# eloj/radix-sorting

Hardware: AMD Instinct MI355X
Metric: Gkeys/s sorting 2^28 u32 (1 GPU) + HBM GB/s vs roofline; 1/2/4/8-GPU scaling (higher is better)
Workload: dtype u32

## Files before the change

### radix_sorting_amd/csrc/rsx_env.hpp

```cpp
#pragma once

#include <algorithm>
#include <atomic>
#include <climits>
#include <cstdint>
#include <cstdlib>
#include <mutex>

namespace {

std::atomic<uint32_t> g_env_epoch{0};
enum : unsigned { UNIQUE_MAX_BITS_COMPILED = 30, UNIQUE_MAX_BITS_DEFAULT = 24 };
enum : unsigned { GROUP_MAX_BITS_COMPILED = 30, GROUP_MAX_BITS_DEFAULT = 24 };
enum : unsigned { LEX_PACK_BYTES_DEFAULT = 4 };
enum : unsigned { LOCATE_MAX_VALUES_DEFAULT = 4096 };
enum : unsigned { REDUCE_LDS_BITS_COMPILED = 12, REDUCE_MAX_BITS_COMPILED = 24, REDUCE_MAX_BITS_DEFAULT = 12 };
enum : unsigned { PARTITION_MAX_EDGES_COMPILED = 255, PARTITION_MAX_EDGES_DEFAULT = 3, PARTITION_BALLOT_PARTS_ENV_DEFAULT = 7 };
enum : unsigned { SEGMENTS_MAX_LONG_COMPILED = 4096, SEGMENTS_MAX_LONG_DEFAULT = 8, SEGMENTS_DEFAULT_CLASSES = 8 };
struct Env {
	bool host_register = false;
	bool force_table_rank = false;
	bool verify = false;
	bool verify_whole = false;
	bool verify_inject = false;
	bool no_hot = false;
	bool elem_loads = false;
	bool no_small_tiles = false;
	bool no_hybrid = false;
	bool no_small_sort = false;
	bool no_fill_runs = false;
	bool no_speculation = false;
	bool compact_bits = false;
	bool no_narrow_keys = false;
	bool no_host_small = false;
	bool no_fused_hist = false;
	bool no_slack = false;
	bool no_self_plan = false;
	bool no_blind = false;
	unsigned blind_min_log2 = 0;
	bool no_leaf_prefix = false;
	bool no_leaf16w2k = false;
	bool no_leaf16q = false;
	bool no_narrow_slots = false;
	bool no_aux_slots = false;
	bool no_narrow1 = false;
	bool no_dense_slots = false;
	bool force_dense_slots = false;
	bool no_unstable = false;
	bool no_shift = false;
	bool no_pass16 = false;
	unsigned pass16_wgs = 2;
	bool no_packed_keys = false;
	bool no_pass32a = false;
	unsigned pass32_min_mi = 0;
	int pass32_prefetch = -1;
	bool no_pass16a = false;
	unsigned pass16_dbg = 0;
	bool no_leafc = false;
	unsigned force_leafc = 0;
	bool no_leaf16 = false;
	unsigned leaf16_maxbin = 25;
	unsigned leaf_grid = 65536;
	unsigned two_level_min_log2 = 27;
	bool no_odd_stride = false;
	unsigned cap1_pad_kib = 0;
	unsigned probe = 0;
	bool no_pass64a = false;
	bool no_log = false;
	bool log_leaf_big = false;
	bool pairs_leaf_big = false;
	unsigned log_min_log2 = 0;
	unsigned unique_max_bits = UNIQUE_MAX_BITS_DEFAULT;
	unsigned group_max_bits = GROUP_MAX_BITS_DEFAULT;
	bool rankdata_no_tables = false;
	unsigned nth_force = 0;
	unsigned topk_force = 0;
	unsigned locate_force = 0;
	unsigned locate_max_values = LOCATE_MAX_VALUES_DEFAULT;
	unsigned locate_counter_sets = 0;
	unsigned reduce_max_bits = REDUCE_MAX_BITS_DEFAULT;
	unsigned reduce_lds_bits = REDUCE_LDS_BITS_COMPILED;
	unsigned reduce_replicas = 0;
	unsigned reduce_force = 0;
	unsigned join_force = 0;
	bool join_no_table = false;
	unsigned lex_pack_bytes = LEX_PACK_BYTES_DEFAULT;
	unsigned partition_force = 0;
	unsigned partition_max_edges = PARTITION_MAX_EDGES_DEFAULT;
	unsigned partition_ballot_parts = PARTITION_BALLOT_PARTS_ENV_DEFAULT;
	unsigned segments_force = 0;
	unsigned segments_max_long = SEGMENTS_MAX_LONG_DEFAULT;
	static bool is_set(const char *name) { return getenv(name) != nullptr; }
	static unsigned one_or_two(const char *name)
	{
		const char *e = getenv(name);
		return !e ? 0u : e[0] == '1' ? 1u : e[0] == '2' ? 2u : 0u;
	}
	static bool is_one(const char *name) { return one_or_two(name) == 1; }
	static void number(const char *name, unsigned *x, int lo = INT_MIN, int hi = INT_MAX)
	{
		if (const char *e = getenv(name))
			*x = (unsigned)std::max(lo, std::min(hi, atoi(e)));
	}
	static void within(const char *name, unsigned *x, int lo, int hi)
	{
		const char *e = getenv(name);
		if (e && atoi(e) >= lo && atoi(e) <= hi)
			*x = (unsigned)atoi(e);
	}
	static void one_else_two(const char *name, unsigned *x)
	{
		if (const char *e = getenv(name))
			*x = atoi(e) == 1 ? 1u : 2u;
	}
	void load()
	{
		*this = Env{};
		host_register = is_one("RSX_HOST_REGISTER");
		force_table_rank = is_one("RSX_FORCE_TABLE_RANK");
		verify = one_or_two("RSX_VERIFY") == 1;
		verify_whole = one_or_two("RSX_VERIFY") == 2;
		verify_inject = is_set("RSX_VERIFY_INJECT");
		no_hot = is_set("RSX_NO_HOT");
		elem_loads = is_one("RSX_ELEM_LOADS");
		no_small_tiles = is_set("RSX_NO_SMALL_TILES");
		no_hybrid = is_one("RSX_NO_HYBRID");
		no_small_sort = is_set("RSX_NO_SMALL_SORT");
		no_fill_runs = is_set("RSX_NO_FILL_RUNS");
		no_speculation = is_set("RSX_NO_SPECULATION");
		compact_bits = is_one("RSX_COMPACT_BITS");
		no_narrow_keys = is_set("RSX_NO_NARROW_KEYS");
		no_host_small = is_set("RSX_NO_HOST_SMALL");
		no_fused_hist = is_one("RSX_NO_FUSED_HIST");
		no_slack = is_one("RSX_NO_SLACK");
		no_self_plan = is_one("RSX_NO_SELF_PLAN");
		no_blind = is_one("RSX_NO_BLIND");
		number("RSX_BLIND_MIN_LOG2", &blind_min_log2, 22, 30);
		no_leaf_prefix = is_one("RSX_NO_LEAF_PREFIX");
		no_leaf16q = is_one("RSX_NO_LEAF16Q");
		no_narrow_slots = is_one("RSX_NO_NARROW_SLOTS");
		no_aux_slots = is_one("RSX_NO_AUX_SLOTS");
		no_narrow1 = is_one("RSX_NO_NARROW_LEVEL1");
		no_dense_slots = is_one("RSX_NO_DENSE_SLOTS");
		force_dense_slots = is_one("RSX_DENSE_SLOTS");
		no_leaf16 = is_one("RSX_NO_LEAF16");
		no_leafc = is_one("RSX_NO_LEAFC");
		no_leaf16w2k = is_one("RSX_NO_LEAF16W2K");
		number("RSX_PASS32_MIN_MI", &pass32_min_mi);
		if (is_set("RSX_PASS32_PREFETCH"))
			pass32_prefetch = is_one("RSX_PASS32_PREFETCH");
		number("RSX_FORCE_LEAFC", &force_leafc);
		no_pass16 = is_one("RSX_NO_PASS16");
		no_pass16a = is_one("RSX_NO_PASS16A");
		no_pass32a = is_one("RSX_NO_PASS32A");
		no_packed_keys = is_one("RSX_NO_PACKED_KEYS");
		one_else_two("RSX_PASS16_WGS", &pass16_wgs);
		number("RSX_PASS16_DBG", &pass16_dbg);
		no_shift = is_one("RSX_NO_SHIFT");
		no_unstable = is_one("RSX_NO_UNSTABLE");
		number("RSX_LEAF16_MAXBIN", &leaf16_maxbin, 0, 25);
		number("RSX_LEAF_GRID", &leaf_grid, 256, 65536);
		no_odd_stride = is_one("RSX_NO_ODD_STRIDE");
		number("RSX_CAP1_PAD_KIB", &cap1_pad_kib, 0, 65536);
		number("RSX_PROBE", &probe);
		no_pass64a = is_one("RSX_NO_PASS64A");
		no_log = is_one("RSX_NO_LOG");
		log_leaf_big = is_one("RSX_LOG_LEAF_BIG");
		pairs_leaf_big = is_one("RSX_PAIRS_LEAF_BIG");
		number("RSX_LOG_MIN_LOG2", &log_min_log2, 20, 29);
		rankdata_no_tables = is_one("RSX_RANKDATA_NO_TABLES");
		topk_force = one_or_two("RSX_TOPK_FORCE");
		nth_force = one_or_two("RSX_NTH_FORCE");
		locate_force = one_or_two("RSX_LOCATE_FORCE");
		within("RSX_LOCATE_MAX_VALUES", &locate_max_values, 1, (int)LOCATE_MAX_VALUES_DEFAULT);
		within("RSX_LOCATE_COUNTER_SETS", &locate_counter_sets, 1, 32);
		within("RSX_LEX_PACK_BYTES", &lex_pack_bytes, 1, 8);
		partition_force = one_or_two("RSX_PARTITION_FORCE");
		within("RSX_PARTITION_MAX_EDGES", &partition_max_edges, 1, (int)PARTITION_MAX_EDGES_COMPILED);
		within("RSX_PARTITION_BALLOT_PARTS", &partition_ballot_parts, 0, 256);
		segments_force = one_or_two("RSX_SEGMENTS_FORCE");
		within("RSX_SEGMENTS_MAX_LONG", &segments_max_long, 0, (int)SEGMENTS_MAX_LONG_COMPILED);
		number("RSX_REDUCE_MAX_BITS", &reduce_max_bits, 0, (int)REDUCE_MAX_BITS_COMPILED);
		number("RSX_REDUCE_LDS_BITS", &reduce_lds_bits, 0, (int)REDUCE_LDS_BITS_COMPILED);
		within("RSX_REDUCE_REPLICAS", &reduce_replicas, 1, 32);
		reduce_force = one_or_two("RSX_REDUCE_FORCE");
		within("RSX_JOIN_FORCE", &join_force, 2, 3);
		join_no_table = is_one("RSX_JOIN_NO_TABLE");
		number("RSX_UNIQUE_MAX_BITS", &unique_max_bits, 0, (int)UNIQUE_MAX_BITS_COMPILED);
		number("RSX_GROUP_MAX_BITS", &group_max_bits, 0, (int)GROUP_MAX_BITS_COMPILED);
		within("RSX_TWO_LEVEL_MIN_LOG2", &two_level_min_log2, 22, 30);
	}
};
Env g_env;
std::once_flag g_env_once;
inline const Env &env()
{
	std::call_once(g_env_once, [] { g_env.load(); });
	return g_env;
}

}
```

### radix_sorting_amd/csrc/rsx_hybrid.hpp

```cpp
#pragma once

#include "rsx_kernels.hpp"

namespace rsx {

enum : u32 { HYB_NONE = 0, HYB_ONE_LEVEL = 1, HYB_TWO_LEVEL = 2 };
enum : u32 { SEG_MODE_NONE = 0, SEG_MODE_LEAVES = 1, SEG_MODE_LSD = 2, SEG_MODE_RETRY = 3 };
static_assert(GATE_DONE == SEG_MODE_LEAVES, "the gate of the histogram-first kernels is SegCtl::mode");

struct SegTile {
	u32 beg, cnt, bucket, first;
};

struct SegCtl {
	u32 ntiles;
	u32 mode;
	u32 maxleaf;
	u32 done;
	u32 nleaf;
	u32 overflow;
	u32 blind;
	u32 cmask_lo, cmask_hi, key0_lo, key0_hi;
	u32 nredo;
	u32 leaf16;
	u32 shift1, shift2;
	u32 narrow;
	u32 compact;
	u32 cpiece[4];
	u32 craw0, cvnot;
	u32 ckind;
	u32 boff_skip, boff_next;
};
__device__ __forceinline__ void segctl_attempt_lost(SegCtl *ctl)
{
	const u32 nx = ctl->boff_next ? (ctl->boff_next < 32u ? 2u * ctl->boff_next : 64u) : 1u;
	ctl->boff_next = nx;
	ctl->boff_skip = nx;
}
enum : u32 { BLIND_NONE = 0, BLIND_GO = 1, BLIND_FAILED = 2 };

template <typename KT>
__device__ __forceinline__ u32 compact_key(u32 raw, const u32 (&piece)[4], u32 nb, const KdfArgs<KT> ka)
{
	u32 c = 0;
#pragma unroll
	for (int i = 0; i < 4; ++i) {
		const u32 p = piece[i];
		c |= __builtin_amdgcn_ubfe(raw, p & 31u, (p >> 8) & 63u) << (p >> 16);
	}
	const u32 all = nb >= 32u ? ~0u : (1u << nb) - 1u;
	const bool neg = ka.fmask != 0 && (raw >> 31) != 0;
	const u32 top = (piece[0] & 31u) + ((piece[0] >> 8) & 63u) == 32u ? 1u << (nb - 1u) : 0u;
	u32 flip = neg ? all : (ka.sflip ? top : 0u);
	if (ka.desc)
		flip ^= all;
	return c ^ flip;
}

struct LeafSeg {
	u32 beg, cnt, ncols;
	u32 slot;
};

constexpr u32 LEAF_MERGE_CAP = 4096;

__device__ __forceinline__ u32 block_scan_256(u32 v, u32 *s_w, u32 &tot)
{
	const u32 lane = threadIdx.x & 63, wid = threadIdx.x >> 6;
	u32 x = v;
#pragma unroll
	for (int off = 1; off < 64; off <<= 1) {
		const u32 y = __shfl_up(x, off);
		if (lane >= (u32)off)
			x += y;
	}
	if (lane == 63)
		s_w[wid] = x;
	__syncthreads();
	u32 base = 0;
#pragma unroll
	for (int k = 0; k < 4; ++k) {
		if (k < (int)wid)
			base += s_w[k];
	}
	tot = s_w[0] + s_w[1] + s_w[2] + s_w[3];
	__syncthreads();
	return base + x - v;
}

__device__ __forceinline__ u32 fixedpoint_key(u32 raw, u32 scale_bits, u32 nb, bool nonneg, bool desc, u32 &bad)
{
	const float tf = __uint_as_float(raw) * __uint_as_float(scale_bits);
	const float hi = __uint_as_float((127u + nb - (nonneg ? 0u : 1u)) << 23);
	const float lo = nonneg ? 0.0f : -hi;
	const int t = (int)tf;
	if (!(tf >= lo && tf < hi) || (float)t != tf || raw == 0x80000000u)
		bad |= 1u;
	u32 key = nonneg ? (u32)t : (u32)(t + (int)(1u << (nb - 1u)));
	if (desc)
		key = ~key & ((1u << nb) - 1u);
	return key;
}

__global__ __launch_bounds__(256) void rsx_seg_tiles_kernel(const u64 *__restrict__ ghist, u64 n, const Plan *__restrict__ plan,
                                                            u32 tile, SegTile *__restrict__ tiles, SegCtl *__restrict__ ctl,
                                                            u32 *__restrict__ btile,
                                                            u64 *__restrict__ off1_out = nullptr, u32 blind_cap = 0,
                                                            const u32 *__restrict__ status0 = nullptr, u32 ntiles0 = 0,
                                                            u32 back_cap = 0, u32 tile_narrow = 0,
                                                            u32 tile_narrow2 = 0)
{
	if (plan->hyb != HYB_TWO_LEVEL || (blind_cap && ctl->blind != BLIND_GO))
		return;
	if (tile_narrow && ctl->narrow)
		tile = (tile_narrow2 && ctl->narrow == 2u) ? tile_narrow2 : tile_narrow;
	__shared__ u32 s_size[256], s_tb[257], s_beg[256], s_w[4], s_back[256];
	const u32 d = threadIdx.x;
	u32 size, back = 0;
	if (blind_cap) {
		if (back_cap) {
			size = __hip_atomic_load(status0 + d, __ATOMIC_RELAXED, __HIP_MEMORY_SCOPE_AGENT);
			back = __hip_atomic_load(status0 + 256 + d, __ATOMIC_RELAXED, __HIP_MEMORY_SCOPE_AGENT);
			size += back;
		} else {
			size = __hip_atomic_load(status0 + ((u64)(ntiles0 - 1) * 256 + d), __ATOMIC_RELAXED, __HIP_MEMORY_SCOPE_AGENT) & StatusBits<u32>::VALMASK;
		}
		const bool over = size > blind_cap || ctl->overflow != 0;
		u32 tot1;
		const u32 o = block_scan_256(size, s_w, tot1);
		if (blockIdx.x == 0)
			off1_out[d] = o;
		if (__syncthreads_or(over ? 1 : 0)) {
			if (blockIdx.x == 0 && d == 0) {
				ctl->blind = BLIND_FAILED;
				segctl_attempt_lost(ctl);
			}
			return;
		}
		s_beg[d] = d * blind_cap;
	} else {
		const u64 *off1 = ghist + 256 * plan->cols[plan->ncols - 1];
		const u64 b = off1[d], e = d == 255 ? n : off1[d + 1];
		size = (u32)(e - b);
		s_beg[d] = (u32)b;
	}
	s_size[d] = size;
	s_back[d] = back;
	u32 total;
	const u32 tb = block_scan_256((size - back + tile - 1) / tile + (back ? 1u : 0u), s_w, total);
	s_tb[d] = tb;
	if (d == 0) {
		s_tb[256] = total;
		if (blockIdx.x == 0) {
			ctl->ntiles = total;
			btile[256] = total;
		}
	}
	if (blockIdx.x == 0)
		btile[d] = tb;
	__syncthreads();
	for (u32 t = blockIdx.x * 256 + d; t < total; t += gridDim.x * 256) {
		u32 lo = 0, hi = 256;
		while (hi - lo > 1) {
			const u32 mid = (lo + hi) >> 1;
			if (s_tb[mid] <= t)
				lo = mid;
			else
				hi = mid;
		}
		while (s_tb[lo + 1] <= t)
			++lo;
		const u32 k = lo, j = t - s_tb[k];
		SegTile st;
		const u32 front = s_size[k] - s_back[k];
		if (j * tile < front) {
			st.beg = s_beg[k] + j * tile;
			const u32 left = front - j * tile;
			st.cnt = left < tile ? left : tile;
		} else {
			st.beg = s_beg[k] + blind_cap - back_cap;
			st.cnt = s_back[k];
		}
		st.bucket = k;
		st.first = s_tb[k];
		tiles[t] = st;
	}
}

template <typename KT>
__global__ __launch_bounds__(1024) void rsx_seg_hist_kernel(const KT *__restrict__ keys, const SegTile *__restrict__ tiles,
                                                            const SegCtl *__restrict__ ctl, const Plan *__restrict__ plan,
                                                            KdfArgs<KT> ka, u32 *__restrict__ seghist)
{
	if (plan->hyb != HYB_TWO_LEVEL || ctl->mode != SEG_MODE_LSD)
		return;
	constexpr int MAXS = sizeof(KT) - 1;
	__shared__ u32 h[MAXS][256];
	const u32 tid = threadIdx.x;
	const u32 nslots = plan->ncols - 2;
	u32 shifts[MAXS];
#pragma unroll
	for (int k = 0; k < MAXS; ++k)
		shifts[k] = 8 * plan->cols[k < (int)nslots ? k : 0];
	const u32 nt = ctl->ntiles;
	const u32 t0 = (u32)((u64)nt * blockIdx.x / gridDim.x), t1 = (u32)((u64)nt * (blockIdx.x + 1) / gridDim.x);
	if (t0 == t1)
		return;
	for (u32 i = tid; i < MAXS * 256; i += 1024)
		(&h[0][0])[i] = 0;
	__syncthreads();
	u32 bucket = tiles[t0].bucket;
	auto flush = [&]() {
		__syncthreads();
		for (u32 i = tid; i < nslots * 256; i += 1024) {
			const u32 v = (&h[0][0])[i];
			if (v)
				atomicAdd(&seghist[(u64)bucket * (MAXS * 256) + i], v);
			(&h[0][0])[i] = 0;
		}
		__syncthreads();
	};
	for (u32 t = t0; t < t1; ++t) {
		const SegTile st = tiles[t];
		if (st.bucket != bucket) {
			flush();
			bucket = st.bucket;
		}
		const KT *p = keys + st.beg;
		constexpr int U = 8;
		for (u32 i0 = 0; i0 < st.cnt; i0 += 1024 * U) {
			KT v[U];
#pragma unroll
			for (int u = 0; u < U; ++u) {
				const u32 i = i0 + u * 1024 + tid;
				v[u] = i < st.cnt ? p[i] : (KT)0;
			}
#pragma unroll
			for (int u = 0; u < U; ++u) {
				const u32 i = i0 + u * 1024 + tid;
				if (i < st.cnt) {
					const KT k = kdf_apply(v[u], ka);
#pragma unroll
					for (int s = 0; s < MAXS; ++s)
						if (s < (int)nslots)
							atomicAdd(&h[s][(u32)(k >> shifts[s]) & 0xFFu], 1u);
				}
			}
		}
	}
	flush();
}

template <typename KT>
__global__ __launch_bounds__(1024) void rsx_seg_hist1_kernel(const KT *__restrict__ keys, const SegTile *__restrict__ tiles,
                                                             const SegCtl *__restrict__ ctl, const Plan *__restrict__ plan,
                                                             KdfArgs<KT> ka, u32 *__restrict__ seghist)
{
	if (plan->hyb != HYB_TWO_LEVEL)
		return;
	constexpr int MAXS = sizeof(KT) - 1, NW = 16;
	__shared__ u32 h[NW][256];
	const u32 tid = threadIdx.x, wid = tid >> 6;
	const u32 slot = plan->ncols - 2;
	const u32 shift = 8 * plan->cols[slot];
	const u32 nt = ctl->ntiles;
	const u32 t0 = (u32)((u64)nt * blockIdx.x / gridDim.x), t1 = (u32)((u64)nt * (blockIdx.x + 1) / gridDim.x);
	if (t0 == t1)
		return;
	for (u32 i = tid; i < NW * 256; i += 1024)
		(&h[0][0])[i] = 0;
	__syncthreads();
	u32 bucket = tiles[t0].bucket;
	auto flush = [&]() {
		__syncthreads();
		if (tid < 256) {
			u32 v = 0;
#pragma unroll
			for (int w = 0; w < NW; ++w) {
				v += h[w][tid];
				h[w][tid] = 0;
			}
			if (v)
				atomicAdd(&seghist[((u64)bucket * MAXS + slot) * 256 + tid], v);
		}
		__syncthreads();
	};
	u32 *hw = h[wid];
	for (u32 t = t0; t < t1; ++t) {
		const SegTile st = tiles[t];
		if (st.bucket != bucket) {
			flush();
			bucket = st.bucket;
		}
		const KT *p = keys + st.beg;
		constexpr int U = 8;
		for (u32 i0 = 0; i0 < st.cnt; i0 += 1024 * U) {
			KT v[U];
			if (i0 + 1024 * U <= st.cnt) {
#pragma unroll
				for (int u = 0; u < U; ++u)
					v[u] = p[i0 + u * 1024 + tid];
#pragma unroll
				for (int u = 0; u < U; ++u)
					atomicAdd(&hw[digit_of(v[u], ka, shift)], 1u);
			} else {
#pragma unroll
				for (int u = 0; u < U; ++u) {
					const u32 i = i0 + u * 1024 + tid;
					v[u] = i < st.cnt ? p[i] : (KT)0;
				}
#pragma unroll
				for (int u = 0; u < U; ++u) {
					const u32 i = i0 + u * 1024 + tid;
					if (i < st.cnt)
						atomicAdd(&hw[digit_of(v[u], ka, shift)], 1u);
				}
			}
		}
	}
	flush();
}

template <typename KT>
__global__ __launch_bounds__(256) void rsx_seg_plan_kernel(u32 *__restrict__ seghist, const u64 *__restrict__ ghist, u64 n,
                                                           const Plan *__restrict__ plan, SegCtl *__restrict__ ctl,
                                                           LeafSeg *__restrict__ segtab, u32 leaf_cap, SegCtl *host_ctl,
                                                           u32 phase)
{
	if (plan->hyb != HYB_TWO_LEVEL || (phase == 1 && ctl->mode != SEG_MODE_LSD))
		return;
	constexpr int MAXS = sizeof(KT) - 1;
	__shared__ u64 tot[256];
	__shared__ u64 lsum[64];
	__shared__ u32 s_max;
	const u32 d = threadIdx.x, b = blockIdx.x;
	const u32 nslots = plan->ncols - 1;
	const u64 *off1 = ghist + 256 * plan->cols[plan->ncols - 1];
	const u64 bbeg = off1[b];
	if (d == 0)
		s_max = 0;
	for (u32 s = phase ? 0 : nslots - 1; s < (phase ? nslots - 1 : nslots); ++s) {
		u32 *row = seghist + ((u64)b * MAXS + s) * 256;
		const u32 c = row[d];
		__syncthreads();
		tot[d] = c;
		__syncthreads();
		if (d < 64)
			wave_scan_256(tot, lsum, d);
		__syncthreads();
		row[d] = (u32)tot[d];
		if (s == nslots - 1) {
			__shared__ u32 s_cnt[256], s_start[257], s_first[257], s_w[4];
			constexpr u32 H = LEAF_MERGE_CAP / 2;
			const u32 o = (u32)tot[d];
			s_cnt[d] = c;
			__syncthreads();
			const bool opens = d == 0 || c > H || s_cnt[d - 1] > H || (o / H) != ((o - s_cnt[d - 1]) / H);
			u32 nleaf;
			const u32 idx = block_scan_256(opens ? 1u : 0u, s_w, nleaf);
			if (opens) {
				s_start[idx] = o;
				s_first[idx] = d;
			}
			if (d == 0) {
				s_start[nleaf] = o;
				s_first[nleaf] = 256;
			}
			__syncthreads();
			if (d == 255)
				s_start[nleaf] = o + c;
			__syncthreads();
			__shared__ u32 s_slot;
			if (d == 0)
				s_slot = atomicAdd(&ctl->nleaf, nleaf);
			__syncthreads();
			u32 mine = 0;
			if (d < nleaf) {
				LeafSeg ls;
				ls.beg = (u32)(bbeg + s_start[d]);
				ls.cnt = s_start[d + 1] - s_start[d];
				ls.ncols = nslots - 1 + (s_first[d + 1] - s_first[d] > 1 ? 1u : 0u);
				ls.slot = 0;
				segtab[s_slot + d] = ls;
				mine = ls.cnt;
			}
			atomicMax(&s_max, mine);
		}
	}
	if (phase)
		return;
	__syncthreads();
	__shared__ u32 s_last;
	if (d == 0) {
		atomicMax(&ctl->maxleaf, s_max);
		__threadfence();
		s_last = atomicAdd(&ctl->done, 1u) == gridDim.x - 1 ? 1u : 0u;
	}
	__syncthreads();
	if (s_last && d == 0) {
		__threadfence();
		const u32 mx = atomicMax(&ctl->maxleaf, 0u);
		const u32 mode = mx <= leaf_cap ? SEG_MODE_LEAVES : SEG_MODE_LSD;
		ctl->mode = mode;
		if (host_ctl) {
			host_ctl->ntiles = ctl->ntiles;
			host_ctl->maxleaf = mx;
			host_ctl->nleaf = ctl->nleaf;
			host_ctl->mode = mode;
			__threadfence_system();
		}
	}
}

template <typename ST>
__global__ __launch_bounds__(256) void rsx_seg_slack_plan_kernel(const ST *__restrict__ status, const u32 *__restrict__ btile,
                                                                 const u64 *__restrict__ ghist, const Plan *__restrict__ plan,
                                                                 SegCtl *__restrict__ ctl, LeafSeg *__restrict__ segtab,
                                                                 u32 slack_cap, SegCtl *host_ctl,
                                                                 const u64 *__restrict__ off1_given = nullptr, u32 blind_ = 0)
{
	u32 blind = blind_ & 0xFFu;
	const u32 rev = blind_ >> 8;
	if (blind == 3u)
		blind = ctl->narrow ? 2u : 1u;
	if (plan->hyb != HYB_TWO_LEVEL || (blind && ctl->blind != BLIND_GO))
		return;
	typedef StatusBits<ST> SB_;
	__shared__ u32 s_w[4];
	const u32 d = threadIdx.x, b = blockIdx.x;
	const u64 *off1 = off1_given ? off1_given : ghist + 256 * plan->cols[plan->ncols - 1];
	const u32 t0 = btile[b], t1 = btile[b + 1];
	const u32 ncols = plan->ncols;
	const u64 bbeg = off1[b];
	u32 c = 0, back = 0;
	if (blind == 2) {
		c = (u32)__hip_atomic_load(status + ((u64)b * 256 + d), __ATOMIC_RELAXED, __HIP_MEMORY_SCOPE_AGENT);
		back = (u32)__hip_atomic_load(status + ((u64)65536 + b * 256 + d), __ATOMIC_RELAXED, __HIP_MEMORY_SCOPE_AGENT);
		c += back;
	} else if (t1 > t0) {
		c = (u32)(__hip_atomic_load(status + ((u64)(t1 - 1) * 256 + d), __ATOMIC_RELAXED, __HIP_MEMORY_SCOPE_AGENT) & SB_::VALMASK);
	}
	if (b == 0 && d == 0) {
		const u32 mode = ctl->overflow == 0 ? SEG_MODE_LEAVES : SEG_MODE_RETRY;
		ctl->mode = mode;
		ctl->nleaf = 65536;
		ctl->maxleaf = slack_cap;
		if (blind) {
			if (mode == SEG_MODE_LEAVES)
				ctl->boff_next = 0;
			else
				segctl_attempt_lost(ctl);
		}
		if (host_ctl) {
			host_ctl->ntiles = ctl->ntiles;
			host_ctl->maxleaf = slack_cap;
			host_ctl->nleaf = 65536;
			host_ctl->overflow = ctl->overflow;
			host_ctl->narrow = ctl->narrow;
			host_ctl->mode = mode;
		}
	}
	u32 total;
	const u32 o = block_scan_256(c, s_w, total);
	LeafSeg ls;
	ls.beg = (u32)(bbeg + o);
	ls.cnt = c <= slack_cap ? c : 0u;
	ls.ncols = (ncols - 2) | (back << 16);
	ls.slot = b * 256 + d + 1;
	segtab[rev ? 65535u - (b * 256 + d) : b * 256 + d] = ls;
}

template <typename KT>
__global__ __launch_bounds__(1024) void rsx_blind_precheck_kernel(const KT *__restrict__ src, u64 n, KdfArgs<KT> ka,
                                                                  SegCtl *__restrict__ ctl, Plan *__restrict__ plan,
                                                                  Plan *host_plan, u32x4 *__restrict__ z, u64 nz, u32 min_cols,
                                                                  u32 allow_shift = 0, u32 allow_narrow = 0, u32 allow_compact = 0,
                                                                  u32 backoff = 0,
                                                                  u32 hints = 0)
{
	constexpr u32 W = sizeof(KT), S = 8, NS = 1024 * S;
	__shared__ u32 h[W][256];
	__shared__ u32 s_desc, s_distinct[W], s_max[W];
	__shared__ u32 h12[4096];
	__shared__ u32 s_max12;
	__shared__ u32 hs[2][256];
	__shared__ u32 s_vary, s_maxs[2];
	const u32 tid = threadIdx.x;
	if (blockIdx.x != 0) {
		const u32x4 zero = {0, 0, 0, 0};
		for (u64 i = (u64)(blockIdx.x - 1) * 1024 + tid; i < nz; i += (u64)(gridDim.x - 1) * 1024)
			z[i] = zero;
		return;
	}
	for (u32 i = tid; i < W * 256; i += 1024)
		(&h[0][0])[i] = 0;
	if (tid < W) {
		s_distinct[tid] = 0;
		s_max[tid] = 0;
	}
	if (tid == 0)
		s_desc = s_max12 = s_vary = s_maxs[0] = s_maxs[1] = 0;
#pragma unroll
	for (u32 i = 0; i < 4; ++i)
		h12[tid + 1024 * i] = 0;
	if (tid < 512)
		(&hs[0][0])[tid] = 0;
	__syncthreads();
	const u64 i0 = ((n - 16 * S) / 63) * (tid >> 4) + (tid & 15u) * S;
	KT k[S];
#pragma unroll
	for (u32 e = 0; e < S; ++e)
		k[e] = kdf_apply(src[i0 + e], ka);
	bool desc = false;
#pragma unroll
	for (u32 e = 0; e < S; ++e) {
		if (e)
			desc |= k[e] < k[e - 1];
#pragma unroll
		for (u32 c = 0; c < W; ++c)
			atomicAdd(&h[c][(u32)(k[e] >> (8 * c)) & 0xFFu], 1u);
	}
	if (__ballot(desc) && (tid & 63) == 0)
		s_desc = 1;
	if constexpr (W == 4) {
		const u32 kw = (u32)__builtin_amdgcn_readfirstlane((int)(u32)k[0]);
		u32 v = 0;
#pragma unroll
		for (u32 e = 0; e < S; ++e)
			v |= (u32)k[e] ^ kw;
#pragma unroll
		for (int off = 32; off > 0; off >>= 1)
			v |= (u32)__shfl_xor((int)v, off);
		if ((tid & 63) == 0)
			atomicOr(&s_vary, v | (kw ^ (u32)kdf_apply(src[0], ka)));
	}
	__syncthreads();
	if (tid < 256) {
#pragma unroll
		for (u32 c = 0; c < W; ++c) {
			const u32 v = h[c][tid];
			const u64 m = __ballot(v != 0);
			u32 mx = v;
#pragma unroll
			for (int off = 32; off > 0; off >>= 1) {
				const u32 y = __shfl_xor(mx, off);
				mx = y > mx ? y : mx;
			}
			if ((tid & 63) == 0) {
				atomicAdd(&s_distinct[c], (u32)__popcll(m));
				atomicMax(&s_max[c], mx);
			}
		}
	}
	__syncthreads();
	u32 shift1 = 0, shift2 = 0;
	{
		u32 nk = 0, ck[8] = {0, 0, 0, 0, 0, 0, 0, 0};
#pragma unroll
		for (u32 c = 0; c < W; ++c) {
			if (s_distinct[c] >= 2)
				ck[nk++] = c;
		}
		bool shifted = false;
		if (nk >= 2) {
			shift1 = 8 * ck[nk - 1];
			shift2 = 8 * ck[nk - 2];
		}
		if constexpr (W == 4) {
			const u32 hb = s_vary ? 31u - (u32)__builtin_clz(s_vary) : 0u;
			if (allow_shift && nk == 4 && hb < 31u && hb >= 23u) {
				shift1 = hb - 7;
				shift2 = hb - 15;
				shifted = true;
			}
		}
		if (nk >= 4) {
#pragma unroll
			for (u32 e = 0; e < S; ++e) {
				atomicAdd(&hs[0][(u32)(k[e] >> shift1) & 0xFFu], 1u);
				atomicAdd(&hs[1][(u32)(k[e] >> shift2) & 0xFFu], 1u);
			}
			if (shifted) {
				const u32 lowmask = (1u << shift2) - 1u, d = shift2 > 12u ? shift2 - 12u : 0u;
#pragma unroll
				for (u32 e = 0; e < S; ++e)
					atomicAdd(&h12[((u32)k[e] & lowmask) >> d], 1u);
			} else {
				const u32 sh_hi = 8 * ck[nk - 3], sh_nx = 8 * ck[nk - 4] + 4;
#pragma unroll
				for (u32 e = 0; e < S; ++e)
					atomicAdd(&h12[(((u32)(k[e] >> sh_hi) & 0xFFu) << 4) | ((u32)(k[e] >> sh_nx) & 0xFu)], 1u);
			}
		}
		__syncthreads();
		u32 m = 0;
#pragma unroll
		for (u32 i = 0; i < 4; ++i)
			m = m > h12[tid + 1024 * i] ? m : h12[tid + 1024 * i];
		u32 ms = tid < 512 ? (&hs[0][0])[tid] : 0u;
#pragma unroll
		for (int off = 32; off > 0; off >>= 1) {
			const u32 y = __shfl_xor(m, off), ys = __shfl_xor(ms, off);
			m = y > m ? y : m;
			ms = ys > ms ? ys : ms;
		}
		if ((tid & 63) == 0) {
			atomicMax(&s_max12, m);
			if (tid < 512)
				atomicMax(&s_maxs[tid >> 8], ms);
		}
		__syncthreads();
	}
	__shared__ u32 s_vraw, s_cnb, s_cpiece[4], s_cmax[2], s_fx[3], s_fxnb, s_fxscale, s_ckind;
	if constexpr (W == 4) {
		if (allow_compact) {
			const u32 raw0 = (u32)src[0];
			u32 raw[S];
			u32 v = 0;
#pragma unroll
			for (u32 e = 0; e < S; ++e) {
				raw[e] = (u32)src[i0 + e];
				v |= raw[e] ^ raw0;
			}
#pragma unroll
			for (int off = 32; off > 0; off >>= 1)
				v |= (u32)__shfl_xor((int)v, off);
			if (tid == 0)
				s_vraw = s_cnb = s_cmax[0] = s_cmax[1] = s_ckind = s_fxnb = s_fxscale = 0;
			if (tid < 512)
				(&hs[0][0])[tid] = 0;
			__syncthreads();
			if ((tid & 63) == 0)
				atomicOr(&s_vraw, v);
			__syncthreads();
			if (tid == 0) {
				u32 vv = s_vraw, np = 0, nb = (u32)__popc(vv), left = nb;
				bool ok = nb >= 17u && nb <= 30u;
				u32 pc[4] = {0, 0, 0, 0};
				while (vv && ok) {
					const u32 hi = 31u - (u32)__builtin_clz(vv);
					const u32 below = ~vv & ((2u << hi) - 1u);
					const u32 lo = below ? 32u - (u32)__builtin_clz(below) : 0u;
					const u32 w = hi - lo + 1u;
					if (np == 4) {
						ok = false;
						break;
					}
					left -= w;
					pc[np++] = lo | (w << 8) | (left << 16);
					vv &= lo ? (1u << lo) - 1u : 0u;
				}
				for (u32 i = 0; i < 4; ++i)
					s_cpiece[i] = pc[i];
				s_cnb = ok ? nb : 0u;
			}
			__syncthreads();
			const u32 cnb = s_cnb;
			if (cnb) {
				const u32 pc[4] = {s_cpiece[0], s_cpiece[1], s_cpiece[2], s_cpiece[3]};
#pragma unroll
				for (u32 e = 0; e < S; ++e) {
					const u32 c = compact_key<KT>(raw[e], pc, cnb, ka);
					atomicAdd(&hs[0][(c >> (cnb - 8u)) & 0xFFu], 1u);
					atomicAdd(&hs[1][(c >> (cnb - 16u)) & 0xFFu], 1u);
				}
			}
			__syncthreads();
			if (cnb) {
				u32 ms = tid < 512 ? (&hs[0][0])[tid] : 0u;
#pragma unroll
				for (int off = 32; off > 0; off >>= 1) {
					const u32 ys = __shfl_xor(ms, off);
					ms = ys > ms ? ys : ms;
				}
				if ((tid & 63) == 0 && tid < 512)
					atomicMax(&s_cmax[tid >> 8], ms);
			}
			__syncthreads();
			const bool packed_ok = s_cnb && s_cmax[0] <= 2 * NS / 256 && s_cmax[1] <= 2 * NS / 256;
			if (!packed_ok && ka.fmask != 0) {
				u32 lo = 0xFFFFFFFFu, hi = 0, flags = 0;
#pragma unroll
				for (u32 e = 0; e < S; ++e) {
					const u32 E = (raw[e] >> 23) & 0xFFu, M = raw[e] & 0x7FFFFFu;
					flags |= (E == 255u || raw[e] == 0x80000000u) ? 1u : 0u;
					flags |= (raw[e] >> 31) ? 2u : 0u;
					if (raw[e] & 0x7FFFFFFFu) {
						const u32 mant = E ? (M | 0x800000u) : M, Ee = E ? E : 1u;
						const u32 w = 256u + Ee - 150u + (u32)__builtin_ctz(mant);
						lo = w < lo ? w : lo;
						const u32 t = 256u + Ee - 126u;
						hi = t > hi ? t : hi;
					}
				}
#pragma unroll
				for (int off = 32; off > 0; off >>= 1) {
					const u32 a = (u32)__shfl_xor((int)lo, off), b = (u32)__shfl_xor((int)hi, off);
					lo = a < lo ? a : lo;
					hi = b > hi ? b : hi;
					flags |= (u32)__shfl_xor((int)flags, off);
				}
				if (tid == 0) {
					s_fx[0] = 0xFFFFFFFFu;
					s_fx[1] = s_fx[2] = 0;
					s_cmax[0] = s_cmax[1] = 0;
					s_fxnb = 0;
				}
				if (tid < 512)
					(&hs[0][0])[tid] = 0;
				__syncthreads();
				if ((tid & 63) == 0) {
					atomicMin(&s_fx[0], lo);
					atomicMax(&s_fx[1], hi);
					atomicOr(&s_fx[2], flags);
				}
				__syncthreads();
				if (tid == 0 && (s_fx[2] & 1u) == 0 && s_fx[1] > s_fx[0]) {
					const int e0 = (int)s_fx[0] - 256, e1 = (int)s_fx[1] - 256;
					const int nb = e1 - e0 + ((s_fx[2] & 2u) ? 1 : 0);
					if (nb >= 17 && nb <= 30 && 127 - e0 >= 1 && 127 - e0 <= 254) {
						s_fxnb = (u32)nb;
						s_fxscale = (u32)(127 - e0) << 23;
					}
				}
				__syncthreads();
				const u32 fnb = s_fxnb;
				if (fnb) {
					const u32 sc = s_fxscale;
					u32 bad = 0;
#pragma unroll
					for (u32 e = 0; e < S; ++e) {
						const u32 c = fixedpoint_key(raw[e], sc, fnb, (s_fx[2] & 2u) == 0, ka.desc != 0, bad);
						atomicAdd(&hs[0][(c >> (fnb - 8u)) & 0xFFu], 1u);
						atomicAdd(&hs[1][(c >> (fnb - 16u)) & 0xFFu], 1u);
					}
					(void)bad;
				}
				__syncthreads();
				if (fnb) {
					u32 ms = tid < 512 ? (&hs[0][0])[tid] : 0u;
#pragma unroll
					for (int off = 32; off > 0; off >>= 1) {
						const u32 ys = __shfl_xor(ms, off);
						ms = ys > ms ? ys : ms;
					}
					if ((tid & 63) == 0 && tid < 512)
						atomicMax(&s_cmax[tid >> 8], ms);
				}
				__syncthreads();
				if (tid == 0 && fnb) {
					s_cnb = fnb;
					s_ckind = 1;
				}
				__syncthreads();
			}
		}
	}
	if (tid == 0) {
		bool go = s_desc != 0;
		u32 nk = 0, cols[8] = {0, 0, 0, 0, 0, 0, 0, 0};
		u64 cmask = 0;
		for (u32 c = 0; c < W; ++c) {
			if (s_distinct[c] >= 2)
				cols[nk++] = c;
			else
				cmask |= (u64)0xFFu << (8 * c);
		}
		if (shift1 + 8 < 8 * W)
			cmask |= ~(((u64)1 << (shift1 + 8)) - 1) & (W == 8 ? ~(u64)0 : (((u64)1 << (8 * (W & 7))) - 1));
		go = go && nk >= min_cols;
		for (u32 i = 0; i + 2 < nk; ++i) {
			go = go && s_max[cols[i]] <= NS / 10;
		}
		go = go && ((hints & 1u) || s_maxs[0] <= 2 * NS / 256) && s_maxs[1] <= 2 * NS / 256;
		const u32 nbins12 = (shift1 & 7u) && shift2 < 12u ? 1u << shift2 : 4096u;
		const u32 max12_ok = 3 * (NS / nbins12) + 18u;
		if (shift1 & 7u)
			go = go && s_max12 <= max12_ok;
		u32 compact = 0;
		if constexpr (W == 4) {
			if (!go && allow_compact && s_cnb && s_desc != 0 && nk == 4 && s_cmax[0] <= 2 * NS / 256 && s_cmax[1] <= 2 * NS / 256) {
				compact = s_cnb;
				go = true;
				shift1 = compact - 8u;
				shift2 = compact - 16u;
				cmask = 0;
			}
		}
		if (backoff && ctl->boff_skip) {
			ctl->boff_skip -= 1u;
			go = false;
			compact = 0;
		}
		ctl->compact = compact;
		ctl->ckind = compact ? s_ckind : 0u;
		for (u32 i = 0; i < 4; ++i)
			ctl->cpiece[i] = compact ? (s_ckind ? (i == 0 ? s_fxscale : i == 1 ? ((s_fx[2] & 2u) ? 0u : 1u) : 0u) : s_cpiece[i]) : 0u;
		ctl->craw0 = compact ? (u32)src[0] : 0u;
		ctl->cvnot = compact ? ~s_vraw : 0u;
		ctl->ntiles = ctl->mode = ctl->maxleaf = ctl->done = ctl->nleaf = ctl->overflow = ctl->nredo = 0;
		ctl->blind = go ? BLIND_GO : BLIND_FAILED;
		ctl->leaf16 = (s_max12 <= max12_ok || compact) ? 1u : 0u;
		u32 narrow = (W == 8 && allow_narrow && go && nk >= 4 && cols[nk - 3] <= 3u && s_max12 <= max12_ok) ? 1u : 0u;
		if (narrow && allow_narrow >= 2u && ((shift1 & 7u) ? shift1 <= 32u : cols[nk - 2] <= 3u))
			narrow = 2u;
		ctl->narrow = narrow;
		ctl->shift1 = shift1;
		ctl->shift2 = shift2;
		ctl->cmask_lo = (u32)cmask;
		ctl->cmask_hi = (u32)(cmask >> 32);
		ctl->key0_lo = (u32)(u64)k[0];
		ctl->key0_hi = (u32)((u64)k[0] >> 32);
		if (go) {
			Plan *const out[2] = {plan, host_plan};
			for (int j = 0; j < 2; ++j) {
				out[j]->ncols = nk;
				out[j]->sorted = 0;
				for (u32 i = 0; i < 8; ++i)
					out[j]->cols[i] = i < nk ? cols[i] : 0u;
				out[j]->hot = 0;
				out[j]->vary_lo = out[j]->vary_hi = 0;
				out[j]->hyb = HYB_TWO_LEVEL;
				out[j]->max1 = 0;
			}
		}
	}
}

template <typename KT, int NW_, int KPT_, int WPE_ = 1, bool RANK1_ = true, bool PREFETCH_ = false> struct LeafCfg {
	static constexpr int NW = NW_, KPT = KPT_, BLOCK = NW_ * 64, CAP = NW_ * 64 * KPT_;
	static constexpr int WPE = WPE_;
	static constexpr bool RANK1 = RANK1_;
	static constexpr bool PREFETCH = PREFETCH_;
	static_assert(CAP <= 32768, "ranks and positions are kept in 16 bits");
};

template <typename KT, typename C, typename CT = KT, bool DENSE = false>
__global__ __launch_bounds__(C::BLOCK, C::WPE) void rsx_leaf_sort_kernel(KT *__restrict__ src, KT *__restrict__ aux, u64 n,
                                                                  const u64 *__restrict__ ghist, const Plan *__restrict__ plan,
                                                                  const LeafSeg *__restrict__ segtab,
                                                                  const SegCtl *__restrict__ ctl, KdfArgs<KT> ka, u32 level,
                                                                  u32 lo, u32 hi, const KT *__restrict__ slots = nullptr,
                                                                  u32 slack_cap = 0, u32 skip_narrowable = 0,
                                                                  const u64 *__restrict__ off1_given = nullptr,
                                                                  const u32 *__restrict__ redo = nullptr)
{
	constexpr int NW = C::NW, KPT = C::KPT, BLOCK = C::BLOCK;
	constexpr bool NARROW = sizeof(CT) < sizeof(KT);
	constexpr int CHUNK = 16 / sizeof(CT);
	constexpr int G = 4;
	static_assert(KPT % G == 0, "whole groups of rounds");
	const u32 hyb = plan->hyb, ncols = plan->ncols, max1 = plan->max1;
	u32 colpack = 0;
#pragma unroll
	for (int k = 0; k < 8; ++k)
		colpack |= (plan->cols[k] & 15u) << (4 * k);
	const u32 mode = level == HYB_TWO_LEVEL ? ctl->mode : (u32)SEG_MODE_LEAVES;
	const u32 maxleaf = level == HYB_TWO_LEVEL ? ctl->maxleaf : max1;
	const bool listed = redo != nullptr && ctl->leaf16 != 0;
	const u32 nseg = level == HYB_TWO_LEVEL ? (listed ? ctl->nredo : ctl->nleaf) : 256u;
	if (hyb != level || mode != SEG_MODE_LEAVES || maxleaf <= lo || maxleaf > hi)
		return;
	const u64 *off1 = off1_given ? off1_given : ghist + 256 * ((colpack >> (4 * (ncols - 1))) & 15u);
	const KT *in = level == HYB_TWO_LEVEL ? src : aux;
	KT *out = (ncols & 1) ? aux : src;

	__shared__ __attribute__((aligned(16))) CT stage[C::CAP];
	__shared__ u32 cell[NW][256];
	__shared__ u32 wsum[4];
	__shared__ KT s_upper;
	const u32 tid = threadIdx.x, lane = tid & 63, wid = tid >> 6;
	auto opaque = [](u32 x) {
		asm volatile("" : "+v"(x));
		return x;
	};
	const CT pad = (CT)~(CT)0;
	auto bounds = [&](u32 s, u32 &beg, u32 &cnt, u32 &nc, u32 &slot) {
		slot = 0;
		if (level == HYB_TWO_LEVEL) {
			const LeafSeg ls = segtab[listed ? redo[s] : s];
			beg = ls.beg;
			cnt = ls.cnt;
			nc = ls.ncols & 0xFFFFu;
			slot = ls.slot;
		} else {
			const u64 b = off1[s], e = s == 255 ? n : off1[s + 1];
			beg = (u32)b;
			cnt = (u32)(e - b);
			nc = ncols - 1;
		}
	};
	const u32 swid = (u32)__builtin_amdgcn_readfirstlane((int)wid);
	auto wave_groups = [&](u32 cnt, u32 ng) {
		const u32 first = swid * ng * (64 * G);
		const u32 mine = cnt > first ? cnt - first : 0u;
		const u32 g = (mine + 64 * G - 1) / (64 * G);
		return g < ng ? g : ng;
	};
	KT first_raw = 0;
	auto request = [&](auto &dst, u32 beg, u32 cnt, u32 slot) {
		const u32 ngall = (cnt + BLOCK * G - 1) / (BLOCK * G);
		const u32 ng = wave_groups(cnt, ngall);
		const u32 wo = opaque(wid * (ngall * 64 * G) + lane);
		if constexpr (DENSE) {
			const CT *q = (const CT *)slots + (u64)(slot - 1) * slack_cap;
#pragma unroll
			for (int g = 0; g < KPT / G; ++g) {
				if (g < (int)ng) {
#pragma unroll
					for (int r = g * G; r < (g + 1) * G; ++r) {
						const u32 i = wo + r * 64;
						dst[r] = i < cnt ? q[i] : pad;
					}
				}
			}
			return;
		}
		const KT *p = slot ? slots + (u64)(slot - 1) * slack_cap : in + beg;
		if constexpr (NARROW)
			first_raw = p[0];
#pragma unroll
		for (int g = 0; g < KPT / G; ++g) {
			if (g < (int)ng) {
#pragma unroll
				for (int r = g * G; r < (g + 1) * G; ++r) {
					const u32 i = wo + r * 64;
					if constexpr (NARROW)
						dst[r] = i < cnt ? ((const CT *)p)[(sizeof(KT) / sizeof(CT)) * i] : (CT)kdf_invert((KT)~(KT)0, ka);
					else
						dst[r] = i < cnt ? p[i] : kdf_invert((KT)~(KT)0, ka);
				}
			}
		}
	};
	auto derive = [&](auto &dst, u32 cnt, u32 slot) {
		if constexpr (DENSE) {
			if (tid == 0) {
				const u32 c1 = (colpack >> (4 * (ncols - 1))) & 15u, c2 = (colpack >> (4 * (ncols - 2))) & 15u;
				const KT key0 = (KT)(((u64)ctl->key0_hi << 32) | ctl->key0_lo);
				const KT digits = (KT)((KT)0xFFu << (8 * c1)) | (KT)((KT)0xFFu << (8 * c2));
				const KT low = (KT)(((KT)1 << (8 * sizeof(CT))) - 1);
				s_upper = (KT)((key0 & ~digits & ~low) | ((KT)((slot - 1) >> 8) << (8 * c1)) | ((KT)((slot - 1) & 255u) << (8 * c2)));
			}
			return;
		}
		const u32 ngall = (cnt + BLOCK * G - 1) / (BLOCK * G);
		const u32 wo = opaque(wid * (ngall * 64 * G) + lane);
		constexpr u32 CBITS = NARROW ? 8 * sizeof(CT) : 0;
		KT upper_raw = 0;
		if constexpr (NARROW) {
			upper_raw = (KT)(first_raw >> CBITS << CBITS);
			if (tid == 0)
				s_upper = (KT)(kdf_apply(first_raw, ka) >> CBITS << CBITS);
		}
#pragma unroll
		for (int r = 0; r < KPT; ++r) {
			if constexpr (NARROW)
				dst[r] = wo + r * 64 < cnt ? (CT)kdf_apply((KT)(upper_raw | (KT)dst[r]), ka) : pad;
			else
				dst[r] = (CT)kdf_apply((KT)dst[r], ka);
		}
	};
	u32 s = blockIdx.x;
	if (s >= nseg)
		return;
	u32 nbeg, ncnt, nnc, nslot;
	bounds(s, nbeg, ncnt, nnc, nslot);
	static_assert(!C::PREFETCH || !NARROW, "one upper part at a time");
	CT nxt[C::PREFETCH ? KPT : 1];
	if constexpr (C::PREFETCH)
		request(nxt, nbeg, ncnt, nslot);
	for (;;) {
		const u32 beg = nbeg, cnt = ncnt, nrem = nnc, slot = nslot;
		const bool narrowable = nrem != 0 && ((colpack >> (4 * (nrem - 1))) & 15u) < 4u && sizeof(KT) == 8;
		if (cnt == 0 || (!DENSE && ((NARROW && !narrowable) || (!NARROW && (skip_narrowable & 1u) && narrowable)))) {
			s += gridDim.x;
			if (s >= nseg)
				break;
			bounds(s, nbeg, ncnt, nnc, nslot);
			continue;
		}
		const u32 ngall = (cnt + BLOCK * G - 1) / (BLOCK * G);
		const u32 per = ngall * (64 * G);
		const u32 ng = wave_groups(cnt, ngall);
		const u32 wo0 = wid * per + lane;
		CT keep[KPT];
		if constexpr (C::PREFETCH) {
#pragma unroll
			for (int r = 0; r < KPT; ++r)
				keep[r] = nxt[r];
		} else {
			request(keep, beg, cnt, slot);
		}
		derive(keep, cnt, slot);
		s += gridDim.x;
		const bool more = s < nseg;
		if (more) {
			bounds(s, nbeg, ncnt, nnc, nslot);
			if constexpr (C::PREFETCH)
				request(nxt, nbeg, ncnt, nslot);
		}
		constexpr bool PREFIX_OK = sizeof(CT) == 8;
		u32 c0 = 0;
		if constexpr (PREFIX_OK) {
			if (nrem >= 5 && !(skip_narrowable & 2u))
				c0 = nrem - 3;
		}
		for (;;) {
		for (u32 c = c0; c < nrem; ++c) {
			const u32 shift = 8 * ((colpack >> (4 * c)) & 15u);
#pragma unroll
			for (int k = 0; k < 4; ++k)
				cell[wid][lane + 64 * k] = 0;
			u32 *wc = cell[wid];
			u32 rk[C::RANK1 ? KPT / 2 : 1];
			if constexpr (C::RANK1) {
#pragma unroll
				for (int i = 0; i < KPT / 2; ++i)
					rk[i] = 0;
			}
#pragma unroll
			for (int g = 0; g < KPT / G; ++g) {
				if (g < (int)ng) {
#pragma unroll
					for (int r = g * G; r < (g + 1) * G; ++r) {
						const u32 old = __hip_atomic_fetch_add(&wc[(u32)(keep[r] >> shift) & 0xFFu], 1u, __ATOMIC_RELAXED,
						                                       __HIP_MEMORY_SCOPE_WORKGROUP);
						if constexpr (C::RANK1)
							rk[r >> 1] |= old << (16 * (r & 1));
					}
				}
			}
			__syncthreads();
			u32 tot = 0, incl = 0;
			if (tid < 256) {
#pragma unroll
				for (int w = 0; w < NW; ++w)
					tot += cell[w][tid];
				u32 x = tot;
#pragma unroll
				for (int off = 1; off < 64; off <<= 1) {
					const u32 y = __shfl_up(x, off);
					if (lane >= (u32)off)
						x += y;
				}
				incl = x;
				if (lane == 63)
					wsum[wid] = x;
			}
			__syncthreads();
			if (tid < 256) {
				u32 acc = incl - tot;
				for (u32 w = 0; w < wid; ++w)
					acc += wsum[w];
#pragma unroll
				for (int w = 0; w < NW; ++w) {
					const u32 k = cell[w][tid];
					cell[w][tid] = acc;
					acc += k;
				}
			}
			__syncthreads();
#pragma unroll
			for (int g = 0; g < KPT / G; ++g) {
				if (g < (int)ng) {
					u32 pos[G];
#pragma unroll
					for (int r = g * G; r < (g + 1) * G; ++r) {
						if constexpr (C::RANK1)
							pos[r - g * G] = wc[(u32)(keep[r] >> shift) & 0xFFu] + ((rk[r >> 1] >> (16 * (r & 1))) & 0xFFFFu);
						else
							pos[r - g * G] = __hip_atomic_fetch_add(&wc[(u32)(keep[r] >> shift) & 0xFFu], 1u, __ATOMIC_RELAXED,
							                                        __HIP_MEMORY_SCOPE_WORKGROUP);
					}
#pragma unroll
					for (int r = g * G; r < (g + 1) * G; ++r)
						stage[pos[r - g * G]] = keep[r];
				}
			}
			__syncthreads();
			if (c + 1 < nrem) {
				const u32 wo = opaque(wo0);
#pragma unroll
				for (int g = 0; g < KPT / G; ++g) {
					if (g < (int)ng) {
#pragma unroll
						for (int r = g * G; r < (g + 1) * G; ++r)
							keep[r] = stage[wo + r * 64];
					}
				}
			}
		}
		if constexpr (!PREFIX_OK) {
			break;
		} else {
			if (c0 == 0)
				break;
			bool rest = false;
			for (u32 it = 0; it < 4 && !rest; ++it) {
				u32 sw = 0;
				for (u32 i = 2 * tid; i + 1 < cnt; i += 2 * BLOCK) {
					const CT a = stage[i], b = stage[i + 1];
					if (a > b) {
						stage[i] = b;
						stage[i + 1] = a;
						sw = 1;
					}
				}
				__syncthreads();
				for (u32 i = 2 * tid + 1; i + 1 < cnt; i += 2 * BLOCK) {
					const CT a = stage[i], b = stage[i + 1];
					if (a > b) {
						stage[i] = b;
						stage[i + 1] = a;
						sw = 1;
					}
				}
				rest = __syncthreads_or((int)sw) == 0;
			}
			if (rest)
				break;
			c0 = 0;
			const u32 wo = opaque(wo0);
#pragma unroll
			for (int g = 0; g < KPT / G; ++g) {
				if (g < (int)ng) {
#pragma unroll
					for (int r = g * G; r < (g + 1) * G; ++r)
						keep[r] = stage[wo + r * 64];
				}
			}
			__syncthreads();
		}
		}
		if (nrem) {
			KT *o = out + beg;
			for (u32 i0 = tid * CHUNK; i0 < cnt; i0 += BLOCK * CHUNK) {
				typedef CT kvec_t __attribute__((ext_vector_type(CHUNK)));
				const kvec_t x = *(const kvec_t *)&stage[i0];
				KT kv[CHUNK];
#pragma unroll
				for (int e = 0; e < CHUNK; ++e)
					kv[e] = kdf_invert(NARROW ? (KT)(s_upper | (KT)x[e]) : (KT)x[e], ka);
				if (i0 + CHUNK <= cnt) {
					if constexpr (sizeof(KT) * CHUNK > 16) {
						KT lo2[CHUNK / 2], hi2[CHUNK / 2];
#pragma unroll
						for (int e = 0; e < CHUNK / 2; ++e) {
							lo2[e] = kv[e];
							hi2[e] = kv[CHUNK / 2 + e];
						}
						store_chunk<KT, CHUNK / 2>(o + i0, lo2);
						store_chunk<KT, CHUNK / 2>(o + i0 + CHUNK / 2, hi2);
					} else {
						store_chunk<KT, CHUNK>(o + i0, kv);
					}
				} else {
#pragma unroll
					for (int e = 0; e < CHUNK; ++e)
						if (i0 + e < cnt)
							o[i0 + e] = kv[e];
				}
			}
		}
		if (!more)
			break;
		__syncthreads();
	}
}

template <typename KT, typename VT, typename C, bool K16 = false>
__global__ __launch_bounds__(C::BLOCK, C::WPE) void rsx_leaf_pairs_kernel(const KT *__restrict__ kslots, const VT *__restrict__ vslots,
                                                                           u32 slack_cap, KT *__restrict__ kout, VT *__restrict__ vout,
                                                                           const Plan *__restrict__ plan,
                                                                           const LeafSeg *__restrict__ segtab,
                                                                           const SegCtl *__restrict__ ctl, KdfArgs<KT> ka,
                                                                           u32 level = HYB_TWO_LEVEL,
                                                                           const u64 *__restrict__ ghist = nullptr, u64 n = 0,
                                                                           const u32 *__restrict__ redo = nullptr)
{
	static_assert(sizeof(KT) == 4 && sizeof(VT) == 4, "pairs of 4-byte keys and 4-byte payloads");
	constexpr int NW = C::NW, KPT = C::KPT, BLOCK = C::BLOCK, G = 4;
	static_assert(KPT % G == 0, "whole groups of rounds");
	if (plan->hyb != level || (level == HYB_TWO_LEVEL && ctl->mode != SEG_MODE_LEAVES))
		return;
	if (level == HYB_TWO_LEVEL && ctl->compact)
		ka.fmask = ka.sflip = ka.desc = 0;
	u32 colpack = 0;
#pragma unroll
	for (int k = 0; k < 8; ++k)
		colpack |= (plan->cols[k] & 15u) << (4 * k);
	const u32 ncols_all = plan->ncols;
	const bool listed = redo != nullptr && ctl->leaf16 != 0;
	const u32 nseg = level == HYB_TWO_LEVEL ? (listed ? ctl->nredo : ctl->nleaf) : 256u;
	const u64 *off1 = ghist + 256 * ((colpack >> (4 * (ncols_all - 1))) & 15u);
	__shared__ __attribute__((aligned(16))) u64 stage[C::CAP];
	__shared__ u32 cell[NW][256];
	__shared__ u32 wsum[4];
	const u32 tid = threadIdx.x, lane = tid & 63, wid = tid >> 6;
	const u32 swid = (u32)__builtin_amdgcn_readfirstlane((int)wid);
	auto opaque = [](u32 x) {
		asm volatile("" : "+v"(x));
		return x;
	};
	for (u32 s = blockIdx.x; s < nseg; s += gridDim.x) {
		LeafSeg ls;
		if (level == HYB_TWO_LEVEL) {
			ls = segtab[listed ? redo[s] : s];
		} else {
			const u64 b = off1[s], e = s == 255 ? n : off1[s + 1];
			ls.beg = (u32)b;
			ls.cnt = (u32)(e - b);
			ls.ncols = ncols_all - 1;
			ls.slot = 0;
		}
		const u32 cnt = ls.cnt, nrem = ls.ncols;
		if (cnt == 0)
			continue;
		const u32 ngall = (cnt + BLOCK * G - 1) / (BLOCK * G);
		const u32 per = ngall * (64 * G);
		const u32 first = swid * per;
		const u32 mine = cnt > first ? cnt - first : 0u;
		u32 ng = (mine + 64 * G - 1) / (64 * G);
		ng = ng < ngall ? ng : ngall;
		const u32 wo0 = wid * per + lane;
		const KT *kp = ls.slot ? kslots + (u64)(ls.slot - 1) * slack_cap : kslots + ls.beg;
		const unsigned short *kp16 = (const unsigned short *)kslots + (u64)(ls.slot ? ls.slot - 1 : 0u) * slack_cap;
		const KT upper16 = (KT)(((KT)((ls.slot - 1) >> 8) << 24) | ((KT)((ls.slot - 1) & 255u) << 16));
		const VT *vp = ls.slot ? vslots + (u64)(ls.slot - 1) * slack_cap : vslots + ls.beg;
		KT kr[KPT];
		VT vr[KPT];
		{
			const u32 wo = opaque(wo0);
#pragma unroll
			for (int g = 0; g < KPT / G; ++g) {
				if (g < (int)ng) {
#pragma unroll
					for (int r = g * G; r < (g + 1) * G; ++r) {
						const u32 i = wo + r * 64;
						if constexpr (K16)
							kr[r] = i < cnt ? (KT)(upper16 | (KT)kp16[i]) : (KT)~(KT)0;
						else
							kr[r] = i < cnt ? kp[i] : kdf_invert((KT)~(KT)0, ka);
						vr[r] = i < cnt ? vp[i] : (VT)0;
					}
				}
			}
		}
		u64 keep[KPT];
#pragma unroll
		for (int r = 0; r < KPT; ++r)
			keep[r] = ((u64)(K16 ? kr[r] : kdf_apply(kr[r], ka)) << 32) | (u64)vr[r];
		for (u32 c = 0; c < nrem; ++c) {
			const u32 shift = 32 + 8 * ((colpack >> (4 * c)) & 15u);
#pragma unroll
			for (int k = 0; k < 4; ++k)
				cell[wid][lane + 64 * k] = 0;
			u32 *wc = cell[wid];
			u32 rk[KPT / 2];
#pragma unroll
			for (int i = 0; i < KPT / 2; ++i)
				rk[i] = 0;
#pragma unroll
			for (int g = 0; g < KPT / G; ++g) {
				if (g < (int)ng) {
#pragma unroll
					for (int r = g * G; r < (g + 1) * G; ++r) {
						const u32 old = __hip_atomic_fetch_add(&wc[(u32)(keep[r] >> shift) & 0xFFu], 1u, __ATOMIC_RELAXED,
						                                       __HIP_MEMORY_SCOPE_WORKGROUP);
						rk[r >> 1] |= old << (16 * (r & 1));
					}
				}
			}
			__syncthreads();
			u32 tot = 0, incl = 0;
			if (tid < 256) {
#pragma unroll
				for (int w = 0; w < NW; ++w)
					tot += cell[w][tid];
				u32 x = tot;
#pragma unroll
				for (int off = 1; off < 64; off <<= 1) {
					const u32 y = __shfl_up(x, off);
					if (lane >= (u32)off)
						x += y;
				}
				incl = x;
				if (lane == 63)
					wsum[wid] = x;
			}
			__syncthreads();
			if (tid < 256) {
				u32 acc = incl - tot;
				for (u32 w = 0; w < wid; ++w)
					acc += wsum[w];
#pragma unroll
				for (int w = 0; w < NW; ++w) {
					const u32 k = cell[w][tid];
					cell[w][tid] = acc;
					acc += k;
				}
			}
			__syncthreads();
#pragma unroll
			for (int g = 0; g < KPT / G; ++g) {
				if (g < (int)ng) {
#pragma unroll
					for (int r = g * G; r < (g + 1) * G; ++r) {
						const u32 pos = wc[(u32)(keep[r] >> shift) & 0xFFu] + ((rk[r >> 1] >> (16 * (r & 1))) & 0xFFFFu);
						stage[pos] = keep[r];
					}
				}
			}
			__syncthreads();
			if (c + 1 < nrem) {
				const u32 wo = opaque(wo0);
#pragma unroll
				for (int g = 0; g < KPT / G; ++g) {
					if (g < (int)ng) {
#pragma unroll
						for (int r = g * G; r < (g + 1) * G; ++r)
							keep[r] = stage[wo + r * 64];
					}
				}
			}
		}
		VT *vo = vout + ls.beg;
		KT *ko = kout ? kout + ls.beg : nullptr;
		for (u32 i0 = tid * 2; i0 < cnt; i0 += BLOCK * 2) {
			typedef u64 pvec_t __attribute__((ext_vector_type(2)));
			const pvec_t x = *(const pvec_t *)&stage[i0];
			vo[i0] = (VT)(u32)x[0];
			if (ko)
				ko[i0] = kdf_invert((KT)(x[0] >> 32), ka);
			if (i0 + 1 < cnt) {
				vo[i0 + 1] = (VT)(u32)x[1];
				if (ko)
					ko[i0 + 1] = kdf_invert((KT)(x[1] >> 32), ka);
			}
		}
		__syncthreads();
	}
}

}
```

### radix_sorting_amd/csrc/rsx_pass16.hpp

```cpp
#pragma once

#include "rsx_kernels.hpp"
#include "rsx_hybrid.hpp"

namespace rsx {

template <int WGS_ = 2> struct Pass16Cfg {
	static constexpr int WGS = WGS_;
	static constexpr int BLOCK = 1024, KPT = 32, TILE = BLOCK * KPT;
	static constexpr int NGROUP = TILE / 8;
};

template <int WGS> struct Pass16Smem {
	__attribute__((aligned(16))) unsigned short stage[32768 + (WGS == 1 ? 8192 : 0)];
	u32 cell[256];
	u32 delta[256];
	unsigned short rend[256];
	unsigned char group_digit[4096];
	u32 wsum[4];
};

template <typename KT, int DIG, typename C = Pass16Cfg<2>>
__global__ __launch_bounds__(C::BLOCK, C::WGS * 4) void rsx_pass16_kernel(const KT *__restrict__ kin, const KT *__restrict__ kin_hi,
                                                                         u32 lo_slots, unsigned short *__restrict__ kout,
                                                                         const SegTile *__restrict__ tiles,
                                                                         const u32 *__restrict__ btile,
                                                                         const SegCtl *__restrict__ ctl,
                                                                         const Plan *__restrict__ plan, u32 *__restrict__ cursors,
                                                                         u32 slack_cap, u32 *__restrict__ overflow, KdfArgs<KT> ka,
                                                                         u32 dbg = 0)
{
	static_assert(sizeof(KT) == 4, "4-byte keys, two-byte values");
	constexpr int BLOCK = C::BLOCK, KPT = C::KPT, TILE = C::TILE;
	if (ctl->blind != BLIND_GO || plan->hyb != HYB_TWO_LEVEL)
		return;
	const u32 t = blockIdx.x;
	if (t >= ctl->ntiles)
		return;
	const SegTile st = tiles[t];
	const u32 cnt = st.cnt, bucket = st.bucket;
	const u32 shift = ctl->shift2;
	const u32 last_tile = btile[bucket + 1] - 1u;
	const KT *p = ((kin_hi && bucket >= lo_slots) ? kin_hi : kin) + st.beg;
	__shared__ Pass16Smem<C::WGS> sm;
	const u32 tid = threadIdx.x, lane = tid & 63, wid = tid >> 6;
	if (tid < 256)
		sm.cell[tid] = 0;
	__syncthreads();

	KT keep[KPT];
	const bool full = cnt == (u32)TILE;
	if (full && (((uintptr_t)p) & 15) == 0) {
		typedef KT vec_t __attribute__((ext_vector_type(4)));
		const vec_t *vp = (const vec_t *)p + tid;
#pragma unroll
		for (int i = 0; i < KPT / 4; ++i) {
			const vec_t v = vp[i * BLOCK];
#pragma unroll
			for (int e = 0; e < 4; ++e)
				keep[4 * i + e] = v[e];
		}
	} else {
#pragma unroll
		for (int r = 0; r < KPT; ++r) {
			const u32 o = tid + r * BLOCK;
			keep[r] = o < cnt ? p[o] : (KT)0;
		}
	}
	if constexpr (DIG != 1) {
#pragma unroll
		for (int r = 0; r < KPT; ++r)
			keep[r] = kdf_apply(keep[r], ka);
	}
	auto count = [&](auto full_c) {
		constexpr bool FULL = decltype(full_c)::value;
#pragma unroll
		for (int r = 0; r < KPT; ++r) {
			if (FULL || tid + r * BLOCK < cnt) {
				const u32 d = (u32)(keep[r] >> shift) & 0xFFu;
				atomicAdd(&sm.cell[d], 1u);
			}
		}
	};
	if (full)
		count(std::true_type{});
	else
		count(std::false_type{});
	__syncthreads();

	u32 c = 0, tb = 0, excl = 0;
	if (tid < 256) {
		c = sm.cell[tid];
		if (c)
			excl = __hip_atomic_fetch_add(cursors + ((u64)last_tile * 256u + tid), c, __ATOMIC_RELAXED, __HIP_MEMORY_SCOPE_AGENT);
		u32 x = c;
#pragma unroll
		for (int off = 1; off < 64; off <<= 1) {
			const u32 y = __shfl_up(x, off);
			if (lane >= (u32)off)
				x += y;
		}
		if (lane == 63)
			sm.wsum[wid] = x;
		tb = x - c;
	}
	__syncthreads();
	if (tid < 256) {
		for (u32 k = 0; k < wid; ++k)
			tb += sm.wsum[k];
		sm.cell[tid] = tb;
		sm.rend[tid] = (unsigned short)(tb + c);
		for (u32 g = (tb + 7u) >> 3; g < (tb + c + 7u) >> 3; ++g)
			sm.group_digit[g] = (unsigned char)tid;
	}
	__syncthreads();

	if (tid < 256) {
		u64 running = ((u64)bucket * 256u + tid) * slack_cap + excl;
		if (excl + c > slack_cap) {
			atomicOr(overflow, 1u);
			running = (u64)65536u * slack_cap;
		}
		sm.delta[tid] = (u32)running - tb;
	}
	auto stage = [&](auto full_c) {
		constexpr bool FULL = decltype(full_c)::value;
		u32 shift_b = shift;
		asm volatile("" : "+s"(shift_b));
#pragma unroll
		for (int r0 = 0; r0 < KPT; r0 += 8) {
			u32 pos[8];
#pragma unroll
			for (int r = 0; r < 8; ++r) {
				pos[r] = 0;
				if (FULL || tid + (r0 + r) * BLOCK < cnt) {
					const u32 d = (u32)(keep[r0 + r] >> shift_b) & 0xFFu;
					pos[r] = __hip_atomic_fetch_add(&sm.cell[d], 1u, __ATOMIC_RELAXED, __HIP_MEMORY_SCOPE_WORKGROUP);
				}
			}
#pragma unroll
			for (int r = 0; r < 8; ++r) {
				if (FULL || tid + (r0 + r) * BLOCK < cnt) {
					*(unsigned short *)((char *)sm.stage + stage_swz<true>(pos[r] * 2u)) = (unsigned short)keep[r0 + r];
				}
			}
		}
	};
	if (full)
		stage(std::true_type{});
	else
		stage(std::false_type{});
	__syncthreads();

#pragma unroll 1
	for (u32 i0 = 8u * tid; i0 < cnt; i0 += 8u * BLOCK) {
		const u32x4 x = *(const u32x4 *)((const char *)sm.stage + stage_swz<true>(i0 * 2u));
		u32 d = sm.group_digit[i0 >> 3];
		const u32 re = sm.rend[d];
		if (dbg) {
			if (dbg == 2) {
				const u32 b0 = i0 & ~31u;
				if (sm.group_digit[b0 >> 3] == d && b0 + 32u <= re && b0 + 32u <= cnt) {
					typedef u32x4 avec_t __attribute__((aligned(16)));
					*(avec_t *)(kout + (u32)(((sm.delta[d] + b0) & ~31u) + (i0 - b0))) = x;
				}
			}
			continue;
		}
		if (i0 + 8u <= re && i0 + 8u <= cnt) {
			typedef u32x4 uvec_t __attribute__((aligned(2)));
			*(uvec_t *)(kout + (u32)(sm.delta[d] + i0)) = x;
		} else {
			const u64 lo = ((u64)x[1] << 32) | x[0], hi = ((u64)x[3] << 32) | x[2];
#pragma unroll 1
			for (u32 e = 0; e < 8u && i0 + e < cnt; ++e) {
				const u32 pos = i0 + e;
				while ((u32)sm.rend[d] <= pos)
					++d;
				kout[(u32)(sm.delta[d] + pos)] = (unsigned short)((e < 4u ? lo : hi) >> (16u * (e & 3u)));
			}
		}
	}
}


struct Pass16aCfg {
	static constexpr int BLOCK = 1024, KPT = 24, TILE = BLOCK * KPT;
	static constexpr u32 ATOM = 32;
	static constexpr u32 BACK = 128;
	static constexpr int STAGE = TILE + 256 * 14;
};

struct Pass16aSmem {
	__attribute__((aligned(16))) unsigned short stage[Pass16aCfg::STAGE];
	__attribute__((aligned(16))) unsigned short carry[256][32];
	u32 cell[2][256];
	u32 delta[256];
	u32 info[256];
	unsigned short rbeg[256], bbeg[256], bend[256];
	unsigned char group_digit[Pass16aCfg::STAGE / 8];
	u32 wsum[4];
};

template <typename KT, int DIG, bool PREFETCH = false>
__global__ __launch_bounds__(Pass16aCfg::BLOCK, 8) void rsx_pass16a_kernel(const KT *__restrict__ kin, const KT *__restrict__ kin_hi,
                                                                          u32 lo_slots, unsigned short *__restrict__ kout,
                                                                          const SegTile *__restrict__ tiles,
                                                                          const SegCtl *__restrict__ ctl,
                                                                          const Plan *__restrict__ plan, u32 *__restrict__ cursors,
                                                                          u32 slack_cap, u32 *__restrict__ overflow, KdfArgs<KT> ka)
{
	static_assert(sizeof(KT) == 4, "4-byte keys, two-byte values");
	typedef Pass16aCfg C;
	constexpr int BLOCK = C::BLOCK, KPT = C::KPT, TILE = C::TILE;
	if (ctl->blind != BLIND_GO || plan->hyb != HYB_TWO_LEVEL)
		return;
	const u32 ntiles = ctl->ntiles;
	const u32 per = (ntiles + gridDim.x - 1) / gridDim.x;
	const u32 t0 = blockIdx.x * per, t1 = t0 + per < ntiles ? t0 + per : ntiles;
	if (t0 >= t1)
		return;
	const u32 shift = ctl->shift2;
	const u32 gran = ctl->leaf16 ? C::ATOM : 1u;
	__shared__ Pass16aSmem sm;
	const u32 tid0 = threadIdx.x;
	auto sidx = [](u32 pos) { return stage_swz<true>(pos * 2u); };
	auto staged = [&](u32 pos) -> unsigned short & { return *(unsigned short *)((char *)sm.stage + sidx(pos)); };
	u32 cc = 0;
	u32 bucket = tiles[t0].bucket;
	if (tid0 < 256)
		sm.cell[0][tid0] = 0;
	auto flush = [&]() {
		const u32 tid = tid0, cd = tid >> 2, part = tid & 3u;
		__syncthreads();
		if (tid < 256) {
			u32 inf = 0, dest = 0;
			if (cc) {
				const u32 slot = bucket * 256u + tid;
				const u32 pos = __hip_atomic_fetch_add(cursors + 65536u + slot, cc, __ATOMIC_RELAXED, __HIP_MEMORY_SCOPE_AGENT);
				if (pos + cc > C::BACK)
					atomicOr(overflow, 1u);
				else {
					inf = cc;
					dest = slot * slack_cap + (slack_cap - C::BACK) + pos;
				}
			}
			sm.info[tid] = inf;
			sm.delta[tid] = dest;
			cc = 0;
		}
		__syncthreads();
		{
			const u32 n = sm.info[cd], dest = sm.delta[cd];
#pragma unroll 2
			for (u32 e = 0; e < 8; ++e) {
				const u32 k = part * 8u + e;
				if (k < n)
					kout[dest + k] = sm.carry[cd][k];
			}
		}
		__syncthreads();
	};
	__syncthreads();
	KT keep[KPT];
	auto request = [&](const u32 t, const u32 tid) {
		const SegTile st = tiles[t];
		const KT *p = ((kin_hi && st.bucket >= lo_slots) ? kin_hi : kin) + st.beg;
		if (st.cnt == (u32)TILE && (((uintptr_t)p) & 15) == 0) {
			typedef KT vec_t __attribute__((ext_vector_type(4)));
			const vec_t *vp = (const vec_t *)p + tid;
#pragma unroll
			for (int i = 0; i < KPT / 4; ++i) {
				const vec_t v = __builtin_nontemporal_load(&vp[i * BLOCK]);
#pragma unroll
				for (int e = 0; e < 4; ++e)
					keep[4 * i + e] = v[e];
			}
		} else {
#pragma unroll
			for (int r = 0; r < KPT; ++r) {
				const u32 o = tid + r * BLOCK;
				keep[r] = o < st.cnt ? p[o] : (KT)0;
			}
		}
	};
	if (blockIdx.x >= gridDim.x / 2)
		__builtin_amdgcn_s_sleep(127);
	if constexpr (PREFETCH)
		request(t0, tid0);
	for (u32 t = t0; t < t1; ++t) {
		u32 tid = tid0;
		asm volatile("" : "+v"(tid));
		const u32 lane = tid & 63, wid = tid >> 6;
		const u32 cd = tid >> 2, part = tid & 3u;
		u32 *const cell = sm.cell[(t - t0) & 1u];
		const SegTile st = tiles[t];
		if (st.bucket != bucket) {
			flush();
			bucket = st.bucket;
		}
		const u32 cnt = st.cnt;
		const bool full = cnt == (u32)TILE;
		if constexpr (!PREFETCH)
			request(t, tid);
		if constexpr (DIG != 1) {
#pragma unroll
			for (int r = 0; r < KPT; ++r)
				keep[r] = kdf_apply(keep[r], ka);
		}
		auto count = [&](auto full_c) {
			constexpr bool FULL = decltype(full_c)::value;
#pragma unroll
			for (int r = 0; r < KPT; ++r) {
				if (FULL || tid + r * BLOCK < cnt)
					atomicAdd(&cell[(u32)(keep[r] >> shift) & 0xFFu], 1u);
			}
		};
		if (full)
			count(std::true_type{});
		else
			count(std::false_type{});
		__syncthreads();

		u32 base = 0;
		{
			u32 rlen = 0, rstart = 0;
			if (tid < 256) {
				const u32 c = cell[tid];
				u32 h, body = 0, tail = 0, atom = 0;
				const bool enough = cc + c >= gran;
				if (enough) {
					h = cc ? gran - cc : 0u;
					atom = cc ? 1u : 0u;
					body = (c - h) & ~(gran - 1u);
					tail = (c - h) & (gran - 1u);
				} else {
					h = c;
				}
				const u32 m = atom * gran + body;
				if (m)
					base = __hip_atomic_fetch_add(cursors + (bucket * 256u + tid), m, __ATOMIC_RELAXED, __HIP_MEMORY_SCOPE_AGENT);
				const u32 o = (8u - (h & 7u)) & 7u;
				rlen = (o + c + 7u) & ~7u;
				sm.info[tid] = cc | (h << 6) | (tail << 12) | (atom << 18) | ((enough ? 1u : 0u) << 19) | (o << 20);
				sm.bend[tid] = (unsigned short)body;
				cc = enough ? tail : cc + c;
				u32 x = rlen;
#pragma unroll
				for (int off = 1; off < 64; off <<= 1) {
					const u32 y = __shfl_up(x, off);
					if (lane >= (u32)off)
						x += y;
				}
				if (lane == 63)
					sm.wsum[wid] = x;
				rstart = x - rlen;
			}
			__syncthreads();
			if (tid < 256) {
				for (u32 k = 0; k < wid; ++k)
					rstart += sm.wsum[k];
				const u32 inf = sm.info[tid];
				const u32 rb = rstart + (inf >> 20), bb = rb + ((inf >> 6) & 63u), be = bb + sm.bend[tid];
				cell[tid] = rb;
				sm.cell[((t - t0) & 1u) ^ 1u][tid] = 0;
				sm.rbeg[tid] = (unsigned short)rb;
				sm.bbeg[tid] = (unsigned short)bb;
				sm.bend[tid] = (unsigned short)be;
				for (u32 g = bb >> 3; g < (be + 7u) >> 3; ++g)
					sm.group_digit[g] = (unsigned char)tid;
			}
		}
		__syncthreads();

		if (tid < 256) {
			const u32 slot = bucket * 256u + tid;
			const u32 atom = (sm.info[tid] >> 18) & 1u, bb = sm.bbeg[tid], m = atom * gran + (sm.bend[tid] - bb);
			u32 dest = slot * slack_cap + base + atom * gran;
			if (m && base + m > slack_cap - C::BACK) {
				atomicOr(overflow, 1u);
				dest = 65536u * slack_cap + C::ATOM;
			}
			sm.delta[tid] = dest - bb;
		}
		u32 shift_b = shift;
		asm volatile("" : "+s"(shift_b));
		auto stage_keys = [&](auto full_c) {
			constexpr bool FULL = decltype(full_c)::value;
#pragma unroll
			for (int r0 = 0; r0 < KPT; r0 += 8) {
				u32 pos[8];
#pragma unroll
				for (int r = 0; r < 8; ++r) {
					pos[r] = 0;
					if (FULL || tid + (r0 + r) * BLOCK < cnt)
						pos[r] = __hip_atomic_fetch_add(&cell[(u32)(keep[r0 + r] >> shift_b) & 0xFFu], 1u, __ATOMIC_RELAXED,
						                                __HIP_MEMORY_SCOPE_WORKGROUP);
				}
#pragma unroll
				for (int r = 0; r < 8; ++r) {
					if (FULL || tid + (r0 + r) * BLOCK < cnt)
						staged(pos[r]) = (unsigned short)keep[r0 + r];
				}
			}
		};
		if (full)
			stage_keys(std::true_type{});
		else
			stage_keys(std::false_type{});
		__syncthreads();

		if constexpr (PREFETCH) {
			if (t + 1 < t1)
				request(t + 1, tid);
		}
		{
			const u32 inf = sm.info[cd];
			const u32 ccd = inf & 63u, hd = (inf >> 6) & 63u, atomd = (inf >> 18) & 1u;
			if (atomd) {
				const u32 rb = sm.rbeg[cd];
				u64 qlo = 0, qhi = 0;
#pragma unroll 1
				for (u32 half = 0; half < 2u; ++half) {
					u64 acc = 0;
#pragma unroll
					for (u32 e = 0; e < 4; ++e) {
						const u32 k = part * 8u + half * 4u + e;
						const u32 v = k < ccd ? (u32)sm.carry[cd][k] : (u32)staged(rb + (k - ccd));
						acc |= (u64)v << (16u * e);
					}
					if (half)
						qhi = acc;
					else
						qlo = acc;
				}
				(void)hd;
				typedef u32x4 avec_t __attribute__((aligned(16)));
				*(avec_t *)(kout + (u32)(sm.delta[cd] + sm.bbeg[cd] - C::ATOM + part * 8u)) =
				    u32x4{(u32)qlo, (u32)(qlo >> 32), (u32)qhi, (u32)(qhi >> 32)};
			}
		}
		{
			const u32 total = (u32)__builtin_amdgcn_readfirstlane((int)sm.wsum[0]) + sm.wsum[1] + sm.wsum[2] + sm.wsum[3];
#pragma unroll 1
			for (u32 i0 = 8u * tid; i0 < total; i0 += 8u * BLOCK) {
				const u32 d = sm.group_digit[i0 >> 3];
				const u32 bb = sm.bbeg[d], be = sm.bend[d];
				if (i0 >= bb && i0 < be) {
					const u32x4 x = *(const u32x4 *)((const char *)sm.stage + sidx(i0));
					if (i0 + 8u <= be) {
						typedef u32x4 uvec_t __attribute__((aligned(2)));
						*(uvec_t *)(kout + (u32)(sm.delta[d] + i0)) = x;
					} else {
						const u64 lo = ((u64)x[1] << 32) | x[0], hi = ((u64)x[3] << 32) | x[2];
#pragma unroll 1
						for (u32 e = 0; i0 + e < be; ++e)
							kout[(u32)(sm.delta[d] + i0 + e)] = (unsigned short)((e < 4u ? lo : hi) >> (16u * (e & 3u)));
					}
				}
			}
		}
		{
			const u32 inf = sm.info[cd];
			const u32 ccd = inf & 63u, hd = (inf >> 6) & 63u, taild = (inf >> 12) & 63u, fulld = (inf >> 19) & 1u;
			const u32 from = fulld ? sm.bend[cd] : sm.rbeg[cd], to = fulld ? 0u : ccd, n = fulld ? taild : hd;
#pragma unroll 2
			for (u32 e = 0; e < 8; ++e) {
				const u32 k = part * 8u + e;
				if (k < n)
					sm.carry[cd][to + k] = staged(from + k);
			}
		}
	}
	flush();
}

}
```

### radix_sorting_amd/csrc/rsx_pass32.hpp

```cpp
#pragma once

#include "rsx_kernels.hpp"
#include "rsx_hybrid.hpp"
#include "rsx_scatter2.hpp"

namespace rsx {

template <int KPT_ = 28, bool RANK1_ = true> struct Pass32aCfgT {
	static constexpr int BLOCK = 1024, KPT = KPT_, TILE = BLOCK * KPT;
	static constexpr bool RANK1 = RANK1_;
	static constexpr int WPE = KPT_ <= 12 ? 8 : 4;
	static constexpr int SB = KPT_ % 7 == 0 ? 7 : 6;
	static constexpr u32 ATOM = 16;
	static constexpr u32 BACK = 8192;
	static constexpr int STAGE = TILE + 256 * 6;
};
typedef Pass32aCfgT<28> Pass32aCfg;
constexpr u32 PASS32_BACK = Pass32aCfg::BACK;

template <typename KT, typename C, int REP = 1> struct Pass32aSmem {
	__attribute__((aligned(16))) KT stage[C::STAGE];
	__attribute__((aligned(16))) KT carry[256][64 / sizeof(KT)];
	__attribute__((aligned(16))) u32 cell[2][256 * REP];
	u32 delta[256];
	u32 info[256];
	unsigned short rbeg[256], bbeg[256], bend[256];
	unsigned char group_digit[C::STAGE / (16 / sizeof(KT))];
	u32 wsum[4];
};

template <typename KT, int DIG, bool PREFETCH = true, typename C = Pass32aCfg, int REP_ = 1, typename OT = KT>
__global__ __launch_bounds__(C::BLOCK, C::WPE) void rsx_pass32a_kernel(const KT *__restrict__ kin, u64 n, OT *__restrict__ kout,
                                                                          u32 lo_slots, u32 off_lo, u32 off_hi, u32 cap,
                                                                          const SegCtl *__restrict__ ctl,
                                                                          u32 *__restrict__ cursors, u32 *__restrict__ overflow,
                                                                          KdfArgs<KT> ka)
{
	static_assert(sizeof(KT) == 4 || sizeof(KT) == 8, "4- or 8-byte keys");
	constexpr int BLOCK = C::BLOCK, KPT = C::KPT, TILE = C::TILE, SB = C::SB;
	constexpr u32 VIN = 16 / sizeof(KT);
	constexpr u32 VEC = 16 / sizeof(OT);
	constexpr u32 ATOM = 64 / sizeof(OT);
	constexpr bool NARROW = sizeof(OT) != sizeof(KT);
	static_assert(!NARROW || (sizeof(KT) == 8 && sizeof(OT) == 4), "8-byte keys into four-byte slots, or the element images");
	static_assert(KPT % (int)VIN == 0, "whole vectors per lane");
	static_assert(sizeof(OT) == 4 || C::STAGE * sizeof(OT) + 256 * 64 <= 150 * 1024, "8-byte slots: 14 Ki-key tiles (Pass32aCfgT<14>)");
	if (ctl->blind != BLIND_GO)
		return;
	if constexpr (sizeof(KT) == 8) {
		if ((ctl->narrow == 2u) != NARROW)
			return;
	}
	const u32 ntiles = (u32)((n + TILE - 1) / TILE);
	const u32 per = (ntiles + gridDim.x - 1) / gridDim.x;
	const u32 t0 = blockIdx.x * per, t1 = t0 + per < ntiles ? t0 + per : ntiles;
	if (t0 >= t1)
		return;
	const u32 shift = ctl->shift1;
	const KT cmask = sizeof(KT) == 8 ? (KT)(((u64)ctl->cmask_hi << 32) | ctl->cmask_lo) : (KT)ctl->cmask_lo;
	const KT key0 = sizeof(KT) == 8 ? (KT)(((u64)ctl->key0_hi << 32) | ctl->key0_lo) : (KT)ctl->key0_lo;
	__shared__ Pass32aSmem<OT, C, REP_> sm;
	const u32 tid0 = threadIdx.x;
	auto sidx = [](u32 pos) { return stage_swz<true>(pos * (u32)sizeof(OT)); };
	auto staged = [&](u32 pos) -> OT & { return *(OT *)((char *)sm.stage + sidx(pos)); };
	auto slot_base = [&](u32 d) { return (d < lo_slots ? off_lo : off_hi) + d * cap; };
	u32 cc = 0;
	constexpr u32 REP = REP_;
	static_assert(REP == 1 || REP == 4, "one counter per digit, or one per lane class");
	if (tid0 < 256 * REP)
		sm.cell[0][tid0] = 0;
	__syncthreads();
	auto bucket_of = [&](KT k, u32 sh) -> u32 { return (u32)(k >> sh) & 0xFFu; };
	KT keep[KPT];
	auto request = [&](const u32 t, const u32 tid) {
		const u64 beg = (u64)t * TILE;
		const u32 cnt = n - beg < (u64)TILE ? (u32)(n - beg) : (u32)TILE;
		const KT *p = kin + beg;
		if (cnt == (u32)TILE && (((uintptr_t)p) & 15) == 0) {
			typedef KT vec_t __attribute__((ext_vector_type(VIN)));
			const vec_t *vp = (const vec_t *)p + tid;
#pragma unroll
			for (int i = 0; i < KPT / (int)VIN; ++i) {
				const vec_t v = vp[i * BLOCK];
#pragma unroll
				for (int e = 0; e < (int)VIN; ++e)
					keep[(int)VIN * i + e] = v[e];
			}
		} else {
#pragma unroll
			for (int r = 0; r < KPT; ++r) {
				const u32 o = tid + r * BLOCK;
				keep[r] = o < cnt ? p[o] : (KT)0;
			}
		}
	};
	if constexpr (PREFETCH)
		request(t0, tid0);
	for (u32 t = t0; t < t1; ++t) {
		u32 tid = tid0;
		asm volatile("" : "+v"(tid));
		const u32 lane = tid & 63, wid = tid >> 6;
		const u32 cd = tid >> 2, part = tid & 3u;
		u32 *const cell = sm.cell[(t - t0) & 1u];
		const u64 beg = (u64)t * TILE;
		const u32 cnt = n - beg < (u64)TILE ? (u32)(n - beg) : (u32)TILE;
		const bool full = cnt == (u32)TILE;
		if constexpr (!PREFETCH)
			request(t, tid);
		u32 rk[C::RANK1 ? (KPT + 1) / 2 : 1];
		auto count = [&](auto full_c) {
			constexpr bool FULL = decltype(full_c)::value;
			KT bad = 0;
#pragma unroll
			for (int r = 0; r < KPT; ++r) {
				u32 mine = 0;
				if (FULL || tid + r * BLOCK < cnt) {
					const KT k = DIG == 1 ? keep[r] : kdf_apply(keep[r], ka);
					bad |= (k ^ key0) & cmask;
					const u32 b = bucket_of(k, shift) * REP + (lane & (REP - 1u));
					if constexpr (C::RANK1)
						mine = __hip_atomic_fetch_add(&cell[b], 1u, __ATOMIC_RELAXED, __HIP_MEMORY_SCOPE_WORKGROUP);
					else
						atomicAdd(&cell[b], 1u);
				}
				if constexpr (C::RANK1)
					rk[r >> 1] = (r & 1) ? rk[r >> 1] | (mine << 16) : mine;
			}
			if (__ballot(bad != 0) && lane == 0)
				atomicOr(overflow, 1u);
		};
		if (full)
			count(std::true_type{});
		else
			count(std::false_type{});
		__syncthreads();

		u32 base = 0;
		{
			u32 rlen = 0, rstart = 0;
			u32 crep[REP];
			if (tid < 256) {
				u32 c = 0;
#pragma unroll
				for (u32 q = 0; q < REP; ++q) {
					crep[q] = cell[tid * REP + q];
					c += crep[q];
				}
				u32 h, body = 0, tail = 0, atom = 0;
				const bool enough = cc + c >= ATOM;
				if (enough) {
					h = cc ? ATOM - cc : 0u;
					atom = cc ? 1u : 0u;
					body = (c - h) & ~(ATOM - 1u);
					tail = (c - h) & (ATOM - 1u);
				} else {
					h = c;
				}
				const u32 m = atom * ATOM + body;
				if (m)
					base = __hip_atomic_fetch_add(cursors + tid, m, __ATOMIC_RELAXED, __HIP_MEMORY_SCOPE_AGENT);
				const u32 o = (VEC - (h & (VEC - 1u))) & (VEC - 1u);
				rlen = (o + c + VEC - 1u) & ~(VEC - 1u);
				sm.info[tid] = cc | (h << 5) | (tail << 10) | (atom << 15) | ((enough ? 1u : 0u) << 16) | (o << 17);
				sm.bend[tid] = (unsigned short)body;
				cc = enough ? tail : cc + c;
				u32 x = rlen;
#pragma unroll
				for (int off = 1; off < 64; off <<= 1) {
					const u32 y = __shfl_up(x, off);
					if (lane >= (u32)off)
						x += y;
				}
				if (lane == 63)
					sm.wsum[wid] = x;
				rstart = x - rlen;
			}
			__syncthreads();
			if (tid < 256) {
				for (u32 k = 0; k < wid; ++k)
					rstart += sm.wsum[k];
				const u32 inf = sm.info[tid];
				const u32 rb = rstart + (inf >> 17), bb = rb + ((inf >> 5) & 31u), be = bb + sm.bend[tid];
				u32 rq = rb;
#pragma unroll
				for (u32 q = 0; q < REP; ++q) {
					cell[tid * REP + q] = rq;
					rq += crep[q];
					sm.cell[((t - t0) & 1u) ^ 1u][tid * REP + q] = 0;
				}
				sm.rbeg[tid] = (unsigned short)rb;
				sm.bbeg[tid] = (unsigned short)bb;
				sm.bend[tid] = (unsigned short)be;
				for (u32 g = bb / VEC; g < (be + VEC - 1u) / VEC; ++g)
					sm.group_digit[g] = (unsigned char)tid;
			}
		}
		__syncthreads();

		if (tid < 256) {
			const u32 atom = (sm.info[tid] >> 15) & 1u, bb = sm.bbeg[tid], m = atom * ATOM + (sm.bend[tid] - bb);
			u32 dest = slot_base(tid) + base + atom * ATOM;
			if (m && base + m > cap - C::BACK) {
				atomicOr(overflow, 1u);
				dest = slot_base(tid) + ATOM;
			}
			sm.delta[tid] = dest - bb;
		}
		u32 shift_b = shift;
		asm volatile("" : "+s"(shift_b));
		auto stage_keys = [&](auto full_c) {
			constexpr bool FULL = decltype(full_c)::value;
#pragma unroll
			for (int r0 = 0; r0 < KPT; r0 += SB) {
				u32 pos[SB];
#pragma unroll
				for (int r = 0; r < SB; ++r) {
					pos[r] = 0;
					if (FULL || tid + (r0 + r) * BLOCK < cnt) {
						const KT k = DIG == 1 ? keep[r0 + r] : kdf_apply(keep[r0 + r], ka);
						const u32 b = bucket_of(k, shift_b) * REP + (lane & (REP - 1u));
						if constexpr (C::RANK1)
							pos[r] = cell[b] + ((rk[(r0 + r) >> 1] >> (16 * ((r0 + r) & 1))) & 0xFFFFu);
						else
							pos[r] = __hip_atomic_fetch_add(&cell[b], 1u, __ATOMIC_RELAXED, __HIP_MEMORY_SCOPE_WORKGROUP);
					}
				}
#pragma unroll
				for (int r = 0; r < SB; ++r) {
					if (FULL || tid + (r0 + r) * BLOCK < cnt) {
						if constexpr (NARROW)
							staged(pos[r]) = (OT)(DIG == 1 ? keep[r0 + r] : kdf_apply(keep[r0 + r], ka));
						else
							staged(pos[r]) = keep[r0 + r];
					}
				}
			}
		};
		if (full)
			stage_keys(std::true_type{});
		else
			stage_keys(std::false_type{});
		__syncthreads();
		if constexpr (PREFETCH) {
			if (t + 1 < t1)
				request(t + 1, tid);
		}

		{
			const u32 inf = sm.info[cd];
			const u32 ccd = inf & 31u, atomd = (inf >> 15) & 1u;
			if (atomd) {
				const u32 rb = sm.rbeg[cd];
				typedef OT kvec_t __attribute__((ext_vector_type(VEC)));
				typedef kvec_t avec_t __attribute__((aligned(16)));
				kvec_t w;
#pragma unroll
				for (u32 e = 0; e < VEC; ++e) {
					const u32 k = part * VEC + e;
					w[e] = k < ccd ? sm.carry[cd][k] : staged(rb + (k - ccd));
				}
				*(avec_t *)(kout + (u32)(sm.delta[cd] + sm.bbeg[cd] - ATOM + part * VEC)) = w;
			}
		}
		{
			const u32 total = (u32)__builtin_amdgcn_readfirstlane((int)sm.wsum[0]) + sm.wsum[1] + sm.wsum[2] + sm.wsum[3];
#pragma unroll 1
			for (u32 i0 = VEC * tid; i0 < total; i0 += VEC * BLOCK) {
				const u32 d = sm.group_digit[i0 / VEC];
				if (i0 >= sm.bbeg[d] && i0 < sm.bend[d]) {
					typedef OT kvec_t __attribute__((ext_vector_type(VEC)));
					typedef kvec_t avec_t __attribute__((aligned(16)));
					*(avec_t *)(kout + (u32)(sm.delta[d] + i0)) = *(const kvec_t *)((const char *)sm.stage + sidx(i0));
				}
			}
		}
		{
			const u32 inf = sm.info[cd];
			const u32 ccd = inf & 31u, hd = (inf >> 5) & 31u, taild = (inf >> 10) & 31u, enoughd = (inf >> 16) & 1u;
			const u32 from = enoughd ? sm.bend[cd] : sm.rbeg[cd], to = enoughd ? 0u : ccd, nk = enoughd ? taild : hd;
#pragma unroll
			for (u32 e = 0; e < VEC; ++e) {
				const u32 k = part * VEC + e;
				if (k < nk)
					sm.carry[cd][to + k] = staged(from + k);
			}
		}
	}
	{
		const u32 tid = tid0, cd = tid >> 2, part = tid & 3u;
		__syncthreads();
		if (tid < 256) {
			u32 inf = 0, dest = 0;
			if (cc) {
				const u32 pos = __hip_atomic_fetch_add(cursors + 256u + tid, cc, __ATOMIC_RELAXED, __HIP_MEMORY_SCOPE_AGENT);
				if (pos + cc > C::BACK)
					atomicOr(overflow, 1u);
				else {
					inf = cc;
					dest = slot_base(tid) + (cap - C::BACK) + pos;
				}
			}
			sm.info[tid] = inf;
			sm.delta[tid] = dest;
		}
		__syncthreads();
		const u32 nk = sm.info[cd], dest = sm.delta[cd];
#pragma unroll
		for (u32 e = 0; e < VEC; ++e) {
			const u32 k = part * VEC + e;
			if (k < nk)
				kout[dest + k] = sm.carry[cd][k];
		}
	}
}

}
```

### radix_sorting_amd/csrc/rsx_route_blind.hpp

```cpp
#pragma once

namespace {

template <typename KT> constexpr int blind_kind(size_t payload_bytes, bool rank = false)
{
	return payload_bytes ? (rank ? 2 : 3) : (sizeof(KT) == 8 ? 1 : 0);
}
inline bool blind_gate(const Ctx &c, bool allow_ws_blind = false)
{
	return !(env().no_blind || env().no_slack || !hybrid_enabled() || !c.fast || capture_armed() || verify_mode() ||
	         (c.small.external && !(allow_ws_blind && c.ws_blind)) || env().no_speculation);
}
inline void blind_called_off(Ctx &c, int kind)
{
	c.blind_backoff[kind] = std::min<u32>(2 * c.blind_backoff[kind] + 1, 31);
	c.blind_skip[kind] = c.blind_backoff[kind];
}
inline void blind_refresh(Ctx &c)
{
	const u32 epoch = g_env_epoch.load();
	if (c.env_epoch != epoch) {
		c.env_epoch = epoch;
		c.blind_no_room = false;
		for (int k = 0; k < 4; ++k)
			c.blind_skip[k] = c.blind_backoff[k] = 0;
		c.log_skip = c.log_backoff = 0;
		c.boff_forget = true;
	}
}
inline int blind_forget_device_backoff(Ctx &c)
{
	if (c.boff_forget && c.seg.p) {
		HIP_TRY(hipMemsetAsync(&SegView(c).ctl()->boff_skip, 0, 2 * sizeof(u32), c.stream));
		c.boff_forget = false;
	}
	return RSX_OK;
}
template <typename KT> size_t blind_keys_end()
{
	if (sizeof(KT) == 4 && dense_cap_max<KT>() >= LEAFC_CAP)
		return (size_t)32769 << 16;
	return (size_t)1 << 30;
}
template <typename KT> bool blind_wanted(Ctx &c, size_t n, size_t payload_bytes = 0, bool rank = false)
{
	if constexpr (sizeof(KT) < 4)
		return false;
	if (!blind_gate(c))
		return false;
	if (n < ((size_t)1 << 22) || n >= (payload_bytes || rank ? (size_t)1 << 30 : blind_keys_end<KT>()))
		return false;
	if (payload_bytes) {
		if (sizeof(KT) != 4 || payload_bytes != 4 || n > ((size_t)1 << 29) ||
		    n < std::min((size_t)1 << 22, (size_t)1 << env().two_level_min_log2))
			return false;
	} else {
		size_t floor_keys = sizeof(KT) == 8 ? (size_t)9 << 19 : (size_t)15 << 19;
		if (env().blind_min_log2)
			floor_keys = (size_t)1 << env().blind_min_log2;
		floor_keys = std::min(floor_keys, (size_t)1 << env().two_level_min_log2);
		if (n < floor_keys)
			return false;
	}
	blind_refresh(c);
	const int kind = blind_kind<KT>(payload_bytes, rank);
	if (c.blind_skip[kind]) {
		--c.blind_skip[kind];
		return false;
	}
	return true;
}

template <typename KT> bool async_blind_ok(Ctx &c, size_t n)
{
	if constexpr (sizeof(KT) < 4)
		return false;
	if (!blind_gate(c, true))
		return false;
	size_t floor_keys = sizeof(KT) == 8 ? (size_t)1 << 23 : (size_t)9 << 20;
	if (env().blind_min_log2)
		floor_keys = (size_t)1 << env().blind_min_log2;
	floor_keys = std::min(floor_keys, (size_t)1 << env().two_level_min_log2);
	blind_refresh(c);
	return n >= std::max(floor_keys, (size_t)1 << 22) && n < (c.ws_blind ? (size_t)1 << 30 : blind_keys_end<KT>());
}
template <typename KT> bool async_pairs_blind_ok(Ctx &c, size_t n, size_t payload_bytes)
{
	if (sizeof(KT) != 4 || payload_bytes != 4)
		return false;
	if (!blind_gate(c))
		return false;
	blind_refresh(c);
	return n >= std::min((size_t)1 << 24, (size_t)1 << env().two_level_min_log2) && n >= ((size_t)1 << 22) && n <= ((size_t)1 << 29);
}

template <typename... Bufs> void blind_give_up_room(Ctx &c, Bufs &...bufs)
{
	(void)hipGetLastError();
	c.slack1_cap = c.slack_cap = 0;
	if (!g_in_async) {
		(bufs.release(), ...);
		c.blind_no_room = true;
	}
}

template <typename KT>
int blind_enqueue(Ctx &c, KT *src, KT *aux, size_t n, KdfArgs<KT> ka, int *enqueued)
{
	typedef Sc2Cfg<KT, NoVal> C2;
	*enqueued = 0;
	const u32 mean1 = (u32)(n >> 8), mean2 = (u32)(n >> 16);
	const u32 cap1 = level1_slot_cap<KT>(mean1);
	const u32 cap2 = slot_cap_for(mean2);
	if (cap2 > std::max((u32)LeafShapes<KT>::Big::CAP, dense_cap_max<KT>()))
		return RSX_OK;
	if (c.blind_no_room)
		return RSX_OK;
	u32 lo = (aux && !env().no_aux_slots && cap1 >= (u32)C2::TILE) ? (u32)std::min<size_t>(n / cap1, 255) : 0u;
	c.slack_cap = cap2;
	c.slack_mean = mean2;
	const size_t slot2_bytes = dense_slots<KT>(c) ? 2 : sizeof(KT);
	if (c.slack1.ensure(((size_t)(256 - lo) * cap1 + C2::TILE) * sizeof(KT)) != RSX_OK ||
	    c.slack.ensure(((size_t)65536 * cap2 + C2::TILE) * slot2_bytes) != RSX_OK) {
		blind_give_up_room(c, c.slack1, c.slack);
		return RSX_OK;
	}
	if (lo && !SlotParts(aux, c.slack1.p, lo, cap1, sizeof(KT), C2::TILE).fits32()) {
		lo = 0;
		if (c.slack1.ensure(((size_t)256 * cap1 + C2::TILE) * sizeof(KT)) != RSX_OK) {
			blind_give_up_room(c, c.slack1, c.slack);
			return RSX_OK;
		}
	}
	c.slack1_lo = lo;
	RSX_TRY(seg_layout<KT>(c, n));
	RSX_TRY(c.gscan.ensure(256 * sizeof(u64)));
	const SegView sv(c);
	const u64 ntiles0 = sv.L.rows - seg_extra_rows<KT>();
	SegCtl *ctl = sv.ctl();
	SegTile *tiles = sv.tiles();
	LeafSeg *segtab = sv.segtab();
	u32 *btile = sv.btile();
	u64 *off1 = (u64 *)c.gscan.p;
	if (!c.seg_ev && !c.small.external)
		HIP_TRY(hipEventCreateWithFlags(&c.seg_ev, hipEventDisableTiming));
	if (c.host_segctl)
		c.host_segctl->mode = SEG_MODE_NONE;
	c.slack1_cap = cap1;
	c.slack_cap = cap2;
	const bool atoms = pass16a_wanted<KT>(c);
	const bool atoms64 = pass64a_narrow_wanted<KT>(c);
	typedef Pass32aCfgT<sizeof(KT) == 8 ? 14 : 28> P32;
	const size_t min32 = env().pass32_min_mi ? (size_t)env().pass32_min_mi << 20 : sizeof(KT) == 8 ? (size_t)3 << 23 : (size_t)13 << 22;
	const bool atoms1 = (sizeof(KT) == 4 ? atoms : !env().no_unstable) && !env().no_pass32a && n >= min32 &&
	                    cap1 >= (u32)P32::TILE + 2 * PASS32_BACK;
	const bool rep4 = (c.hints & 1u) != 0 || (env().probe & 4u) != 0;
	c.narrow1 = sizeof(KT) == 8 && atoms1 && atoms64 && lo != 0 && !rep4 && !env().no_narrow1 && (((uintptr_t)aux) & 63) == 0 &&
	            (size_t)256 * cap1 * 4 <= n * sizeof(KT);
	static_assert(sizeof(SegCtl) <= 256, "the control block is not part of what is zeroed");
	RSX_TRY(blind_forget_device_backoff(c));
	hipLaunchKernelGGL((rsx_blind_precheck_kernel<KT>), dim3(1 + 512), dim3(1024), 0, c.stream, (const KT *)src, (u64)n, ka, ctl,
	                   c.plan(), c.dev_host_plan, (u32x4 *)sv.status(0), (u64)(2 * sv.L.st_bytes / 16),
	                   4u,
	                   (u32)(sizeof(KT) == 4 && dense_slots<KT>(c) && !env().no_leaf16 && !env().no_shift ? 1 : 0),
	                   (u32)(narrow_slots_ok<KT>(cap2) ? (c.narrow1 ? 2 : 1) : 0), 0u,
	                   (u32)(g_in_async ? 1 : 0), (u32)((env().probe & 4u) ? 1u : c.hints));
	{
		if (atoms1) {
			const SlotParts parts(aux, c.slack1.p, lo, cap1, sizeof(KT), C2::TILE);
			KT *kbase = (KT *)parts.base;
			const u32 off_lo = parts.off_lo, off_hi = parts.off_hi;
			u32 *cur1 = sv.cursors(1);
			u32 *ovf = &ctl->overflow;
			const bool plain = ka.fmask == 0 && ka.sflip == 0 && ka.desc == 0;
			ProfScope prof(1, (u64)n * 2 * sizeof(KT), c.stream);
			const bool prefetch = sizeof(KT) == 4 && env().pass32_prefetch > 0;
#define RSX_LAUNCH_P32R(DIGV, PF, REPV)                                                                                      \
			hipLaunchKernelGGL((rsx_pass32a_kernel<KT, DIGV, PF, P32, REPV>), dim3(256), dim3(P32::BLOCK), 0, c.stream,              \
			                   (const KT *)src, (u64)n, kbase, lo, off_lo, off_hi, cap1, (const SegCtl *)ctl, cur1, ovf, ka)
#define RSX_LAUNCH_P32(DIGV, PF)                                                                                             \
			do {                                                                                                                 \
				if (rep4 && !(PF))                                                                                               \
					RSX_LAUNCH_P32R(DIGV, false, 4);                                                                             \
				else                                                                                                             \
					RSX_LAUNCH_P32R(DIGV, PF, 1);                                                                                \
			} while (0)
			if constexpr (sizeof(KT) == 4) {
				if (plain && prefetch)
					RSX_LAUNCH_P32(DIG_PLAIN, true);
				else if (!plain && prefetch)
					RSX_LAUNCH_P32(DIG_GENERIC, true);
			}
			if (plain && !prefetch)
				RSX_LAUNCH_P32(DIG_PLAIN, false);
			else if (!prefetch)
				RSX_LAUNCH_P32(DIG_GENERIC, false);
#undef RSX_LAUNCH_P32
#undef RSX_LAUNCH_P32R
			if constexpr (sizeof(KT) == 8) {
				if (c.narrow1) {
					if (plain)
						hipLaunchKernelGGL((rsx_pass32a_kernel<KT, DIG_PLAIN, false, P32, 1, u32>), dim3(256), dim3(P32::BLOCK), 0, c.stream,
						                   (const KT *)src, (u64)n, (u32 *)aux, 256u, 0u, 0u, cap1, (const SegCtl *)ctl, cur1, ovf, ka);
					else
						hipLaunchKernelGGL((rsx_pass32a_kernel<KT, DIG_GENERIC, false, P32, 1, u32>), dim3(256), dim3(P32::BLOCK), 0, c.stream,
						                   (const KT *)src, (u64)n, (u32 *)aux, 256u, 0u, 0u, cap1, (const SegCtl *)ctl, cur1, ovf, ka);
				}
			}
			HIP_TRY(hipGetLastError());
		}
	}
	if (!atoms1)
		RSX_TRY(launch_seg_pass<KT>(c, src, lo ? aux : nullptr, n, ka, -2, 1));
	hipLaunchKernelGGL(rsx_seg_tiles_kernel, dim3(32), dim3(256), 0, c.stream, (const u64 *)c.ghist(), (u64)n, (const Plan *)c.plan(),
	                   atoms ? (u32)Pass16aCfg::TILE : (u32)C2::TILE, tiles, ctl, btile, off1, cap1,
	                   (const u32 *)sv.cursors(1), (u32)ntiles0, atoms1 ? PASS32_BACK : 0u,
	                   atoms64 ? (u32)Pass2wCfg<u32>::TILE : 0u, c.narrow1 ? (u32)Pass64aCfgLow::TILE : 0u);
	RSX_TRY(launch_seg_pass<KT>(c, lo ? aux : nullptr, nullptr, n, ka, -2, 2));
	hipLaunchKernelGGL((rsx_seg_slack_plan_kernel<u32>), dim3(256), dim3(256), 0, c.stream,
	                   (const u32 *)sv.cursors(0), (const u32 *)btile, (const u64 *)c.ghist(),
	                   (const Plan *)c.plan(), ctl, segtab, cap2, c.dev_host_segctl, (const u64 *)off1,
	                   (atoms ? 2u : atoms64 ? 3u : 1u) | ((env().probe & 1u) << 8));
	HIP_TRY(hipGetLastError());
	if (c.seg_ev)
		HIP_TRY(hipEventRecord(c.seg_ev, c.stream));
	u32 leaf_shape = LeafShapes<KT>::shape_for_slots(cap2);
	if (dense_slots<KT>(c))
		leaf_shape |= 0x100u;
	if (sizeof(KT) == 8 && cap2 <= 5120u)
		leaf_shape |= 0x200u;
	RSX_TRY(launch_leaves<KT>(c, src, aux, n, ka, HYB_TWO_LEVEL, leaf_shape, (const u64 *)off1));
	*enqueued = 1;
	return RSX_OK;
}

inline int blind_verdict(Ctx &c, int kind, size_t pmark, bool *through)
{
	HIP_TRY(hipEventSynchronize(c.seg_ev));
	*through = c.host_segctl->mode == SEG_MODE_LEAVES;
	if (*through) {
		c.blind_backoff[kind] = 0;
	} else {
		blind_called_off(c, kind);
		prof_called_off(pmark, c.stream);
	}
	return RSX_OK;
}

template <typename KT>
int sort_keys_blind(Ctx &c, KT *src, KT *aux, size_t n, KdfArgs<KT> ka, KT **result, rsx_info *info, int *done)
{
	*done = 0;
	int enqueued = 0;
	const size_t pmark = prof_mark();
	RSX_TRY(blind_enqueue<KT>(c, src, aux, n, ka, &enqueued));
	if (!enqueued)
		return RSX_OK;
	bool through = false;
	RSX_TRY(blind_verdict(c, blind_kind<KT>(0), pmark, &through));
	if (!through) {
		c.slack_cap = 0;
		return RSX_OK;
	}
	if (sizeof(KT) == 8 && c.host_segctl->narrow) {
		const bool n1 = c.host_segctl->narrow == 2u;
		prof_rebook(pmark, c.stream, 2, (u64)n * (4 + sizeof(KT)));
		prof_rebook(pmark, c.stream, 1, (u64)n * ((n1 ? 4 : sizeof(KT)) + 4), 3);
		if (n1)
			prof_rebook(pmark, c.stream, 1, (u64)n * (sizeof(KT) + 4));
	}
	const Plan plan = *c.host_plan;
	info_from_plan(info, plan);
	KT *final = (plan.ncols & 1) ? aux : src;
	*result = final;
	if (info) {
		info->result_in_aux = final == aux;
		info->hybrid = 5u;
	}
	*done = 1;
	return RSX_OK;
}

template <typename KT> WsBlind blind_sizes(size_t n)
{
	typedef Sc2Cfg<KT, NoVal> C2;
	const u32 cap1 = level1_slot_cap<KT>((u32)(n >> 8)), cap2 = slot_cap_for((u32)(n >> 16));
	const u32 lo = cap1 >= (u32)C2::TILE ? (u32)std::min<size_t>(n / cap1, 255) : 0u;
	const size_t slot2 = (sizeof(KT) == 4 && cap2 <= dense_cap_max<KT>()) ? 2 : sizeof(KT);
	WsBlind b;
	b.gscan = 256 * sizeof(u64);
	b.seg = ws_align256(seg_bytes<KT>(n));
	b.slack1 = ws_align256(((size_t)(256 - lo) * cap1 + C2::TILE) * sizeof(KT));
	b.slack = ws_align256(((size_t)65536 * cap2 + C2::TILE) * slot2);
	return b;
}

inline void borrow_blind(Ctx &v, char *ws, size_t ws_bytes, const WsLayout &l)
{
	if (!l.blind_fits(ws_bytes))
		return;
	v.gscan.borrow(ws + l.gscan_off, l.blind.gscan);
	v.seg.borrow(ws + l.seg_off, l.blind.seg);
	v.slack1.borrow(ws + l.slack1_off, l.blind.slack1);
	v.slack.borrow(ws + l.slack_off, l.blind.slack);
	v.ws_blind = true;
}

template <typename KT, typename VT, typename LC>
void launch_leaf_pairs16(Ctx &c, unsigned grid, u32 cap2, KT *kfinal, VT *vfinal, const LeafSeg *segtab, const SegCtl *ctl,
                         KdfArgs<KT> ka, const u32 *redo)
{
	hipLaunchKernelGGL((rsx_leaf_pairs_kernel<KT, VT, LC, true>), dim3(grid), dim3(LC::BLOCK), 0, c.stream, (const KT *)c.slack.p,
	                   (const VT *)c.slack_v.p, cap2, kfinal, vfinal, (const Plan *)c.plan(), segtab, ctl, ka, (u32)HYB_TWO_LEVEL,
	                   (const u64 *)nullptr, (u64)0, redo);
}

template <typename KT, typename VT>
int pairs_blind_enqueue(Ctx &c, const KT *kin, const VT *vin, KT *kfinal, VT *vfinal, size_t n, KdfArgs<KT> ka, int *enqueued,
                        KT *kspare = nullptr, VT *vspare = nullptr)
{
	typedef Sc2Cfg<KT, VT> C2;
	typedef LeafCfg<u32, 4, 20, 3> L;
	typedef unsigned short K2;
	static_assert(sizeof(KT) == 4, "two MSB digits above two bytes");
	*enqueued = 0;
	const u32 mean1 = (u32)(n >> 8), mean2 = (u32)(n >> 16);
	const u32 cap1 = slot_cap_for(mean1), cap2 = slot_cap_for(mean2);
	typedef LeafCfg<u32, 16, 12, 1> LB;
	typedef LeafKCfg<1024, 10240, 4, 13> P10;
	if (cap2 > (u32)P10::CAP)
		return RSX_OK;
	const bool big = cap2 > (u32)L::CAP || env().pairs_leaf_big;
	if (c.blind_no_room)
		return RSX_OK;
	u32 lo = (!env().no_aux_slots && cap1 >= (u32)C2::TILE && (kspare || vspare)) ? (u32)std::min<size_t>(n / cap1, 255) : 0u;
	for (int attempt = 0; attempt < 2; ++attempt) {
		const u32 klo = kspare ? lo : 0u, vlo = vspare ? lo : 0u;
		if (c.slack1.ensure(((size_t)(256 - klo) * cap1 + C2::TILE) * sizeof(KT)) != RSX_OK ||
		    c.slack1_v.ensure(((size_t)(256 - vlo) * cap1 + C2::TILE) * sizeof(VT)) != RSX_OK)
			break;
		if (lo && ((klo && !SlotParts(kspare, c.slack1.p, lo, cap1, sizeof(KT), C2::TILE).fits32()) ||
		           (vlo && !SlotParts(vspare, c.slack1_v.p, lo, cap1, sizeof(VT), C2::TILE).fits32()))) {
			lo = 0;
			continue;
		}
		break;
	}
	const u32 klo = kspare ? lo : 0u, vlo = vspare ? lo : 0u;
	if (c.slack1.ensure(((size_t)(256 - klo) * cap1 + C2::TILE) * sizeof(KT)) != RSX_OK ||
	    c.slack1_v.ensure(((size_t)(256 - vlo) * cap1 + C2::TILE) * sizeof(VT)) != RSX_OK ||
	    c.slack.ensure(((size_t)65536 * cap2 + C2::TILE) * sizeof(K2)) != RSX_OK ||
	    c.slack_v.ensure(((size_t)65536 * cap2 + C2::TILE) * sizeof(VT)) != RSX_OK) {
		blind_give_up_room(c, c.slack1, c.slack1_v, c.slack, c.slack_v);
		return RSX_OK;
	}
	RSX_TRY(seg_layout<KT>(c, n));
	static_assert((int)C2::TILE == (int)Sc2Cfg<KT, NoVal>::TILE, "one layout for both");
	RSX_TRY(c.gscan.ensure(256 * sizeof(u64)));
	const SegView sv(c);
	const u64 rows = sv.L.rows, ntiles0 = rows - seg_extra_rows<KT>();
	SegCtl *ctl = sv.ctl();
	SegTile *tiles = sv.tiles();
	LeafSeg *segtab = sv.segtab();
	u32 *btile = sv.btile();
	u64 *off1 = (u64 *)c.gscan.p;
	if (!c.seg_ev)
		HIP_TRY(hipEventCreateWithFlags(&c.seg_ev, hipEventDisableTiming));
	c.host_segctl->mode = SEG_MODE_NONE;
	RSX_TRY(blind_forget_device_backoff(c));
	hipLaunchKernelGGL((rsx_blind_precheck_kernel<KT>), dim3(1 + 512), dim3(1024), 0, c.stream, kin, (u64)n, ka, ctl, c.plan(),
	                   c.dev_host_plan, (u32x4 *)sv.status(0), (u64)(2 * sv.L.st_bytes / 16),
	                   (u32)sizeof(KT),
	                   0u, 0u,
	                   (u32)((vin == nullptr && kfinal == nullptr && !env().no_packed_keys) ? 1 : 0), (u32)(g_in_async ? 1 : 0));
	SegArgs sa = sv.args(sizeof(KT));
	KT *k1out = (KT *)c.slack1.p, *k1lo = (KT *)c.slack1.p;
	VT *v1out = (VT *)c.slack1_v.p, *v1lo = (VT *)c.slack1_v.p;
	const void *k1hi = nullptr, *v1hi = nullptr;
	sa.lo_slots = lo;
	if (klo) {
		const SlotParts parts(kspare, c.slack1.p, lo, cap1, sizeof(KT), C2::TILE);
		sa.out_off_lo = parts.off_lo;
		sa.out_off_hi = parts.off_hi;
		k1out = (KT *)parts.base;
		k1lo = kspare;
		k1hi = (const void *)parts.hi;
	}
	if (vlo) {
		const SlotParts parts(vspare, c.slack1_v.p, lo, cap1, sizeof(VT), C2::TILE);
		sa.v_off_lo = parts.off_lo;
		sa.v_off_hi = parts.off_hi;
		v1out = (VT *)parts.base;
		v1lo = vspare;
		v1hi = (const void *)parts.hi;
	}
	{
		ProfScope prof(1, (u64)n * (2 * sizeof(KT) + (vin ? 2 : 1) * sizeof(VT)), c.stream);
		sa.slack_cap = cap1;
		const u32 flags = (u32)SCATTER_SEG_SLACK | (u32)SCATTER_BLIND | (u32)SCATTER_BLIND_TOP | (vin ? 0u : (u32)SCATTER_GEN_INDEX);
		hipLaunchKernelGGL((rsx_scatter2_kernel<KT, VT, u32, C2, false, DIG_GENERIC, false, KT, true>), dim3((unsigned)ntiles0),
		                   dim3(C2::BLOCK), 0, c.stream, kin, k1out, vin, v1out, (u64)n, 0u,
		                   (const u64 *)c.ghist(), 1u, sv.cursors(1), sv.status(1), ka, flags, (u64 *)nullptr,
		                   (const Plan *)c.plan(), 0u, 0u, (const u32 *)nullptr, sa);
	}
	sa.out_off_lo = sa.out_off_hi = sa.v_off_lo = sa.v_off_hi = 0;
	sa.kin_hi = k1hi;
	sa.vin_hi = v1hi;
	hipLaunchKernelGGL(rsx_seg_tiles_kernel, dim3(32), dim3(256), 0, c.stream, (const u64 *)c.ghist(), (u64)n, (const Plan *)c.plan(),
	                   (u32)C2::TILE, tiles, ctl, btile, off1, cap1, (const u32 *)sv.cursors(1), (u32)ntiles0);
	{
		ProfScope prof(1, (u64)n * (sizeof(KT) + sizeof(K2) + 2 * sizeof(VT)), c.stream);
		sa.slack_cap = cap2;
		hipLaunchKernelGGL((rsx_scatter2_kernel<KT, VT, u32, C2, false, DIG_GENERIC, false, K2, true>), dim3((unsigned)rows),
		                   dim3(C2::BLOCK), 0, c.stream, (const KT *)k1lo, (K2 *)c.slack.p, (const VT *)v1lo,
		                   (VT *)c.slack_v.p, (u64)n, 0u, (const u64 *)c.ghist(), 1u, sv.cursors(0), sv.status(0), ka,
		                   (u32)SCATTER_SEG_SLACK | (u32)SCATTER_BLIND, (u64 *)nullptr, (const Plan *)c.plan(), 0u, 0u,
		                   (const u32 *)nullptr, sa);
	}
	hipLaunchKernelGGL((rsx_seg_slack_plan_kernel<u32>), dim3(256), dim3(256), 0, c.stream, (const u32 *)sv.cursors(0), (const u32 *)btile,
	                   (const u64 *)c.ghist(), (const Plan *)c.plan(), ctl, segtab, cap2, c.dev_host_segctl, (const u64 *)off1,
	                   1u | ((env().probe & 1u) << 8));
	HIP_TRY(hipGetLastError());
	HIP_TRY(hipEventRecord(c.seg_ev, c.stream));
	{
		ProfScope prof(2, (u64)n * (sizeof(K2) + 2 * sizeof(VT) + (kfinal ? sizeof(KT) : 0)), c.stream);
		unsigned lds_grid = env().leaf_grid;
		const u32 *lds_redo = nullptr;
		if (!env().no_leaf16) {
			typedef LeafKCfg<512, 5120, 8> P5;
			typedef LeafKCfg<256, 2560, 8, 11> P2;
			typedef LeafKCfg<128, 1280, 6, 10> P1;
			u32 *redo = sv.redo();
#define RSX_LEAFP(P) \
	hipLaunchKernelGGL((rsx_leafp_kernel<KT, VT, P, true>), dim3(65536u), dim3(P::BLOCK), 0, c.stream, (const KT *)c.slack.p, \
	                   (const VT *)c.slack_v.p, cap2, kfinal, vfinal, (const Plan *)c.plan(), (const LeafSeg *)segtab, ctl, ka, redo, \
	                   (u32)env().leaf16_maxbin)
			typedef LeafKCfg<64, 256, 8, 9> P0;
			typedef LeafKCfg<64, 512, 8, 10> P0b;
			if (big)
				RSX_LEAFP(P10);
			else if (cap2 <= (u32)P0::CAP && !env().no_leaf16q)
				RSX_LEAFP(P0);
			else if (cap2 <= (u32)P0b::CAP && !env().no_leaf16q)
				RSX_LEAFP(P0b);
			else if (cap2 <= (u32)P1::CAP)
				RSX_LEAFP(P1);
			else if (cap2 <= (u32)P2::CAP)
				RSX_LEAFP(P2);
			else
				RSX_LEAFP(P5);
#undef RSX_LEAFP
			lds_grid = 4096;
			lds_redo = redo;
		}
		if (big)
			launch_leaf_pairs16<KT, VT, LB>(c, lds_grid, cap2, kfinal, vfinal, segtab, ctl, ka, lds_redo);
		else
			launch_leaf_pairs16<KT, VT, L>(c, lds_grid, cap2, kfinal, vfinal, segtab, ctl, ka, lds_redo);
	}
	HIP_TRY(hipGetLastError());
	*enqueued = 1;
	return RSX_OK;
}

template <typename KT, typename VT>
int pairs_blind(Ctx &c, const KT *kin, const VT *vin, KT *kfinal, VT *vfinal, size_t n, KdfArgs<KT> ka, rsx_info *info, int *done,
                KT *kspare = nullptr, VT *vspare = nullptr)
{
	*done = 0;
	int enqueued = 0;
	const size_t pmark = prof_mark();
	RSX_TRY((pairs_blind_enqueue<KT, VT>(c, kin, vin, kfinal, vfinal, n, ka, &enqueued, kspare, vspare)));
	if (!enqueued)
		return RSX_OK;
	bool through = false;
	RSX_TRY(blind_verdict(c, blind_kind<KT>(sizeof(VT), vin == nullptr), pmark, &through));
	if (!through)
		return RSX_OK;
	info_from_plan(info, *c.host_plan);
	if (info)
		info->hybrid = 5u;
	*done = 1;
	return RSX_OK;
}

}
```

### radix_sorting_amd/csrc/rsx_route_levels.hpp

```cpp
#pragma once

namespace {

static_assert(sizeof(SegCtl) <= SEG_CTL_BYTES && sizeof(LeafSeg) == SEG_LEAFSEG_BYTES && sizeof(SegTile) == SEG_TILE_BYTES,
              "rsx_seg_layout.hpp states the sizes of rsx_hybrid.hpp's structs");

template <typename KT> constexpr u64 seg_extra_rows() { return sizeof(KT) == 8 ? 512 : 256; }

template <typename KT> u64 seg_tile_rows(size_t n, u64 rows)
{
	if (sizeof(KT) == 4)
		return (n + Pass16aCfg::TILE - 1) / Pass16aCfg::TILE + 514;
	return std::max<u64>(rows, (n + Pass2wCfg<u32>::TILE - 1) / Pass2wCfg<u32>::TILE + 514);
}

template <typename KT> SegLayout seg_layout_of(size_t n)
{
	typedef Sc2Cfg<KT, NoVal> C2;
	const u64 rows = seg_rows(n, C2::TILE, seg_extra_rows<KT>());
	return seg_layout_for(sizeof(KT), n, C2::TILE, seg_extra_rows<KT>(), seg_tile_rows<KT>(n, rows));
}

template <typename KT> size_t seg_bytes(size_t n) { return seg_layout_of<KT>(n).total; }

template <typename KT> int seg_layout(Ctx &c, size_t n)
{
	c.seg_lay = seg_layout_of<KT>(n);
	const void *before = c.seg.p;
	RSX_TRY(c.seg.ensure(c.seg_lay.total));
	if (c.seg.p != before || c.seg.external)
		HIP_TRY(hipMemsetAsync(c.seg.p, 0, SEG_CTL_BYTES, c.stream));
	return RSX_OK;
}

struct SegView {
	char *const p;
	const SegLayout &L;
	explicit SegView(const Ctx &c) : p((char *)c.seg.p), L(c.seg_lay) {}
	SegCtl *ctl() const { return (SegCtl *)p; }
	u32 *hist() const { return (u32 *)(p + L.hist_off); }
	SegTile *tiles() const { return (SegTile *)(p + L.tiles_off); }
	LeafSeg *segtab() const { return (LeafSeg *)(p + L.segtab_off); }
	u32 *btile() const { return (u32 *)(p + L.btile_off); }
	u32 *redo() const { return (u32 *)(p + L.redo_off); }
	u32 *status(u32 j) const { return (u32 *)(p + L.status(j)); }
	u32 *cursors(u32 j) const { return (u32 *)(p + L.cursors(j)); }
	SegArgs args(size_t key_bytes) const
	{
		SegArgs sa{};
		sa.ctl = ctl();
		sa.hist = hist();
		sa.tiles = tiles();
		sa.slots = (u32)key_bytes - 1;
		sa.overflow = &ctl()->overflow;
		return sa;
	}
	int reset_and_tiles(Ctx &c, size_t n, u32 tile) const
	{
		HIP_TRY(hipMemsetAsync(p, 0, L.status(1), c.stream));
		hipLaunchKernelGGL(rsx_seg_tiles_kernel, dim3(32), dim3(256), 0, c.stream, (const u64 *)c.ghist(), (u64)n, (const Plan *)c.plan(),
		                   tile, tiles(), ctl(), btile());
		return RSX_OK;
	}
};

template <typename KT> struct LeafShapes {
	typedef LeafCfg<KT, 4, 32, sizeof(KT) == 8 ? 2 : 4, true, false> Small;
	typedef LeafCfg<KT, 16, sizeof(KT) == 8 ? 16 : 32> Big;
	static constexpr bool HAS_MEDIUM = sizeof(KT) == 4;
	typedef LeafCfg<KT, 8, 32, 4, true, false> Medium;
	static constexpr bool HAS_FIT = sizeof(KT) == 4;
	typedef LeafCfg<KT, 4, 20, 4, true, false> Fit;
	typedef LeafCfg<KT, 4, 8, 8, true, false> Fit2k;
	typedef LeafCfg<KT, 4, 12, 6, true, false> Fit3k;
	static u32 shape_for_slots(u32 cap)
	{
		if (HAS_FIT && cap <= (u32)Fit2k::CAP)
			return 32u;
		if (HAS_FIT && cap <= (u32)Fit3k::CAP)
			return 64u;
		if (HAS_FIT && cap <= (u32)Fit::CAP)
			return 8u;
		return shape_for(cap);
	}
	static u32 shape_for(u32 m)
	{
		if (m <= (u32)Small::CAP)
			return 1u;
		if (HAS_MEDIUM && m <= (u32)Medium::CAP)
			return 4u;
		return 2u;
	}
};

bool hybrid_enabled() { return !env().no_hybrid; }

template <typename KT> HybCaps hybrid_caps(size_t n)
{
	HybCaps caps{0, 0, 0, 0};
	if constexpr (sizeof(KT) >= 4) {
		if (hybrid_enabled() && n < ((size_t)1 << 30)) {
			caps.cap1 = (u32)LeafShapes<KT>::Big::CAP;
			caps.min_cols1 = 3;
			if (n >= ((size_t)1 << env().two_level_min_log2)) {
				caps.cap2 = (u32)LeafShapes<KT>::Big::CAP;
				caps.min_cols2 = 4;
			}
		}
	}
	return caps;
}

static inline u32 slot_cap_for(u32 mean)
{
	u32 r = 0;
	while ((u64)(r + 1) * (r + 1) <= mean)
		++r;
	const u32 need = std::max(mean + mean / 4, mean + 7 * (r + 1) + 8);
	return ((need + 255) / 256) * 256;
}

template <typename KT> u32 level1_slot_cap(u32 mean)
{
	u32 cap1 = slot_cap_for(mean) + env().cap1_pad_kib * (1024u / (u32)sizeof(KT));
	if (!env().no_odd_stride && (size_t)cap1 * sizeof(KT) >= ((size_t)1 << 20)) {
		const u32 unit = 65536u / (u32)sizeof(KT);
		cap1 = (cap1 + unit - 1) / unit * unit;
		if ((cap1 / unit) % 2u == 0)
			cap1 += unit;
	}
	return cap1;
}

template <typename KT> bool narrow_slots_ok(u32 cap2)
{
	return sizeof(KT) == 8 && cap2 >= 512u && cap2 <= 5120u && !env().no_leaf16 && !env().no_narrow_slots;
}

constexpr u32 LEAFC_CAP = 40960;
template <typename KT> u32 dense_cap_max()
{
	if (sizeof(KT) != 4)
		return 0u;
	const bool big = !env().no_leafc && !env().no_leaf16 && !env().no_pass16 && !env().no_pass16a && !env().no_unstable;
	return big ? LEAFC_CAP : (u32)LeafShapes<KT>::Fit::CAP;
}
template <typename KT> bool dense_slots(const Ctx &c)
{
	if (sizeof(KT) != 4 || env().no_dense_slots || c.slack_cap == 0 || c.slack_cap > dense_cap_max<KT>())
		return false;
	if (c.slack_cap > (u32)LeafShapes<KT>::Fit::CAP)
		return true;
	if (!env().no_leaf16)
		return true;
	return env().force_dense_slots || c.slack_cap > (u32)LeafShapes<KT>::Fit3k::CAP;
}

template <typename KT>
int launch_leaves(Ctx &c, KT *src, KT *aux, size_t n, KdfArgs<KT> ka, u32 level, u32 shapes, const u64 *off1 = nullptr)
{
	typedef typename LeafShapes<KT>::Small S;
	typedef typename LeafShapes<KT>::Big B;
	const unsigned grid_s = level == HYB_TWO_LEVEL ? env().leaf_grid : 256u;
	const unsigned grid_1 = 65536u;
	const unsigned grid_b = 256u;
	const SegView sv(c);
	const LeafSeg *segtab = level == HYB_TWO_LEVEL ? (const LeafSeg *)sv.segtab() : nullptr;
	const SegCtl *ctl = sv.ctl();
	const bool dense = (shapes & 0x100u) != 0;
	ProfScope prof(2, (u64)n * (dense ? 2 + sizeof(KT) : 2 * sizeof(KT)), c.stream);
	const KT *slots = level == HYB_TWO_LEVEL ? (const KT *)c.slack.p : nullptr;
	const u32 nopre = env().no_leaf_prefix ? 2u : 0u;
	u32 skip_narrowable = nopre;
	if constexpr (sizeof(KT) == 8) {
		if ((shapes & 0x200u) && !env().no_leaf16) {
			u32 *redo = sv.redo();
			SegCtl *wctl = sv.ctl();
#define RSX_LEAFK(K4, K8)                                                                                                      \
	do {                                                                                                                       \
		hipLaunchKernelGGL((rsx_leafk_kernel<KT, u32, K4>), dim3(grid_1), dim3(K4::BLOCK), 0, c.stream, src, aux,               \
		                   (const Plan *)c.plan(), segtab, wctl, ka, 0u, (u32)K4::CAP, slots, c.slack_cap, redo,               \
		                   (u32)env().leaf16_maxbin);                                                                          \
		hipLaunchKernelGGL((rsx_leafk_kernel<KT, u64, K8>), dim3(grid_1), dim3(K8::BLOCK), 0, c.stream, src, aux,               \
		                   (const Plan *)c.plan(), segtab, wctl, ka, 0u, (u32)K8::CAP, slots, c.slack_cap, redo,               \
		                   (u32)env().leaf16_maxbin);                                                                          \
		if (narrow_slots_ok<KT>(c.slack_cap))                                             \
			hipLaunchKernelGGL((rsx_leafk_kernel<KT, u32, K4, true>), dim3(grid_1), dim3(K4::BLOCK), 0, c.stream, src, aux,     \
			                   (const Plan *)c.plan(), segtab, wctl, ka, 0u, (u32)K4::CAP, slots, c.slack_cap, redo,           \
			                   (u32)env().leaf16_maxbin);                                                                      \
	} while (0)
			typedef LeafKCfg<512, 5120, 8> K4;
			typedef LeafKCfg<512, 5120, 8> K8;
			typedef LeafKCfg<256, 2560, 8, 11> K2;
			typedef LeafKCfg<128, 1280, 6, 10> K1;
			typedef LeafKCfg<64, 256, 8, 9> K0;
			typedef LeafKCfg<64, 512, 8, 10> K0b;
			if (c.slack_cap <= (u32)K0::CAP && !env().no_leaf16q)
				RSX_LEAFK(K0, K0);
			else if (c.slack_cap <= (u32)K0b::CAP && !env().no_leaf16q)
				RSX_LEAFK(K0b, K0b);
			else if (c.slack_cap <= (u32)K1::CAP)
				RSX_LEAFK(K1, K1);
			else if (c.slack_cap <= (u32)K2::CAP)
				RSX_LEAFK(K2, K2);
			else {
				hipLaunchKernelGGL((rsx_leafk_kernel<KT, u32, K4>), dim3(grid_1), dim3(K4::BLOCK), 0, c.stream, src, aux,
				                   (const Plan *)c.plan(), segtab, wctl, ka, 0u, (u32)K4::CAP, slots, c.slack_cap, redo,
				                   (u32)env().leaf16_maxbin);
				hipLaunchKernelGGL((rsx_leafk8_kernel<KT, u64, LeafK8Cfg>), dim3(grid_1), dim3(LeafK8Cfg::BLOCK), 0, c.stream, src, aux,
				                   (const Plan *)c.plan(), segtab, wctl, ka, 0u, (u32)LeafK8Cfg::CAP, slots, c.slack_cap, redo,
				                   (u32)env().leaf16_maxbin);
				if (narrow_slots_ok<KT>(c.slack_cap))
					hipLaunchKernelGGL((rsx_leafk_kernel<KT, u32, K4, true>), dim3(grid_1), dim3(K4::BLOCK), 0, c.stream, src, aux,
					                   (const Plan *)c.plan(), segtab, wctl, ka, 0u, (u32)K4::CAP, slots, c.slack_cap, redo,
					                   (u32)env().leaf16_maxbin);
			}
#undef RSX_LEAFK
			typedef LeafCfg<u32, 4, 32, 3, true, false> N;
			hipLaunchKernelGGL((rsx_leaf_sort_kernel<KT, N, u32>), dim3(2048), dim3(N::BLOCK), 0, c.stream, src, aux, (u64)n,
			                   (const u64 *)c.ghist(), (const Plan *)c.plan(), segtab, ctl, ka, level, 0u, (u32)S::CAP, slots,
			                   c.slack_cap, nopre, off1, (const u32 *)redo);
			hipLaunchKernelGGL((rsx_leaf_sort_kernel<KT, S>), dim3(2048), dim3(S::BLOCK), 0, c.stream, src, aux, (u64)n,
			                   (const u64 *)c.ghist(), (const Plan *)c.plan(), segtab, ctl, ka, level, 0u, (u32)S::CAP, slots,
			                   c.slack_cap, nopre | 1u, off1, (const u32 *)redo);
			HIP_TRY(hipGetLastError());
			return RSX_OK;
		}
		if (shapes & 1u) {
			typedef LeafCfg<u32, 4, 32, 3, true, false> N;
			static_assert(N::CAP == S::CAP, "the narrow shape takes the small shape's leaves");
			hipLaunchKernelGGL((rsx_leaf_sort_kernel<KT, N, u32>), dim3(grid_s), dim3(N::BLOCK), 0, c.stream, src, aux, (u64)n,
			                   (const u64 *)c.ghist(), (const Plan *)c.plan(), segtab, ctl, ka, level, 0u, (u32)S::CAP, slots,
			                   c.slack_cap, nopre, off1);
			skip_narrowable |= 1u;
		}
	}
	if constexpr (sizeof(KT) == 4) {
		if (dense && !env().no_leaf16) {
			u32 *redo = sv.redo();
			SegCtl *wctl = sv.ctl();
			if (c.slack_cap > 5120u || (env().force_leafc && c.slack_cap <= LEAFC_CAP)) {
				const unsigned force = env().force_leafc;
				typedef Leaf16Cfg<256, 6144, 8, 12> L6k;
				typedef Leaf16Cfg<256, 7680, 8, 12> L7k;
				typedef Leaf16Cfg<512, 10240, 8, 13> L10k;
				typedef Leaf16Cfg<512, 15360, 8, 13> L15k;
				typedef Leaf16Cfg<1024, 20480, 8, 14> L20k;
				const unsigned grid_c = 256u;
#define RSX_LAUNCH_LC(NVEC, REDO)                                                                                           \
				hipLaunchKernelGGL((rsx_leafc_kernel<KT, LeafCCfg<NVEC>>), dim3(grid_c), dim3(LeafCCfg<NVEC>::BLOCK), 0, c.stream, src, aux, \
				                   (const Plan *)c.plan(), segtab, ctl, ka, 0u, (u32)LeafCCfg<NVEC>::CAP, (const uint16_t *)slots,     \
				                   c.slack_cap, (const u32 *)(REDO))
#define RSX_LAUNCH_L16B(CFG, NVEC)                                                                                          \
				do {                                                                                                        \
					hipLaunchKernelGGL((rsx_leaf16_kernel<KT, CFG>), dim3(grid_1), dim3(CFG::BLOCK), 0, c.stream, src, aux,   \
					                   (const Plan *)c.plan(), segtab, wctl, ka, 0u, (u32)CFG::CAP, (const uint16_t *)slots,   \
					                   c.slack_cap, redo, (u32)env().leaf16_maxbin);                                          \
					RSX_LAUNCH_LC(NVEC, redo);                                                                                \
				} while (0)
				const u32 cap = c.slack_cap;
				const unsigned pick = force ? force
				                            : cap <= (u32)L6k::CAP ? 4u : cap <= (u32)L7k::CAP ? 5u : cap <= (u32)L10k::CAP ? 2u
				                            : cap <= (u32)L15k::CAP ? 6u : cap <= (u32)L20k::CAP ? 3u : 1u;
				if (pick == 4 && cap <= (u32)L6k::CAP)
					RSX_LAUNCH_L16B(L6k, 2);
				else if (pick == 5 && cap <= (u32)L7k::CAP)
					RSX_LAUNCH_L16B(L7k, 2);
				else if (pick == 2 && cap <= (u32)L10k::CAP)
					RSX_LAUNCH_L16B(L10k, 2);
				else if (pick == 6 && cap <= (u32)L15k::CAP)
					RSX_LAUNCH_L16B(L15k, 2);
				else if (pick == 3 && cap <= (u32)L20k::CAP)
					RSX_LAUNCH_L16B(L20k, 3);
				else if (cap <= (u32)LeafCCfg<4>::CAP)
					RSX_LAUNCH_LC(4, nullptr);
				else
					RSX_LAUNCH_LC(5, nullptr);
#undef RSX_LAUNCH_L16B
#undef RSX_LAUNCH_LC
				HIP_TRY(hipGetLastError());
				return RSX_OK;
			}
			typedef Leaf16Cfg<256, 5120, 8, 12> L5k;
			typedef Leaf16Cfg<128, 2560, 8, 11> L2k;
			typedef Leaf16WCfg<1024, 10, 4> W1k;
			typedef Leaf16WCfg<512, 9, 4> W512;
			typedef Leaf16WCfg<2048, 10, 4> W2k;
			if (c.slack_cap > (u32)W1k::CAP && c.slack_cap <= (u32)W2k::CAP && !env().no_leaf16w2k) {
				hipLaunchKernelGGL((rsx_leaf16w_kernel<KT, W2k>), dim3(grid_1 / W2k::NW), dim3(W2k::BLOCK), 0, c.stream, src, aux,
				                   (const Plan *)c.plan(), segtab, wctl, ka, 0u, (u32)W2k::CAP, (const uint16_t *)slots, c.slack_cap);
				HIP_TRY(hipGetLastError());
				return RSX_OK;
			}
			if (c.slack_cap <= (u32)W1k::CAP) {
				typedef Leaf16QCfg<4> Q256;
				if (c.slack_cap <= (u32)Q256::CAP && !env().no_leaf16q)
					hipLaunchKernelGGL((rsx_leaf16q_kernel<KT, Q256>), dim3(grid_1 / Q256::ROWS), dim3(Q256::BLOCK), 0, c.stream, src, aux,
					                   (const Plan *)c.plan(), segtab, wctl, ka, 0u, (u32)Q256::CAP, (const uint16_t *)slots, c.slack_cap);
				else if (c.slack_cap <= (u32)W512::CAP)
					hipLaunchKernelGGL((rsx_leaf16w_kernel<KT, W512>), dim3(grid_1 / W512::NW), dim3(W512::BLOCK), 0, c.stream, src, aux,
					                   (const Plan *)c.plan(), segtab, wctl, ka, 0u, (u32)W512::CAP, (const uint16_t *)slots, c.slack_cap);
				else
					hipLaunchKernelGGL((rsx_leaf16w_kernel<KT, W1k>), dim3(grid_1 / W1k::NW), dim3(W1k::BLOCK), 0, c.stream, src, aux,
					                   (const Plan *)c.plan(), segtab, wctl, ka, 0u, (u32)W1k::CAP, (const uint16_t *)slots, c.slack_cap);
				HIP_TRY(hipGetLastError());
				return RSX_OK;
			}
#define RSX_LAUNCH_L16(KERNEL, CFG, GRID)                                                                                     \
			hipLaunchKernelGGL((KERNEL<KT, CFG>), dim3(GRID), dim3(CFG::BLOCK), 0, c.stream, src, aux, (const Plan *)c.plan(),  \
			                   segtab, wctl, ka, 0u, (u32)CFG::CAP, (const uint16_t *)slots, c.slack_cap, redo,                \
			                   (u32)env().leaf16_maxbin)
			if (c.slack_cap <= (u32)L2k::CAP)
				RSX_LAUNCH_L16(rsx_leaf16_kernel, L2k, grid_1);
			else
				RSX_LAUNCH_L16(rsx_leaf16_kernel, L5k, grid_1);
#undef RSX_LAUNCH_L16
			typedef typename LeafShapes<KT>::Fit F_;
			hipLaunchKernelGGL((rsx_leaf_sort_kernel<KT, F_, uint16_t, true>), dim3(4096), dim3(F_::BLOCK), 0, c.stream, src, aux,
			                   (u64)n, (const u64 *)c.ghist(), (const Plan *)c.plan(), segtab, ctl, ka, level, 0u, (u32)F_::CAP, slots,
			                   c.slack_cap, nopre, off1, (const u32 *)redo);
			HIP_TRY(hipGetLastError());
			return RSX_OK;
		}
	}
	if constexpr (LeafShapes<KT>::HAS_FIT) {
#define RSX_LAUNCH_FIT(BIT, SHAPE)                                                                                          \
		if (shapes & (BIT)) {                                                                                               \
			typedef typename LeafShapes<KT>::SHAPE F_;                                                                      \
			if (dense)                                                                                                      \
				hipLaunchKernelGGL((rsx_leaf_sort_kernel<KT, F_, uint16_t, true>), dim3(grid_s), dim3(F_::BLOCK), 0, c.stream, \
				                   src, aux, (u64)n, (const u64 *)c.ghist(), (const Plan *)c.plan(), segtab, ctl, ka, level, 0u, \
				                   (u32)F_::CAP, slots, c.slack_cap, nopre, off1);                                          \
			else                                                                                                            \
				hipLaunchKernelGGL((rsx_leaf_sort_kernel<KT, F_>), dim3(grid_s), dim3(F_::BLOCK), 0, c.stream, src, aux,     \
				                   (u64)n, (const u64 *)c.ghist(), (const Plan *)c.plan(), segtab, ctl, ka, level, 0u,       \
				                   (u32)F_::CAP, slots, c.slack_cap, nopre, off1);                                          \
		}
		RSX_LAUNCH_FIT(32u, Fit2k)
		RSX_LAUNCH_FIT(64u, Fit3k)
		RSX_LAUNCH_FIT(8u, Fit)
#undef RSX_LAUNCH_FIT
	}
	if (shapes & 1u)
		hipLaunchKernelGGL((rsx_leaf_sort_kernel<KT, S>), dim3(grid_s), dim3(S::BLOCK), 0, c.stream, src, aux, (u64)n,
		                   (const u64 *)c.ghist(), (const Plan *)c.plan(), segtab, ctl, ka, level, 0u, (u32)S::CAP, slots,
		                   c.slack_cap, skip_narrowable, off1);
	typedef typename LeafShapes<KT>::Medium M;
	const u32 big_lo = LeafShapes<KT>::HAS_MEDIUM ? (u32)M::CAP : (u32)S::CAP;
	if constexpr (LeafShapes<KT>::HAS_MEDIUM) {
		if (shapes & 4u)
			hipLaunchKernelGGL((rsx_leaf_sort_kernel<KT, M>), dim3(level == HYB_TWO_LEVEL ? env().leaf_grid : 256u), dim3(M::BLOCK), 0, c.stream, src,
			                   aux, (u64)n, (const u64 *)c.ghist(), (const Plan *)c.plan(), segtab, ctl, ka, level, (u32)S::CAP, (u32)M::CAP,
			                   slots, c.slack_cap, nopre, off1);
	}
	if (shapes & 2u)
		hipLaunchKernelGGL((rsx_leaf_sort_kernel<KT, B>), dim3(grid_b), dim3(B::BLOCK), 0, c.stream, src, aux, (u64)n,
		                   (const u64 *)c.ghist(), (const Plan *)c.plan(), segtab, ctl, ka, level, big_lo, (u32)B::CAP, slots,
		                   c.slack_cap, nopre, off1);
	HIP_TRY(hipGetLastError());
	return RSX_OK;
}

template <typename KT> bool pass16a_wanted(const Ctx &c)
{
	if constexpr (sizeof(KT) == 4)
	{
		if (!dense_slots<KT>(c) || env().no_pass16 || env().no_pass16a || env().no_unstable || env().no_leaf16)
			return false;
		if (c.slack_cap > 1024u)
			return true;
		if (c.slack_cap == 1024u && c.slack_mean) {
			u32 r = 0;
			while ((u64)(r + 1) * (r + 1) <= c.slack_mean)
				++r;
			return c.slack_mean + 7 * (r + 1) + 8 <= c.slack_cap - LEAF16_BACK;
		}
		return false;
	}
	return false;
}

template <typename KT> bool pass64a_narrow_wanted(const Ctx &c)
{
	if (sizeof(KT) != 8 || !narrow_slots_ok<KT>(c.slack_cap) || env().no_pass64a || env().no_unstable || !c.slack_mean)
		return false;
	u32 r = 0;
	while ((u64)(r + 1) * (r + 1) <= c.slack_mean)
		++r;
	return c.slack_mean + 6 * (r + 1) + 8 <= c.slack_cap - Pass2wCfg<u32>::BACK;
}

template <typename KT>
int launch_seg_pass(Ctx &c, const KT *aux, KT *src, size_t n, KdfArgs<KT> ka, int j, int blind = 0)
{
	typedef Sc2Cfg<KT, NoVal> C2;
	const SegView sv(c);
	const u64 rows = sv.L.rows;
	const u32 region = blind == 1 ? 1u : j < 0 ? 0u : (u32)j;
	u32 *const ticket = sv.status(region), *const st = sv.cursors(region);
	SegArgs sa = sv.args(sizeof(KT));
	sa.slack_cap = blind == 1 ? c.slack1_cap : j == -2 ? c.slack_cap : 0u;
	KT *const second = blind == 1 ? src : blind == 2 ? const_cast<KT *>(aux) : nullptr;
	if (j == -2)
		src = (KT *)c.slack.p;
	if (blind == 1 || blind == 2) {
		KT *first = (KT *)c.slack1.p;
		if (second && c.slack1_lo) {
			sa.lo_slots = c.slack1_lo;
			const SlotParts parts(second, c.slack1.p, c.slack1_lo, c.slack1_cap, sizeof(KT), C2::TILE);
			if (blind == 1) {
				sa.out_off_lo = parts.off_lo;
				sa.out_off_hi = parts.off_hi;
				first = (KT *)parts.base;
			} else {
				sa.kin_hi = (const void *)parts.hi;
				first = second;
			}
		}
		if (blind == 1)
			src = first;
		else
			aux = first;
	}
	const bool dense = sizeof(KT) == 4 && blind == 2 && dense_slots<KT>(c);
	ProfScope prof(dense ? 3 : 1, (u64)n * (dense ? sizeof(KT) + 2 : 2 * sizeof(KT)), c.stream);
	const bool plain = ka.fmask == 0 && ka.sflip == 0 && ka.desc == 0;
	u32 flags = j == -2 ? (u32)SCATTER_SEG_SLACK : j < 0 ? (u32)SCATTER_SEG_LEAVES : 0u;
	if (blind)
		flags |= SCATTER_BLIND | (blind == 1 ? (u32)SCATTER_BLIND_TOP : 0u);
	if (blind && !env().no_unstable)
		flags |= SCATTER_UNSTABLE;
	const u32 pi = j < 0 ? 0u : (u32)j;
	const unsigned grid = blind == 1 ? (unsigned)(rows - seg_extra_rows<KT>()) : (unsigned)rows;
	const u32 shift0 = 0u;
#define RSX_LAUNCH_SEG(DIGV)                                                                                               \
	hipLaunchKernelGGL((rsx_scatter2_kernel<KT, NoVal, u32, C2, false, DIGV, false, KT, true>), dim3(grid),                 \
	                   dim3(C2::BLOCK), 0, c.stream, aux, src, (const NoVal *)nullptr, (NoVal *)nullptr, (u64)n, shift0,     \
	                   (const u64 *)c.ghist(), 1u, st, ticket, ka, flags, (u64 *)nullptr,             \
	                   (const Plan *)c.plan(), pi, 0u, (const u32 *)nullptr, sa)
	if constexpr (sizeof(KT) == 4) {
		if (dense && pass16a_wanted<KT>(c)) {
			const unsigned pgrid = 512;
			if (plain)
				hipLaunchKernelGGL((rsx_pass16a_kernel<KT, DIG_PLAIN>), dim3(pgrid), dim3(Pass16aCfg::BLOCK), 0, c.stream, (const KT *)aux,
				                   (const KT *)sa.kin_hi, sa.lo_slots, (unsigned short *)src, sa.tiles, sa.ctl, (const Plan *)c.plan(),
				                   st, sa.slack_cap, sa.overflow, ka);
			else
				hipLaunchKernelGGL((rsx_pass16a_kernel<KT, DIG_GENERIC>), dim3(pgrid), dim3(Pass16aCfg::BLOCK), 0, c.stream, (const KT *)aux,
				                   (const KT *)sa.kin_hi, sa.lo_slots, (unsigned short *)src, sa.tiles, sa.ctl, (const Plan *)c.plan(),
				                   st, sa.slack_cap, sa.overflow, ka);
			HIP_TRY(hipGetLastError());
			return RSX_OK;
		}
		if (dense && !env().no_pass16 && !env().no_unstable && !env().no_leaf16) {
			const u32 *btile = sv.btile();
#define RSX_LAUNCH_P16(DIGV, CFG)                                                                                          \
	hipLaunchKernelGGL((rsx_pass16_kernel<KT, DIGV, CFG>), dim3(grid), dim3(CFG::BLOCK), 0, c.stream, (const KT *)aux,      \
	                   (const KT *)sa.kin_hi, sa.lo_slots, (unsigned short *)src, sa.tiles, btile, sa.ctl,                  \
	                   (const Plan *)c.plan(), st, sa.slack_cap, sa.overflow, ka, (u32)env().pass16_dbg)
			if (env().pass16_wgs == 1) {
				if (plain)
					RSX_LAUNCH_P16(DIG_PLAIN, Pass16Cfg<1>);
				else
					RSX_LAUNCH_P16(DIG_GENERIC, Pass16Cfg<1>);
			} else {
				if (plain)
					RSX_LAUNCH_P16(DIG_PLAIN, Pass16Cfg<2>);
				else
					RSX_LAUNCH_P16(DIG_GENERIC, Pass16Cfg<2>);
			}
#undef RSX_LAUNCH_P16
			HIP_TRY(hipGetLastError());
			return RSX_OK;
		}
		if (dense) {
#define RSX_LAUNCH_SEG16(DIGV)                                                                                             \
	hipLaunchKernelGGL((rsx_scatter2_kernel<KT, NoVal, u32, C2, false, DIGV, false, uint16_t, true>), dim3(grid),           \
	                   dim3(C2::BLOCK), 0, c.stream, aux, (uint16_t *)src, (const NoVal *)nullptr, (NoVal *)nullptr, (u64)n, \
	                   shift0, (const u64 *)c.ghist(), 1u, st, ticket, ka, flags, (u64 *)nullptr,      \
	                   (const Plan *)c.plan(), pi, 0u, (const u32 *)nullptr, sa)
			if (plain)
				RSX_LAUNCH_SEG16(DIG_PLAIN);
			else
				RSX_LAUNCH_SEG16(DIG_GENERIC);
#undef RSX_LAUNCH_SEG16
			HIP_TRY(hipGetLastError());
			return RSX_OK;
		}
	}
	if (plain)
		RSX_LAUNCH_SEG(DIG_PLAIN);
	else
		RSX_LAUNCH_SEG(DIG_GENERIC);
#undef RSX_LAUNCH_SEG
	if constexpr (sizeof(KT) == 8) {
		if (blind == 2 && narrow_slots_ok<KT>(c.slack_cap)) {
#define RSX_LAUNCH_SEG32(DIGV)                                                                                             \
	hipLaunchKernelGGL((rsx_scatter2_kernel<KT, NoVal, u32, C2, false, DIGV, false, u32, true>), dim3(grid),                \
	                   dim3(C2::BLOCK), 0, c.stream, aux, (u32 *)src, (const NoVal *)nullptr, (NoVal *)nullptr, (u64)n,     \
	                   shift0, (const u64 *)c.ghist(), 1u, st, ticket, ka, flags, (u64 *)nullptr,     \
	                   (const Plan *)c.plan(), pi, 0u, (const u32 *)nullptr, sa)
			if (pass64a_narrow_wanted<KT>(c)) {
				typedef Pass2wCfg<u32> P64;
				hipLaunchKernelGGL((rsx_pass64a_kernel<KT, u32>), dim3(P64::GRID), dim3(P64::BLOCK), 0, c.stream, (const KT *)aux,
				                   (const KT *)sa.kin_hi, sa.lo_slots, (u32 *)src, sa.tiles, sa.ctl, (const Plan *)c.plan(),
				                   st, sa.slack_cap, sa.overflow, ka);
				if (c.narrow1 && second) {
					typedef Pass64aCfgLow P64L;
					hipLaunchKernelGGL((rsx_pass64a_kernel<u32, u32, P64L>), dim3(P64L::GRID), dim3(P64L::BLOCK), 0, c.stream, (const u32 *)second,
					                   (const u32 *)nullptr, 0u, (u32 *)src, sa.tiles, sa.ctl, (const Plan *)c.plan(),
					                   st, sa.slack_cap, sa.overflow, KdfArgs<u32>{0, 0, 0});
				}
			} else if (plain)
				RSX_LAUNCH_SEG32(DIG_PLAIN);
			else
				RSX_LAUNCH_SEG32(DIG_GENERIC);
#undef RSX_LAUNCH_SEG32
		}
	}
	HIP_TRY(hipGetLastError());
	return RSX_OK;
}

template <typename KT>
int sort_keys_two_level(Ctx &c, KT *src, KT *aux, size_t n, KdfArgs<KT> ka, const Plan &plan, KT **result, u32 *how)
{
	typedef Sc2Cfg<KT, NoVal> C2;
	RSX_TRY(seg_layout<KT>(c, n));
	const SegView sv(c);
	const size_t st_bytes = sv.L.st_bytes;
	SegCtl *ctl = sv.ctl();
	u32 *seghist = sv.hist();
	SegTile *tiles = sv.tiles();
	LeafSeg *segtab = sv.segtab();
	u32 *btile = sv.btile();
	KT *final = (plan.ncols & 1) ? aux : src;
	if (!c.seg_ev)
		HIP_TRY(hipEventCreateWithFlags(&c.seg_ev, hipEventDisableTiming));
	RSX_TRY(sv.reset_and_tiles(c, n, (u32)C2::TILE));
	HIP_TRY(hipGetLastError());
	c.slack_cap = 0;
	if (!env().no_slack && n >= ((size_t)1 << 26)) {
		const u32 mean = (u32)(n >> 16);
		const u32 cap = slot_cap_for(mean);
		if (cap <= (u32)LeafShapes<KT>::Big::CAP && c.slack.ensure(((size_t)65536 * cap + C2::TILE) * sizeof(KT)) == RSX_OK) {
			c.slack_cap = cap;
			RSX_TRY(launch_seg_pass<KT>(c, aux, src, n, ka, -2));
			hipLaunchKernelGGL((rsx_seg_slack_plan_kernel<u32>), dim3(256), dim3(256), 0, c.stream,
			                   (const u32 *)sv.cursors(0), (const u32 *)btile, (const u64 *)c.ghist(),
			                   (const Plan *)c.plan(), ctl, segtab, cap, c.dev_host_segctl);
			HIP_TRY(hipGetLastError());
			HIP_TRY(hipEventRecord(c.seg_ev, c.stream));
			RSX_TRY(launch_leaves<KT>(c, src, aux, n, ka, HYB_TWO_LEVEL, LeafShapes<KT>::shape_for_slots(cap)));
			HIP_TRY(hipEventSynchronize(c.seg_ev));
			if (c.host_segctl->mode == SEG_MODE_LEAVES) {
				*result = final;
				*how = 4u;
				return RSX_OK;
			}
			c.slack_cap = 0;
			RSX_TRY(sv.reset_and_tiles(c, n, (u32)C2::TILE));
		} else {
			(void)hipGetLastError();
		}
	}
	{
		ProfScope prof(0, (u64)n * sizeof(KT), c.stream);
		hipLaunchKernelGGL((rsx_seg_hist1_kernel<KT>), dim3(512), dim3(1024), 0, c.stream, (const KT *)aux, (const SegTile *)tiles,
		                   (const SegCtl *)ctl, (const Plan *)c.plan(), ka, seghist);
	}
	hipLaunchKernelGGL((rsx_seg_plan_kernel<KT>), dim3(256), dim3(256), 0, c.stream, seghist, (const u64 *)c.ghist(), (u64)n,
	                   (const Plan *)c.plan(), ctl, segtab, (u32)LeafShapes<KT>::Big::CAP, c.dev_host_segctl, 0u);
	HIP_TRY(hipGetLastError());
	HIP_TRY(hipEventRecord(c.seg_ev, c.stream));
	RSX_TRY(launch_seg_pass<KT>(c, aux, src, n, ka, -1));
	RSX_TRY(launch_leaves<KT>(c, src, aux, n, ka, HYB_TWO_LEVEL, 1u));
	HIP_TRY(hipEventSynchronize(c.seg_ev));
	const SegCtl hc = *c.host_segctl;
	if (hc.mode == SEG_MODE_LEAVES) {
		if (hc.maxleaf > (u32)LeafShapes<KT>::Small::CAP)
			RSX_TRY(launch_leaves<KT>(c, src, aux, n, ka, HYB_TWO_LEVEL, LeafShapes<KT>::shape_for(hc.maxleaf)));
	} else {
		if (plan.ncols > 2) {
			ProfScope prof(0, (u64)n * sizeof(KT), c.stream);
			hipLaunchKernelGGL((rsx_seg_hist_kernel<KT>), dim3(512), dim3(1024), 0, c.stream, (const KT *)aux, (const SegTile *)tiles,
			                   (const SegCtl *)ctl, (const Plan *)c.plan(), ka, seghist);
		}
		hipLaunchKernelGGL((rsx_seg_plan_kernel<KT>), dim3(256), dim3(256), 0, c.stream, seghist, (const u64 *)c.ghist(), (u64)n,
		                   (const Plan *)c.plan(), ctl, segtab, 0u, (SegCtl *)nullptr, 1u);
		if (plan.ncols > 2)
			HIP_TRY(hipMemsetAsync(sv.status(1), 0, (plan.ncols - 2) * st_bytes, c.stream));
		for (u32 j = 0; j + 1 < plan.ncols; ++j)
			RSX_TRY(launch_seg_pass<KT>(c, aux, src, n, ka, (int)j));
	}
	*result = final;
	*how = hc.mode == SEG_MODE_LEAVES ? 2u : 3u;
	return RSX_OK;
}

template <typename KT> HybCaps hybrid_caps_pairs(size_t n, size_t val_bytes_, bool counted_too = false)
{
	HybCaps caps{0, 0, 0, 0};
	if (sizeof(KT) != 4 || val_bytes_ != 4 || !hybrid_enabled())
		return caps;
	caps.cap1 = 5120;
	caps.min_cols1 = 3;
	if ((!env().no_slack || counted_too) && n >= ((size_t)1 << env().two_level_min_log2) && n <= ((size_t)1 << 28)) {
		caps.cap2 = (u32)LeafShapes<KT>::Small::CAP;
		caps.min_cols2 = 4;
	}
	return caps;
}

template <typename KT, typename VT>
int pairs_two_level(Ctx &c, const KT *k1, const VT *v1, KT *kfinal, VT *vfinal, size_t n, KdfArgs<KT> ka, bool *ok,
                    KT *kdense = nullptr, VT *vdense = nullptr)
{
	typedef Sc2Cfg<KT, VT> C2;
	typedef LeafCfg<u32, 4, 20, 3> L;
	*ok = false;
	RSX_TRY(seg_layout<KT>(c, n));
	static_assert((int)C2::TILE == (int)Sc2Cfg<KT, NoVal>::TILE, "one layout for both");
	static_assert(sizeof(KT) == 4, "the pairs' leaves take 4-byte keys");
	const SegView sv(c);
	const u64 rows = sv.L.rows;
	SegCtl *ctl = sv.ctl();
	SegTile *tiles = sv.tiles();
	LeafSeg *segtab = sv.segtab();
	u32 *btile = sv.btile();
	if (env().no_slack) {
		if (!kdense || !vdense || !kfinal)
			return RSX_OK;
		u32 *seghist = sv.hist();
		if (!c.seg_ev)
			HIP_TRY(hipEventCreateWithFlags(&c.seg_ev, hipEventDisableTiming));
		c.host_segctl->mode = SEG_MODE_NONE;
		RSX_TRY(sv.reset_and_tiles(c, n, (u32)C2::TILE));
		{
			ProfScope prof(0, (u64)n * sizeof(KT), c.stream);
			hipLaunchKernelGGL((rsx_seg_hist1_kernel<KT>), dim3(512), dim3(1024), 0, c.stream, k1, (const SegTile *)tiles, (const SegCtl *)ctl,
			                   (const Plan *)c.plan(), ka, seghist);
		}
		hipLaunchKernelGGL((rsx_seg_plan_kernel<KT>), dim3(256), dim3(256), 0, c.stream, seghist, (const u64 *)c.ghist(), (u64)n,
		                   (const Plan *)c.plan(), ctl, segtab, (u32)L::CAP, c.dev_host_segctl, 0u);
		HIP_TRY(hipGetLastError());
		HIP_TRY(hipEventRecord(c.seg_ev, c.stream));
		HIP_TRY(hipEventSynchronize(c.seg_ev));
		if (c.host_segctl->mode != SEG_MODE_LEAVES)
			return RSX_OK;
		const SegArgs sa = sv.args(sizeof(KT));
		{
			ProfScope prof(1, (u64)n * 2 * (sizeof(KT) + sizeof(VT)), c.stream);
			hipLaunchKernelGGL((rsx_scatter2_kernel<KT, VT, u32, C2, false, DIG_GENERIC, false, KT, true>), dim3((unsigned)rows),
			                   dim3(C2::BLOCK), 0, c.stream, k1, kdense, v1, vdense, (u64)n, 0u, (const u64 *)c.ghist(), 1u,
			                   sv.cursors(0), sv.status(0), ka, (u32)SCATTER_SEG_LEAVES, (u64 *)nullptr, (const Plan *)c.plan(), 0u, 0u,
			                   (const u32 *)nullptr, sa);
		}
		{
			ProfScope prof(2, (u64)n * 2 * (sizeof(KT) + sizeof(VT)), c.stream);
			hipLaunchKernelGGL((rsx_leaf_pairs_kernel<KT, VT, L>), dim3(env().leaf_grid), dim3(L::BLOCK), 0, c.stream, (const KT *)kdense,
			                   (const VT *)vdense, 0u, kfinal, vfinal, (const Plan *)c.plan(), (const LeafSeg *)segtab, (const SegCtl *)ctl,
			                   ka);
		}
		HIP_TRY(hipGetLastError());
		*ok = true;
		return RSX_OK;
	}
	const u32 mean = (u32)(n >> 16);
	const u32 cap = slot_cap_for(mean);
	if (cap > (u32)L::CAP)
		return RSX_OK;
	if (c.slack.ensure(((size_t)65536 * cap + C2::TILE) * sizeof(KT)) != RSX_OK ||
	    c.slack_v.ensure(((size_t)65536 * cap + C2::TILE) * sizeof(VT)) != RSX_OK) {
		(void)hipGetLastError();
		return RSX_OK;
	}
	if (!c.seg_ev)
		HIP_TRY(hipEventCreateWithFlags(&c.seg_ev, hipEventDisableTiming));
	RSX_TRY(sv.reset_and_tiles(c, n, (u32)C2::TILE));
	SegArgs sa = sv.args(sizeof(KT));
	sa.slack_cap = cap;
	{
		ProfScope prof(1, (u64)n * 2 * (sizeof(KT) + sizeof(VT)), c.stream);
		hipLaunchKernelGGL((rsx_scatter2_kernel<KT, VT, u32, C2, false, DIG_GENERIC, false, KT, true>), dim3((unsigned)rows),
		                   dim3(C2::BLOCK), 0, c.stream, k1, (KT *)c.slack.p, v1, (VT *)c.slack_v.p, (u64)n, 0u, (const u64 *)c.ghist(), 1u,
		                   sv.cursors(0), sv.status(0), ka, (u32)SCATTER_SEG_SLACK, (u64 *)nullptr, (const Plan *)c.plan(), 0u, 0u,
		                   (const u32 *)nullptr, sa);
	}
	hipLaunchKernelGGL((rsx_seg_slack_plan_kernel<u32>), dim3(256), dim3(256), 0, c.stream, (const u32 *)sv.cursors(0), (const u32 *)btile,
	                   (const u64 *)c.ghist(), (const Plan *)c.plan(), ctl, segtab, cap, c.dev_host_segctl);
	HIP_TRY(hipGetLastError());
	HIP_TRY(hipEventRecord(c.seg_ev, c.stream));
	{
		ProfScope prof(2, (u64)n * (sizeof(KT) + 2 * sizeof(VT) + (kfinal ? sizeof(KT) : 0)), c.stream);
		hipLaunchKernelGGL((rsx_leaf_pairs_kernel<KT, VT, L>), dim3(env().leaf_grid), dim3(L::BLOCK), 0, c.stream, (const KT *)c.slack.p,
		                   (const VT *)c.slack_v.p, cap, kfinal, vfinal, (const Plan *)c.plan(), (const LeafSeg *)segtab,
		                   (const SegCtl *)ctl, ka);
	}
	HIP_TRY(hipGetLastError());
	HIP_TRY(hipEventSynchronize(c.seg_ev));
	*ok = c.host_segctl->mode == SEG_MODE_LEAVES;
	return RSX_OK;
}

template <typename KT, typename VT>
int pairs_one_level(Ctx &c, const KT *k1, const VT *v1, KT *kfinal, VT *vfinal, size_t n, KdfArgs<KT> ka)
{
	typedef LeafCfg<u32, 4, 20, 3> L;
	ProfScope prof(2, (u64)n * (sizeof(KT) + 2 * sizeof(VT) + (kfinal ? sizeof(KT) : 0)), c.stream);
	hipLaunchKernelGGL((rsx_leaf_pairs_kernel<KT, VT, L>), dim3(256), dim3(L::BLOCK), 0, c.stream, k1, v1, 0u, kfinal, vfinal,
	                   (const Plan *)c.plan(), (const LeafSeg *)nullptr, (const SegCtl *)nullptr, ka, (u32)HYB_ONE_LEVEL,
	                   (const u64 *)c.ghist(), (u64)n);
	HIP_TRY(hipGetLastError());
	return RSX_OK;
}

}
```

Measured before the change: 218.9.

## Pack level-1 slot keys into 24-bit atoms to cut intermediate traffic

When the first pass has consumed the top byte (shift ≤ 24), pass32a now writes its level-1 bucket slots as 24-bit keys packed 21 per 64-byte atom. pass16a reads these atoms back with lane-quarter unpacking (a DPP neighbour exchange) using smaller tiles. This is meant to cut HBM write and read traffic of the intermediate buffer by roughly a quarter. The cost is more complex staging, extra ALU work for packing and unpacking, and an overflow fallback when the shift is too large. The path is gated on size, plain-ish conditions and alignment, and can be disabled by an env flag.

```diff
diff --git a/radix_sorting_amd/csrc/rsx_env.hpp b/radix_sorting_amd/csrc/rsx_env.hpp
--- a/radix_sorting_amd/csrc/rsx_env.hpp
+++ b/radix_sorting_amd/csrc/rsx_env.hpp
@@ -44,6 +44,7 @@
 	bool no_narrow_slots = false;
 	bool no_aux_slots = false;
 	bool no_narrow1 = false;
+	bool no_pack24 = false;
 	bool no_dense_slots = false;
 	bool force_dense_slots = false;
 	bool no_unstable = false;
@@ -141,6 +142,7 @@
 		no_narrow_slots = is_one("RSX_NO_NARROW_SLOTS");
 		no_aux_slots = is_one("RSX_NO_AUX_SLOTS");
 		no_narrow1 = is_one("RSX_NO_NARROW_LEVEL1");
+		no_pack24 = is_one("RSX_NO_PACK24");
 		no_dense_slots = is_one("RSX_NO_DENSE_SLOTS");
 		force_dense_slots = is_one("RSX_DENSE_SLOTS");
 		no_leaf16 = is_one("RSX_NO_LEAF16");
diff --git a/radix_sorting_amd/csrc/rsx_hybrid.hpp b/radix_sorting_amd/csrc/rsx_hybrid.hpp
--- a/radix_sorting_amd/csrc/rsx_hybrid.hpp
+++ b/radix_sorting_amd/csrc/rsx_hybrid.hpp
@@ -1,6 +1,7 @@
 #pragma once
 
 #include "rsx_kernels.hpp"
+#include "rsx_pack24.hpp"
 
 namespace rsx {
 
@@ -108,7 +109,8 @@
                                                             u64 *__restrict__ off1_out = nullptr, u32 blind_cap = 0,
                                                             const u32 *__restrict__ status0 = nullptr, u32 ntiles0 = 0,
                                                             u32 back_cap = 0, u32 tile_narrow = 0,
-                                                            u32 tile_narrow2 = 0)
+                                                            u32 tile_narrow2 = 0,
+                                                            u32 pack24_slots = 0)
 {
 	if (plan->hyb != HYB_TWO_LEVEL || (blind_cap && ctl->blind != BLIND_GO))
 		return;
@@ -117,15 +119,20 @@
 	__shared__ u32 s_size[256], s_tb[257], s_beg[256], s_w[4], s_back[256];
 	const u32 d = threadIdx.x;
 	u32 size, back = 0;
+	bool packed_over = false;
 	if (blind_cap) {
 		if (back_cap) {
 			size = __hip_atomic_load(status0 + d, __ATOMIC_RELAXED, __HIP_MEMORY_SCOPE_AGENT);
 			back = __hip_atomic_load(status0 + 256 + d, __ATOMIC_RELAXED, __HIP_MEMORY_SCOPE_AGENT);
+			if (pack24_slots) {
+				packed_over = size > blind_cap - back_cap || back > back_cap;
+				size = pack24::words_to_keys(size);
+			}
 			size += back;
 		} else {
 			size = __hip_atomic_load(status0 + ((u64)(ntiles0 - 1) * 256 + d), __ATOMIC_RELAXED, __HIP_MEMORY_SCOPE_AGENT) & StatusBits<u32>::VALMASK;
 		}
-		const bool over = size > blind_cap || ctl->overflow != 0;
+		const bool over = (pack24_slots ? packed_over : size > blind_cap) || ctl->overflow != 0;
 		u32 tot1;
 		const u32 o = block_scan_256(size, s_w, tot1);
 		if (blockIdx.x == 0)
@@ -174,7 +181,7 @@
 		SegTile st;
 		const u32 front = s_size[k] - s_back[k];
 		if (j * tile < front) {
-			st.beg = s_beg[k] + j * tile;
+			st.beg = s_beg[k] + (pack24_slots ? pack24::keys_to_words(j * tile) : j * tile);
 			const u32 left = front - j * tile;
 			st.cnt = left < tile ? left : tile;
 		} else {
diff --git a/radix_sorting_amd/csrc/rsx_pack24.hpp b/radix_sorting_amd/csrc/rsx_pack24.hpp
--- /dev/null
+++ b/radix_sorting_amd/csrc/rsx_pack24.hpp
@@ -0,0 +1,64 @@
+#pragma once
+
+#include <cstddef>
+#include <cstdint>
+
+namespace pack24 {
+
+constexpr uint32_t ATOM_KEYS = 21, ATOM_WORDS = 16, ATOM_BYTES = 64, MASK = 0xFFFFFFu;
+constexpr uint32_t TILE_ATOMS = 1024;
+constexpr uint32_t TILE_KEYS = TILE_ATOMS * ATOM_KEYS;
+
+constexpr uint32_t key_byte(uint32_t j) { return 3u * j; }
+constexpr uint32_t pack_first(uint32_t part) { return 5u * part; }
+constexpr uint32_t pack_skip(uint32_t part) { return 16u * part - key_byte(pack_first(part)); }
+constexpr uint32_t lane_first(uint32_t part) { return part ? 5u * part + 1u : 0u; }
+constexpr uint32_t lane_count(uint32_t part) { return part ? 5u : 6u; }
+constexpr uint32_t lane_start(uint32_t part) { return key_byte(lane_first(part)) - 16u * part; }
+constexpr uint32_t words_to_keys(uint32_t words) { return words / ATOM_WORDS * ATOM_KEYS; }
+constexpr uint32_t keys_to_words(uint32_t keys) { return (keys + ATOM_KEYS - 1u) / ATOM_KEYS * ATOM_WORDS; }
+
+constexpr uint32_t align_byte(uint32_t hi, uint32_t lo, uint32_t s) { return (uint32_t)((((uint64_t)hi << 32) | lo) >> (8u * s)); }
+
+constexpr void pack_quarter(const uint32_t (&k)[6], uint32_t part, uint32_t (&out)[4])
+{
+	const uint32_t d0 = k[0] | (k[1] << 24), d1 = (k[1] >> 8) | (k[2] << 16), d2 = (k[2] >> 16) | (k[3] << 8);
+	const uint32_t d3 = k[4] | (k[5] << 24), d4 = k[5] >> 8;
+	const uint32_t s = pack_skip(part);
+	out[0] = align_byte(d1, d0, s);
+	out[1] = align_byte(d2, d1, s);
+	out[2] = align_byte(d3, d2, s);
+	out[3] = align_byte(d4, d3, s);
+}
+
+constexpr void unpack_quarter(const uint32_t (&v)[4], uint32_t next, uint32_t part, uint32_t (&k)[6])
+{
+	const uint32_t s = lane_start(part);
+	const uint32_t r0 = align_byte(v[1], v[0], s), r1 = align_byte(v[2], v[1], s), r2 = align_byte(v[3], v[2], s);
+	const uint32_t r3 = align_byte(next, v[3], s), r4 = align_byte(0u, next, s);
+	k[0] = r0 & MASK;
+	k[1] = align_byte(r1, r0, 3u) & MASK;
+	k[2] = align_byte(r2, r1, 2u) & MASK;
+	k[3] = r2 >> 8;
+	k[4] = r3 & MASK;
+	k[5] = align_byte(r4, r3, 3u) & MASK;
+}
+
+constexpr uint32_t slot_stride_words(uint32_t cap_keys, uint32_t back, bool odd_stride)
+{
+	uint32_t w = keys_to_words(cap_keys > back ? cap_keys - back : 0u) + back;
+	if (odd_stride && (size_t)w * 4u >= ((size_t)1 << 20)) {
+		const uint32_t unit = 65536u / 4u;
+		w = (w + unit - 1u) / unit * unit;
+		if ((w / unit) % 2u == 0u)
+			w += unit;
+	}
+	return w;
+}
+constexpr bool slots_fit(size_t n, uint32_t stride_words, uintptr_t addr)
+{
+	return addr != 0 && (addr & 63u) == 0 && stride_words % ATOM_WORDS == 0 && (size_t)256 * stride_words <= n;
+}
+constexpr uint32_t front_keys(uint32_t stride_words, uint32_t back) { return words_to_keys(stride_words - back); }
+
+}
diff --git a/radix_sorting_amd/csrc/rsx_pass16.hpp b/radix_sorting_amd/csrc/rsx_pass16.hpp
--- a/radix_sorting_amd/csrc/rsx_pass16.hpp
+++ b/radix_sorting_amd/csrc/rsx_pass16.hpp
@@ -202,15 +202,17 @@
 	u32 wsum[4];
 };
 
-template <typename KT, int DIG, bool PREFETCH = false>
+template <typename KT, int DIG, bool PREFETCH = false, bool PACK = false>
 __global__ __launch_bounds__(Pass16aCfg::BLOCK, 8) void rsx_pass16a_kernel(const KT *__restrict__ kin, const KT *__restrict__ kin_hi,
                                                                           u32 lo_slots, unsigned short *__restrict__ kout,
                                                                           const SegTile *__restrict__ tiles,
                                                                           const SegCtl *__restrict__ ctl,
                                                                           const Plan *__restrict__ plan, u32 *__restrict__ cursors,
-                                                                          u32 slack_cap, u32 *__restrict__ overflow, KdfArgs<KT> ka)
+                                                                          u32 slack_cap, u32 *__restrict__ overflow, KdfArgs<KT> ka,
+                                                                          u32 pack_cap = 0, u32 pack_front = 0)
 {
 	static_assert(sizeof(KT) == 4, "4-byte keys, two-byte values");
+	static_assert(!PACK || (!PREFETCH && (int)pack24::TILE_KEYS <= Pass16aCfg::TILE && Pass16aCfg::KPT == 24), "four quarter atoms per lane, six registers each");
 	typedef Pass16aCfg C;
 	constexpr int BLOCK = C::BLOCK, KPT = C::KPT, TILE = C::TILE;
 	if (ctl->blind != BLIND_GO || plan->hyb != HYB_TWO_LEVEL)
@@ -263,9 +265,30 @@
 	};
 	__syncthreads();
 	KT keep[KPT];
+	auto packed_tile = [&](const SegTile &st) { return PACK && st.beg - st.bucket * pack_cap < pack_front; };
 	auto request = [&](const u32 t, const u32 tid) {
 		const SegTile st = tiles[t];
 		const KT *p = ((kin_hi && st.bucket >= lo_slots) ? kin_hi : kin) + st.beg;
+		if constexpr (PACK) {
+			if (packed_tile(st)) {
+				const u32 natoms = st.cnt / pack24::ATOM_KEYS, part = tid & 3u;
+				const u32x4 *vp = (const u32x4 *)p + tid;
+#pragma unroll
+				for (int i = 0; i < 4; ++i) {
+					u32x4 v = {0u, 0u, 0u, 0u};
+					if ((u32)i * (BLOCK / 4) + (tid >> 2) < natoms)
+						v = __builtin_nontemporal_load(&vp[i * BLOCK]);
+					const u32 next = (u32)__builtin_amdgcn_update_dpp(0, (int)v[0], 0xF9, 0xF, 0xF, true);
+					const u32 q[4] = {v[0], v[1], v[2], v[3]};
+					u32 six[6];
+					pack24::unpack_quarter(q, next, part, six);
+#pragma unroll
+					for (int e = 0; e < 6; ++e)
+						keep[6 * i + e] = six[e];
+				}
+				return;
+			}
+		}
 		if (st.cnt == (u32)TILE && (((uintptr_t)p) & 15) == 0) {
 			typedef KT vec_t __attribute__((ext_vector_type(4)));
 			const vec_t *vp = (const vec_t *)p + tid;
@@ -301,25 +324,37 @@
 		}
 		const u32 cnt = st.cnt;
 		const bool full = cnt == (u32)TILE;
+		const bool packed = packed_tile(st);
+		const u32 natoms = cnt / pack24::ATOM_KEYS;
+		auto holds = [&](auto mode_c, int r) -> bool {
+			constexpr int MODE = decltype(mode_c)::value;
+			if constexpr (MODE == 0)
+				return true;
+			else if constexpr (MODE == 1)
+				return tid + r * BLOCK < cnt;
+			else
+				return (u32)(r / 6) * (BLOCK / 4) + (tid >> 2) < natoms && (r % 6 < 5 || part == 0u);
+		};
 		if constexpr (!PREFETCH)
 			request(t, tid);
-		if constexpr (DIG != 1) {
+		if constexpr (DIG != 1 && !PACK) {
 #pragma unroll
 			for (int r = 0; r < KPT; ++r)
 				keep[r] = kdf_apply(keep[r], ka);
 		}
-		auto count = [&](auto full_c) {
-			constexpr bool FULL = decltype(full_c)::value;
+		auto count = [&](auto mode_c) {
 #pragma unroll
 			for (int r = 0; r < KPT; ++r) {
-				if (FULL || tid + r * BLOCK < cnt)
+				if (holds(mode_c, r))
 					atomicAdd(&cell[(u32)(keep[r] >> shift) & 0xFFu], 1u);
 			}
 		};
-		if (full)
-			count(std::true_type{});
+		if (PACK && packed)
+			count(std::integral_constant<int, 2>{});
+		else if (full)
+			count(std::integral_constant<int, 0>{});
 		else
-			count(std::false_type{});
+			count(std::integral_constant<int, 1>{});
 		__syncthreads();
 
 		u32 base = 0;
@@ -385,29 +420,30 @@
 		}
 		u32 shift_b = shift;
 		asm volatile("" : "+s"(shift_b));
-		auto stage_keys = [&](auto full_c) {
-			constexpr bool FULL = decltype(full_c)::value;
+		auto stage_keys = [&](auto mode_c) {
 #pragma unroll
 			for (int r0 = 0; r0 < KPT; r0 += 8) {
 				u32 pos[8];
 #pragma unroll
 				for (int r = 0; r < 8; ++r) {
 					pos[r] = 0;
-					if (FULL || tid + (r0 + r) * BLOCK < cnt)
+					if (holds(mode_c, r0 + r))
 						pos[r] = __hip_atomic_fetch_add(&cell[(u32)(keep[r0 + r] >> shift_b) & 0xFFu], 1u, __ATOMIC_RELAXED,
 						                                __HIP_MEMORY_SCOPE_WORKGROUP);
 				}
 #pragma unroll
 				for (int r = 0; r < 8; ++r) {
-					if (FULL || tid + (r0 + r) * BLOCK < cnt)
+					if (holds(mode_c, r0 + r))
 						staged(pos[r]) = (unsigned short)keep[r0 + r];
 				}
 			}
 		};
-		if (full)
-			stage_keys(std::true_type{});
+		if (PACK && packed)
+			stage_keys(std::integral_constant<int, 2>{});
+		else if (full)
+			stage_keys(std::integral_constant<int, 0>{});
 		else
-			stage_keys(std::false_type{});
+			stage_keys(std::integral_constant<int, 1>{});
 		__syncthreads();
 
 		if constexpr (PREFETCH) {
diff --git a/radix_sorting_amd/csrc/rsx_pass32.hpp b/radix_sorting_amd/csrc/rsx_pass32.hpp
--- a/radix_sorting_amd/csrc/rsx_pass32.hpp
+++ b/radix_sorting_amd/csrc/rsx_pass32.hpp
@@ -3,6 +3,7 @@
 #include "rsx_kernels.hpp"
 #include "rsx_hybrid.hpp"
 #include "rsx_scatter2.hpp"
+#include "rsx_pack24.hpp"
 
 namespace rsx {
 
@@ -18,18 +19,19 @@
 typedef Pass32aCfgT<28> Pass32aCfg;
 constexpr u32 PASS32_BACK = Pass32aCfg::BACK;
 
-template <typename KT, typename C, int REP = 1> struct Pass32aSmem {
+template <typename KT, typename C, int REP = 1, bool PACK = false> struct Pass32aSmem {
 	__attribute__((aligned(16))) KT stage[C::STAGE];
-	__attribute__((aligned(16))) KT carry[256][64 / sizeof(KT)];
+	__attribute__((aligned(16))) KT carry[256][PACK ? pack24::ATOM_KEYS : 64 / sizeof(KT)];
 	__attribute__((aligned(16))) u32 cell[2][256 * REP];
 	u32 delta[256];
 	u32 info[256];
 	unsigned short rbeg[256], bbeg[256], bend[256];
 	unsigned char group_digit[C::STAGE / (16 / sizeof(KT))];
+	unsigned short abeg[PACK ? 256 : 1];
 	u32 wsum[4];
 };
 
-template <typename KT, int DIG, bool PREFETCH = true, typename C = Pass32aCfg, int REP_ = 1, typename OT = KT>
+template <typename KT, int DIG, bool PREFETCH = true, typename C = Pass32aCfg, int REP_ = 1, typename OT = KT, bool PACK = false>
 __global__ __launch_bounds__(C::BLOCK, C::WPE) void rsx_pass32a_kernel(const KT *__restrict__ kin, u64 n, OT *__restrict__ kout,
                                                                           u32 lo_slots, u32 off_lo, u32 off_hi, u32 cap,
                                                                           const SegCtl *__restrict__ ctl,
@@ -41,6 +43,9 @@
 	constexpr u32 VIN = 16 / sizeof(KT);
 	constexpr u32 VEC = 16 / sizeof(OT);
 	constexpr u32 ATOM = 64 / sizeof(OT);
+	constexpr u32 ATOMK = PACK ? pack24::ATOM_KEYS : ATOM;
+	constexpr u32 CPT = PACK ? 6 : VEC;
+	static_assert(!PACK || (sizeof(KT) == 4 && sizeof(OT) == 4), "packed slots: 4-byte keys");
 	constexpr bool NARROW = sizeof(OT) != sizeof(KT);
 	static_assert(!NARROW || (sizeof(KT) == 8 && sizeof(OT) == 4), "8-byte keys into four-byte slots, or the element images");
 	static_assert(KPT % (int)VIN == 0, "whole vectors per lane");
@@ -57,9 +62,16 @@
 	if (t0 >= t1)
 		return;
 	const u32 shift = ctl->shift1;
+	if constexpr (PACK) {
+		if (shift > 24u) {
+			if (threadIdx.x == 0)
+				atomicOr(overflow, 1u);
+			return;
+		}
+	}
 	const KT cmask = sizeof(KT) == 8 ? (KT)(((u64)ctl->cmask_hi << 32) | ctl->cmask_lo) : (KT)ctl->cmask_lo;
 	const KT key0 = sizeof(KT) == 8 ? (KT)(((u64)ctl->key0_hi << 32) | ctl->key0_lo) : (KT)ctl->key0_lo;
-	__shared__ Pass32aSmem<OT, C, REP_> sm;
+	__shared__ Pass32aSmem<OT, C, REP_, PACK> sm;
 	const u32 tid0 = threadIdx.x;
 	auto sidx = [](u32 pos) { return stage_swz<true>(pos * (u32)sizeof(OT)); };
 	auto staged = [&](u32 pos) -> OT & { return *(OT *)((char *)sm.stage + sidx(pos)); };
@@ -147,20 +159,27 @@
 					c += crep[q];
 				}
 				u32 h, body = 0, tail = 0, atom = 0;
-				const bool enough = cc + c >= ATOM;
+				const bool enough = cc + c >= ATOMK;
+				u32 nbody = 0;
 				if (enough) {
-					h = cc ? ATOM - cc : 0u;
+					h = cc ? ATOMK - cc : 0u;
 					atom = cc ? 1u : 0u;
-					body = (c - h) & ~(ATOM - 1u);
-					tail = (c - h) & (ATOM - 1u);
+					if constexpr (PACK) {
+						nbody = (c - h) / ATOMK;
+						body = nbody * ATOMK;
+						tail = c - h - body;
+					} else {
+						body = (c - h) & ~(ATOM - 1u);
+						tail = (c - h) & (ATOM - 1u);
+					}
 				} else {
 					h = c;
 				}
-				const u32 m = atom * ATOM + body;
+				const u32 m = PACK ? (atom + nbody) * ATOM : atom * ATOM + body;
 				if (m)
 					base = __hip_atomic_fetch_add(cursors + tid, m, __ATOMIC_RELAXED, __HIP_MEMORY_SCOPE_AGENT);
-				const u32 o = (VEC - (h & (VEC - 1u))) & (VEC - 1u);
-				rlen = (o + c + VEC - 1u) & ~(VEC - 1u);
+				const u32 o = PACK ? 0u : (VEC - (h & (VEC - 1u))) & (VEC - 1u);
+				rlen = PACK ? c | (nbody << 16) : (o + c + VEC - 1u) & ~(VEC - 1u);
 				sm.info[tid] = cc | (h << 5) | (tail << 10) | (atom << 15) | ((enough ? 1u : 0u) << 16) | (o << 17);
 				sm.bend[tid] = (unsigned short)body;
 				cc = enough ? tail : cc + c;
@@ -180,7 +199,7 @@
 				for (u32 k = 0; k < wid; ++k)
 					rstart += sm.wsum[k];
 				const u32 inf = sm.info[tid];
-				const u32 rb = rstart + (inf >> 17), bb = rb + ((inf >> 5) & 31u), be = bb + sm.bend[tid];
+				const u32 rb = (PACK ? rstart & 0xFFFFu : rstart) + (inf >> 17), bb = rb + ((inf >> 5) & 31u), be = bb + sm.bend[tid];
 				u32 rq = rb;
 #pragma unroll
 				for (u32 q = 0; q < REP; ++q) {
@@ -191,20 +210,31 @@
 				sm.rbeg[tid] = (unsigned short)rb;
 				sm.bbeg[tid] = (unsigned short)bb;
 				sm.bend[tid] = (unsigned short)be;
-				for (u32 g = bb / VEC; g < (be + VEC - 1u) / VEC; ++g)
-					sm.group_digit[g] = (unsigned char)tid;
+				if constexpr (PACK) {
+					const u32 ab = rstart >> 16;
+					sm.abeg[tid] = (unsigned short)ab;
+					for (u32 g = ab; g < ab + (be - bb) / ATOMK; ++g)
+						sm.group_digit[g] = (unsigned char)tid;
+				} else {
+					for (u32 g = bb / VEC; g < (be + VEC - 1u) / VEC; ++g)
+						sm.group_digit[g] = (unsigned char)tid;
+				}
 			}
 		}
 		__syncthreads();
 
 		if (tid < 256) {
-			const u32 atom = (sm.info[tid] >> 15) & 1u, bb = sm.bbeg[tid], m = atom * ATOM + (sm.bend[tid] - bb);
+			const u32 atom = (sm.info[tid] >> 15) & 1u, bb = sm.bbeg[tid];
+			const u32 m = PACK ? (atom + (sm.bend[tid] - bb) / ATOMK) * ATOM : atom * ATOM + (sm.bend[tid] - bb);
 			u32 dest = slot_base(tid) + base + atom * ATOM;
 			if (m && base + m > cap - C::BACK) {
 				atomicOr(overflow, 1u);
 				dest = slot_base(tid) + ATOM;
 			}
-			sm.delta[tid] = dest - bb;
+			if constexpr (PACK)
+				sm.delta[tid] = dest - sm.abeg[tid] * ATOM;
+			else
+				sm.delta[tid] = dest - bb;
 		}
 		u32 shift_b = shift;
 		asm volatile("" : "+s"(shift_b));
@@ -228,7 +258,9 @@
 #pragma unroll
 				for (int r = 0; r < SB; ++r) {
 					if (FULL || tid + (r0 + r) * BLOCK < cnt) {
-						if constexpr (NARROW)
+						if constexpr (PACK)
+							staged(pos[r]) = (OT)(DIG == 1 ? keep[r0 + r] : kdf_apply(keep[r0 + r], ka)) & pack24::MASK;
+						else if constexpr (NARROW)
 							staged(pos[r]) = (OT)(DIG == 1 ? keep[r0 + r] : kdf_apply(keep[r0 + r], ka));
 						else
 							staged(pos[r]) = keep[r0 + r];
@@ -254,15 +286,42 @@
 				typedef OT kvec_t __attribute__((ext_vector_type(VEC)));
 				typedef kvec_t avec_t __attribute__((aligned(16)));
 				kvec_t w;
-#pragma unroll
-				for (u32 e = 0; e < VEC; ++e) {
-					const u32 k = part * VEC + e;
-					w[e] = k < ccd ? sm.carry[cd][k] : staged(rb + (k - ccd));
-				}
-				*(avec_t *)(kout + (u32)(sm.delta[cd] + sm.bbeg[cd] - ATOM + part * VEC)) = w;
-			}
-		}
-		{
+				if constexpr (PACK) {
+					u32 six[6], q[4];
+#pragma unroll
+					for (u32 e = 0; e < 6; ++e) {
+						const u32 k = pack24::pack_first(part) + e;
+						six[e] = k < ccd ? sm.carry[cd][k] : staged(rb + (k - ccd));
+					}
+					pack24::pack_quarter(six, part, q);
+					w = kvec_t{q[0], q[1], q[2], q[3]};
+					*(avec_t *)(kout + (u32)(sm.delta[cd] + (sm.abeg[cd] - 1u) * ATOM + part * VEC)) = w;
+				} else {
+#pragma unroll
+					for (u32 e = 0; e < VEC; ++e) {
+						const u32 k = part * VEC + e;
+						w[e] = k < ccd ? sm.carry[cd][k] : staged(rb + (k - ccd));
+					}
+					*(avec_t *)(kout + (u32)(sm.delta[cd] + sm.bbeg[cd] - ATOM + part * VEC)) = w;
+				}
+			}
+		}
+		if constexpr (PACK) {
+			const u32 natoms = ((u32)__builtin_amdgcn_readfirstlane((int)sm.wsum[0]) + sm.wsum[1] + sm.wsum[2] + sm.wsum[3]) >> 16;
+#pragma unroll 1
+			for (u32 a = cd; a < natoms; a += BLOCK / 4) {
+				const u32 d = sm.group_digit[a];
+				const u32 kb = sm.bbeg[d] + (a - sm.abeg[d]) * ATOMK + pack24::pack_first(part);
+				u32 six[6], q[4];
+#pragma unroll
+				for (u32 e = 0; e < 6; ++e)
+					six[e] = staged(kb + e);
+				pack24::pack_quarter(six, part, q);
+				typedef u32 kvec_t __attribute__((ext_vector_type(4)));
+				typedef kvec_t avec_t __attribute__((aligned(16)));
+				*(avec_t *)(kout + (u32)(sm.delta[d] + a * ATOM + part * VEC)) = kvec_t{q[0], q[1], q[2], q[3]};
+			}
+		} else {
 			const u32 total = (u32)__builtin_amdgcn_readfirstlane((int)sm.wsum[0]) + sm.wsum[1] + sm.wsum[2] + sm.wsum[3];
 #pragma unroll 1
 			for (u32 i0 = VEC * tid; i0 < total; i0 += VEC * BLOCK) {
@@ -279,8 +338,8 @@
 			const u32 ccd = inf & 31u, hd = (inf >> 5) & 31u, taild = (inf >> 10) & 31u, enoughd = (inf >> 16) & 1u;
 			const u32 from = enoughd ? sm.bend[cd] : sm.rbeg[cd], to = enoughd ? 0u : ccd, nk = enoughd ? taild : hd;
 #pragma unroll
-			for (u32 e = 0; e < VEC; ++e) {
-				const u32 k = part * VEC + e;
+			for (u32 e = 0; e < CPT; ++e) {
+				const u32 k = part * CPT + e;
 				if (k < nk)
 					sm.carry[cd][to + k] = staged(from + k);
 			}
@@ -306,8 +365,8 @@
 		__syncthreads();
 		const u32 nk = sm.info[cd], dest = sm.delta[cd];
 #pragma unroll
-		for (u32 e = 0; e < VEC; ++e) {
-			const u32 k = part * VEC + e;
+		for (u32 e = 0; e < CPT; ++e) {
+			const u32 k = part * CPT + e;
 			if (k < nk)
 				kout[dest + k] = sm.carry[cd][k];
 		}
diff --git a/radix_sorting_amd/csrc/rsx_route_blind.hpp b/radix_sorting_amd/csrc/rsx_route_blind.hpp
--- a/radix_sorting_amd/csrc/rsx_route_blind.hpp
+++ b/radix_sorting_amd/csrc/rsx_route_blind.hpp
@@ -119,8 +119,20 @@
 	u32 lo = (aux && !env().no_aux_slots && cap1 >= (u32)C2::TILE) ? (u32)std::min<size_t>(n / cap1, 255) : 0u;
 	c.slack_cap = cap2;
 	c.slack_mean = mean2;
+	u32 capp = 0;
+	bool pack24 = false;
+	if constexpr (sizeof(KT) == 4) {
+		const size_t floor24 = env().pass32_min_mi ? (size_t)env().pass32_min_mi << 20 : (size_t)13 << 22;
+		if (!g_in_async && !env().no_pack24 && !env().no_aux_slots && !env().no_pass32a && !c.small.external && (c.hints & 1u) == 0 &&
+		    (env().probe & 4u) == 0 && pass16a_wanted<KT>(c) && n >= floor24 && n <= ((size_t)1 << 29)) {
+			capp = pack24::slot_stride_words(slot_cap_for(mean1) + env().cap1_pad_kib * 256u, PASS32_BACK, !env().no_odd_stride);
+			pack24 = capp >= (u32)Pass32aCfg::TILE + 2 * PASS32_BACK && pack24::slots_fit(n, capp, (uintptr_t)aux);
+		}
+	}
+	if (pack24)
+		lo = 0;
 	const size_t slot2_bytes = dense_slots<KT>(c) ? 2 : sizeof(KT);
-	if (c.slack1.ensure(((size_t)(256 - lo) * cap1 + C2::TILE) * sizeof(KT)) != RSX_OK ||
+	if ((!pack24 && c.slack1.ensure(((size_t)(256 - lo) * cap1 + C2::TILE) * sizeof(KT)) != RSX_OK) ||
 	    c.slack.ensure(((size_t)65536 * cap2 + C2::TILE) * slot2_bytes) != RSX_OK) {
 		blind_give_up_room(c, c.slack1, c.slack);
 		return RSX_OK;
@@ -146,14 +158,15 @@
 		HIP_TRY(hipEventCreateWithFlags(&c.seg_ev, hipEventDisableTiming));
 	if (c.host_segctl)
 		c.host_segctl->mode = SEG_MODE_NONE;
-	c.slack1_cap = cap1;
+	const u32 slot1 = pack24 ? capp : cap1;
+	c.slack1_cap = slot1;
 	c.slack_cap = cap2;
 	const bool atoms = pass16a_wanted<KT>(c);
 	const bool atoms64 = pass64a_narrow_wanted<KT>(c);
 	typedef Pass32aCfgT<sizeof(KT) == 8 ? 14 : 28> P32;
 	const size_t min32 = env().pass32_min_mi ? (size_t)env().pass32_min_mi << 20 : sizeof(KT) == 8 ? (size_t)3 << 23 : (size_t)13 << 22;
-	const bool atoms1 = (sizeof(KT) == 4 ? atoms : !env().no_unstable) && !env().no_pass32a && n >= min32 &&
-	                    cap1 >= (u32)P32::TILE + 2 * PASS32_BACK;
+	const bool atoms1 = pack24 || ((sizeof(KT) == 4 ? atoms : !env().no_unstable) && !env().no_pass32a && n >= min32 &&
+	                                 cap1 >= (u32)P32::TILE + 2 * PASS32_BACK);
 	const bool rep4 = (c.hints & 1u) != 0 || (env().probe & 4u) != 0;
 	c.narrow1 = sizeof(KT) == 8 && atoms1 && atoms64 && lo != 0 && !rep4 && !env().no_narrow1 && (((uintptr_t)aux) & 63) == 0 &&
 	            (size_t)256 * cap1 * 4 <= n * sizeof(KT);
@@ -173,7 +186,7 @@
 			u32 *cur1 = sv.cursors(1);
 			u32 *ovf = &ctl->overflow;
 			const bool plain = ka.fmask == 0 && ka.sflip == 0 && ka.desc == 0;
-			ProfScope prof(1, (u64)n * 2 * sizeof(KT), c.stream);
+			ProfScope prof(1, pack24 ? (u64)n * sizeof(KT) + (u64)n * 64 / 21 : (u64)n * 2 * sizeof(KT), c.stream);
 			const bool prefetch = sizeof(KT) == 4 && env().pass32_prefetch > 0;
 #define RSX_LAUNCH_P32R(DIGV, PF, REPV)                                                                                      \
 			hipLaunchKernelGGL((rsx_pass32a_kernel<KT, DIGV, PF, P32, REPV>), dim3(256), dim3(P32::BLOCK), 0, c.stream,              \
@@ -185,13 +198,23 @@
 				else                                                                                                             \
 					RSX_LAUNCH_P32R(DIGV, PF, 1);                                                                                \
 			} while (0)
+#define RSX_LAUNCH_P32P(DIGV)                                                                                                \
+			hipLaunchKernelGGL((rsx_pass32a_kernel<KT, DIGV, false, P32, 1, KT, true>), dim3(256), dim3(P32::BLOCK), 0, c.stream,     \
+			                   (const KT *)src, (u64)n, (KT *)aux, 256u, 0u, 0u, capp, (const SegCtl *)ctl, cur1, ovf, ka)
 			if constexpr (sizeof(KT) == 4) {
-				if (plain && prefetch)
+				if (pack24 && plain)
+					RSX_LAUNCH_P32P(DIG_PLAIN);
+				else if (pack24)
+					RSX_LAUNCH_P32P(DIG_GENERIC);
+				else if (plain && prefetch)
 					RSX_LAUNCH_P32(DIG_PLAIN, true);
 				else if (!plain && prefetch)
 					RSX_LAUNCH_P32(DIG_GENERIC, true);
 			}
-			if (plain && !prefetch)
+#undef RSX_LAUNCH_P32P
+			if (pack24)
+				;
+			else if (plain && !prefetch)
 				RSX_LAUNCH_P32(DIG_PLAIN, false);
 			else if (!prefetch)
 				RSX_LAUNCH_P32(DIG_GENERIC, false);
@@ -213,10 +236,20 @@
 	if (!atoms1)
 		RSX_TRY(launch_seg_pass<KT>(c, src, lo ? aux : nullptr, n, ka, -2, 1));
 	hipLaunchKernelGGL(rsx_seg_tiles_kernel, dim3(32), dim3(256), 0, c.stream, (const u64 *)c.ghist(), (u64)n, (const Plan *)c.plan(),
-	                   atoms ? (u32)Pass16aCfg::TILE : (u32)C2::TILE, tiles, ctl, btile, off1, cap1,
+	                   pack24 ? pack24::TILE_KEYS : atoms ? (u32)Pass16aCfg::TILE : (u32)C2::TILE, tiles, ctl, btile, off1, slot1,
 	                   (const u32 *)sv.cursors(1), (u32)ntiles0, atoms1 ? PASS32_BACK : 0u,
-	                   atoms64 ? (u32)Pass2wCfg<u32>::TILE : 0u, c.narrow1 ? (u32)Pass64aCfgLow::TILE : 0u);
-	RSX_TRY(launch_seg_pass<KT>(c, lo ? aux : nullptr, nullptr, n, ka, -2, 2));
+	                   atoms64 ? (u32)Pass2wCfg<u32>::TILE : 0u, c.narrow1 ? (u32)Pass64aCfgLow::TILE : 0u, pack24 ? 1u : 0u);
+	if (pack24) {
+		if constexpr (sizeof(KT) == 4) {
+			ProfScope prof(3, (u64)n * 2 + (u64)n * 64 / 21, c.stream);
+			hipLaunchKernelGGL((rsx_pass16a_kernel<KT, DIG_PLAIN, false, true>), dim3(512), dim3(Pass16aCfg::BLOCK), 0, c.stream,
+			                   (const KT *)aux, (const KT *)nullptr, 0u, (unsigned short *)c.slack.p, (const SegTile *)tiles,
+			                   (const SegCtl *)ctl, (const Plan *)c.plan(), sv.cursors(0), cap2, &ctl->overflow, ka, capp,
+			                   capp - PASS32_BACK);
+			HIP_TRY(hipGetLastError());
+		}
+	} else
+		RSX_TRY(launch_seg_pass<KT>(c, lo ? aux : nullptr, nullptr, n, ka, -2, 2));
 	hipLaunchKernelGGL((rsx_seg_slack_plan_kernel<u32>), dim3(256), dim3(256), 0, c.stream,
 	                   (const u32 *)sv.cursors(0), (const u32 *)btile, (const u64 *)c.ghist(),
 	                   (const Plan *)c.plan(), ctl, segtab, cap2, c.dev_host_segctl, (const u64 *)off1,
diff --git a/radix_sorting_amd/csrc/rsx_route_levels.hpp b/radix_sorting_amd/csrc/rsx_route_levels.hpp
--- a/radix_sorting_amd/csrc/rsx_route_levels.hpp
+++ b/radix_sorting_amd/csrc/rsx_route_levels.hpp
@@ -9,8 +9,9 @@
 
 template <typename KT> u64 seg_tile_rows(size_t n, u64 rows)
 {
+	static_assert(pack24::TILE_KEYS <= (u32)Pass16aCfg::TILE, "the packed tiles are the smaller ones");
 	if (sizeof(KT) == 4)
-		return (n + Pass16aCfg::TILE - 1) / Pass16aCfg::TILE + 514;
+		return (n + pack24::TILE_KEYS - 1) / pack24::TILE_KEYS + 514;
 	return std::max<u64>(rows, (n + Pass2wCfg<u32>::TILE - 1) / Pass2wCfg<u32>::TILE + 514);
 }
 
```

Result: no change. 217.8, median of 2 (-0.5%).
